# ColdCloudd/QKD_LDPC

Hardware: AMD Instinct MI355X
Metric: decoded key bits/sec + FER, N=10240 R=0.49 @ QBER=0.02, 50 iters (higher is better)
Workload: dtype f64; 1 GPU; configs[1]: alist (N=10240,M=5231,R=0.49,CW=3,SEED=666), QBER 0.02, <= 50 iterations, clamp 100.0, 4096-frame batch per GPU; frames_per_gpu=4096, decoder=sp_f64, parallelism=frames sharded over 1 GPU(s), counters all-reduced

## Files before the change

### include/qkd_ldpc.h

```cpp
#ifndef QKD_LDPC_H
#define QKD_LDPC_H

#include <stddef.h>
#include <stdint.h>

#ifdef __cplusplus
extern "C" {
#endif

#define QKD_LDPC_ABI_VERSION 1

#if defined(__GNUC__)
#define QKD_API __attribute__((visibility("default")))
#else
#define QKD_API
#endif

typedef enum qkd_status {
    QKD_OK = 0,
    QKD_ERR_INVALID_ARG = 1,
    QKD_ERR_BAD_CODE = 2,
    QKD_ERR_UNSORTED = 3,
    QKD_ERR_QBER_TOO_SMALL = 4,
    QKD_ERR_DEVICE = 5,
    QKD_ERR_OUT_OF_MEMORY = 6,
    QKD_ERR_IO = 7,
    QKD_ERR_UNSUPPORTED = 8
} qkd_status;

#define QKD_FLAG_THRESHOLD 0x1u

#define QKD_VARIANT_MASK   0x30u
#define QKD_VARIANT_SP_F64 0x00u
#define QKD_VARIANT_SP_F32 0x10u
#define QKD_VARIANT_MINSUM 0x20u
#define QKD_MINSUM_SCALE_SHIFT 8
#define QKD_MINSUM_SCALE(x) ((((uint32_t)((x) * 256.0 + 0.5)) & 0xffu) << QKD_MINSUM_SCALE_SHIFT)
#define QKD_MINSUM_DEFAULT_SCALE 0.8125
#define QKD_MINSUM_OFFSET_SHIFT 16
#define QKD_MINSUM_OFFSET(x) ((((uint32_t)((x) * 64.0 + 0.5)) & 0xffu) << QKD_MINSUM_OFFSET_SHIFT)
#define QKD_MINSUM_SELF_CORRECT 0x1000000u

typedef struct qkd_code qkd_code;
typedef struct qkd_workspace qkd_workspace;

typedef struct qkd_code_info {
    int32_t n_bits;
    int32_t n_checks;
    int32_t n_edges;
    int32_t max_bit_degree;
    int32_t max_check_degree;
    int32_t is_regular;
    int32_t device;
} qkd_code_info;

typedef struct qkd_counters {
    uint64_t frames;
    uint64_t sp_ok;
    uint64_t ldpc_ok;
    uint64_t sum_iters;
    uint64_t sum_iters_sq;
    uint32_t min_iters;
    uint32_t max_iters;
} qkd_counters;

QKD_API int qkd_abi_version(void);
QKD_API const char *qkd_last_error(void);
QKD_API const char *qkd_status_string(qkd_status s);
QKD_API int qkd_device_count(void);

QKD_API qkd_code *qkd_code_create(int32_t n_bits, int32_t n_checks, const int32_t *check_ptr,
                          const int32_t *check_idx, int device, qkd_status *status);
QKD_API qkd_code *qkd_code_from_alist(const char *path, int device, qkd_status *status);
#define QKD_READ_SORT_ROWS 0x1u
QKD_API qkd_code *qkd_code_from_alist_ex(const char *path, int device, uint32_t read_flags,
                                         qkd_status *status);
QKD_API qkd_code *qkd_code_from_dense(const char *path, int device, qkd_status *status);
QKD_API void qkd_code_destroy(qkd_code *code);
QKD_API qkd_status qkd_code_get_info(const qkd_code *code, qkd_code_info *info);
QKD_API qkd_status qkd_code_get_adjacency(const qkd_code *code, int32_t *check_ptr, int32_t *check_idx,
                                  int32_t *bit_ptr, int32_t *bit_idx);

QKD_API qkd_workspace *qkd_workspace_create(const qkd_code *code, qkd_status *status);
QKD_API void qkd_workspace_destroy(qkd_workspace *ws);


QKD_API qkd_status qkd_syndrome_batch(const qkd_code *code, const uint8_t *bits, size_t n_frames,
                              uint8_t *syndrome, void *stream);

QKD_API qkd_status qkd_decode_batch(const qkd_code *code, qkd_workspace *ws, const double *llr,
                            const uint8_t *syndrome, size_t n_frames, uint32_t max_iterations,
                            double msg_threshold, uint32_t flags, uint8_t *bits_out,
                            uint32_t *iterations, uint8_t *syndromes_match, void *stream);

QKD_API qkd_status qkd_qkd_ldpc_batch(const qkd_code *code, qkd_workspace *ws, const uint8_t *alice,
                              const uint8_t *bob, size_t n_frames, double qber,
                              uint32_t max_iterations, double msg_threshold, uint32_t flags,
                              uint8_t *bits_out, uint32_t *iterations, uint8_t *syndromes_match,
                              uint8_t *keys_match, void *stream);

QKD_API qkd_status qkd_keygen_batch(const qkd_code *code, qkd_workspace *ws, const uint64_t *seeds,
                            uint64_t seed_offset, size_t n_frames, double q_nominal,
                            uint8_t *alice, uint8_t *bob, double *exact_qber, void *stream);

QKD_API qkd_status qkd_trials_batch(const qkd_code *code, qkd_workspace *ws, const uint64_t *seeds,
                            uint64_t seed_offset, size_t n_frames, double q_nominal,
                            uint32_t max_iterations, double msg_threshold, uint32_t flags,
                            uint32_t *iterations, uint8_t *syndromes_match, uint8_t *keys_match,
                            double *exact_qber, qkd_counters *counters, void *stream);

QKD_API qkd_status qkd_interactive_batch(const qkd_code *code, qkd_workspace *ws, uint64_t simulation_seed,
                                         size_t n_points, const double *q_nominal, uint32_t max_iterations,
                                         double msg_threshold, uint32_t flags, uint32_t *iterations,
                                         uint8_t *syndromes_match, uint8_t *keys_match, double *exact_qber,
                                         uint32_t *errors, size_t *points_done);

QKD_API qkd_status qkd_counters_batch(const uint32_t *iterations, const uint8_t *syndromes_match,
                              const uint8_t *keys_match, size_t n_frames, qkd_counters *counters,
                              int device, void *stream);

QKD_API qkd_status qkd_counters_merge(const qkd_counters *records, size_t n_records, qkd_counters *out,
                                      int device, void *stream);

QKD_API qkd_status qkd_debug_set_option(qkd_workspace *ws, const char *name, const char *value);
QKD_API qkd_status qkd_debug_phase_cycles(qkd_workspace *ws, uint64_t *cycles7);
QKD_API qkd_status qkd_debug_decoder_timing(qkd_workspace *ws, int start, double *ms_total, uint64_t *launches);
QKD_API qkd_status qkd_debug_spec_replays(qkd_workspace *ws, uint64_t *replays, int reset);
QKD_API qkd_status qkd_trace_decode(const qkd_code *code, const double *llr, const uint8_t *syndrome,
                                    uint32_t max_iterations, double msg_threshold, uint32_t flags,
                                    double *c2b_trace, double *total_trace, uint32_t *iterations,
                                    uint8_t *syndrome_match);
QKD_API qkd_status qkd_debug_math(int which, const double *x, double *y, size_t n, void *stream);
QKD_API qkd_status qkd_debug_phi_sweep(int which, uint32_t first_bits, uint32_t last_bits, uint64_t *result);

QKD_API qkd_status qkd_debug_bit_order(int32_t n_bits, int32_t n_checks, const int32_t *check_ptr,
                                       const int32_t *check_idx, const char *mode, int32_t *perm_out,
                                       uint32_t *plan_out, int32_t *n_tasks_out);

QKD_API qkd_status qkd_make_seeds(uint64_t simulation_seed, size_t count, uint64_t *seeds_host);
QKD_API qkd_status qkd_qber_range(double begin, double end, double step, double *values_host,
                          size_t capacity, size_t *count);

#ifdef __cplusplus
}
#endif

#endif
```

### qkd_ldpc_amd/__init__.py

```python
from __future__ import annotations

import ctypes as C
from dataclasses import dataclass

import numpy as np

from . import _native as N
from ._native import FLAG_THRESHOLD, QkdError

try:
    import torch
except Exception:
    torch = None

__all__ = [
    "HMatrix", "QkdError", "calculate_syndrome", "sum_product_decoding",
    "sum_product_decoding_irregular", "sum_product_decoding_regular", "qkd_ldpc",
    "QKD_LDPC_irregular", "QKD_LDPC_regular", "keygen", "run_trials", "make_seeds",
    "qber_range", "Workspace", "counters_to_stats", "decoder_flags", "trace_decode", "set_debug_option",
    "spec_replays", "interactive_simulation",
]


def decoder_flags(threshold_enabled: bool = True, variant: str = "sp_f64",
                  minsum_scale: float | None = None, minsum_offset: float | None = None,
                  minsum_self_correct: bool = False) -> int:
    if variant not in N.VARIANTS:
        raise ValueError(f"unknown decoder variant {variant!r}; one of {sorted(N.VARIANTS)}")
    flags = (FLAG_THRESHOLD if threshold_enabled else 0) | N.VARIANTS[variant]
    if minsum_scale is not None:
        if variant != "minsum":
            raise ValueError("minsum_scale applies to variant='minsum' only")
        q = round(minsum_scale * 256)
        if not (1 <= q <= 255) or q != minsum_scale * 256:
            raise ValueError("minsum_scale must be k/256 for k in 1..255")
        flags |= q << N.MINSUM_SCALE_SHIFT
    if minsum_offset is not None:
        if variant != "minsum":
            raise ValueError("minsum_offset applies to variant='minsum' only")
        q = round(minsum_offset * 64)
        if not (0 <= q <= 255) or q != minsum_offset * 64:
            raise ValueError("minsum_offset must be k/64 for k in 0..255")
        flags |= q << N.MINSUM_OFFSET_SHIFT
    if minsum_self_correct:
        if variant != "minsum":
            raise ValueError("minsum_self_correct applies to variant='minsum' only")
        flags |= N.MINSUM_SELF_CORRECT
    return flags


def _ptr(t) -> int | None:
    if t is None:
        return None
    return int(t.data_ptr())


def _stream(stream, device: int) -> int | None:
    if stream is None:
        return int(torch.cuda.current_stream(device).cuda_stream)
    if isinstance(stream, int):
        return stream
    return int(stream.cuda_stream)


def _need_cuda(t, dtype, name, H: "HMatrix | None" = None):
    if not (isinstance(t, torch.Tensor) and t.is_cuda and t.dtype == dtype and t.is_contiguous()):
        raise QkdError(N.ERR_INVALID_ARG, f"{name} must be a contiguous {dtype} CUDA tensor")
    if H is not None and t.device.index != H.device:
        raise QkdError(N.ERR_INVALID_ARG,
                       f"{name} is on {t.device}, the code lives on cuda:{H.device}")


def _frames(t, width: int, name: str, frames: int | None = None) -> int:
    if t.dim() == 1 and t.numel() == width:
        f = 1
    elif t.dim() == 2 and t.shape[1] == width:
        f = int(t.shape[0])
    else:
        raise QkdError(N.ERR_INVALID_ARG,
                       f"{name} must have shape [F, {width}], got {list(t.shape)}")
    if frames is not None and f != frames:
        raise QkdError(N.ERR_INVALID_ARG, f"{name} holds {f} frames, expected {frames}")
    return f


def _need_vec(t, dtype, count: int, name: str, H: "HMatrix"):
    _need_cuda(t, dtype, name, H)
    if t.numel() != count:
        raise QkdError(N.ERR_INVALID_ARG, f"{name} must hold {count} elements, got {t.numel()}")


class HMatrix:

    def __init__(self, handle: int):
        self._h = C.c_void_p(handle)
        info = N.CodeInfo()
        N.check(N.lib().qkd_code_get_info(self._h, C.byref(info)))
        self.num_bit_nodes = info.n_bits
        self.num_check_nodes = info.n_checks
        self.n_edges = info.n_edges
        self.max_bit_nodes_weight = info.max_bit_degree
        self.max_check_nodes_weight = info.max_check_degree
        self.is_regular = bool(info.is_regular)
        self.device = info.device

    @classmethod
    def _make(cls, fn, *args):
        st = C.c_int(0)
        h = fn(*args, C.byref(st))
        if not h:
            raise QkdError(st.value, N.last_error())
        return cls(h)

    @classmethod
    def from_alist(cls, path: str, device: int = 0, sort_rows: bool = False) -> "HMatrix":
        return cls._make(N.lib().qkd_code_from_alist_ex, str(path).encode(), device,
                         N.READ_SORT_ROWS if sort_rows else 0)

    @classmethod
    def from_dense(cls, path: str, device: int = 0) -> "HMatrix":
        return cls._make(N.lib().qkd_code_from_dense, str(path).encode(), device)

    @classmethod
    def from_check_lists(cls, n_bits: int, check_ptr, check_idx, device: int = 0) -> "HMatrix":
        cp = np.ascontiguousarray(check_ptr, dtype=np.int32)
        ci = np.ascontiguousarray(check_idx, dtype=np.int32)
        return cls._make(N.lib().qkd_code_create, n_bits, cp.size - 1, cp.ctypes.data,
                         ci.ctypes.data, device)

    @classmethod
    def from_dense_array(cls, dense, device: int = 0) -> "HMatrix":
        d = np.asarray(dense)
        ptr, idx = [0], []
        for row in d:
            idx.extend(np.nonzero(row)[0].tolist())
            ptr.append(len(idx))
        return cls.from_check_lists(d.shape[1], ptr, idx, device)

    def adjacency(self):
        n, m, e = self.num_bit_nodes, self.num_check_nodes, self.n_edges
        cp = np.zeros(m + 1, np.int32)
        ci = np.zeros(e, np.int32)
        bp = np.zeros(n + 1, np.int32)
        bi = np.zeros(e, np.int32)
        N.check(N.lib().qkd_code_get_adjacency(self._h, cp.ctypes.data, ci.ctypes.data,
                                               bp.ctypes.data, bi.ctypes.data))
        return cp, ci, bp, bi

    @property
    def handle(self):
        return self._h

    def close(self):
        if getattr(self, "_h", None) is not None and self._h.value:
            N.lib().qkd_code_destroy(self._h)
            self._h = None

    def __del__(self):
        try:
            self.close()
        except Exception:
            pass


class Workspace:

    def __init__(self, H: HMatrix):
        st = C.c_int(0)
        h = N.lib().qkd_workspace_create(H.handle, C.byref(st))
        if not h:
            raise QkdError(st.value, N.last_error())
        self._h = C.c_void_p(h)

    @property
    def handle(self):
        return self._h

    def close(self):
        if getattr(self, "_h", None) is not None and self._h.value:
            N.lib().qkd_workspace_destroy(self._h)
            self._h = None

    def __del__(self):
        try:
            self.close()
        except Exception:
            pass


def _ws(ws):
    return ws.handle if ws is not None else None


def set_debug_option(name: str, value=None, workspace: "Workspace | None" = None) -> None:
    v = None if value is None else str(value).encode()
    N.check(N.lib().qkd_debug_set_option(_ws(workspace), name.encode(), v))


def spec_replays(ws: Workspace, reset: bool = False) -> int:
    v = C.c_uint64(0)
    N.check(N.lib().qkd_debug_spec_replays(ws.handle, C.byref(v), int(reset)))
    return int(v.value)


def calculate_syndrome(H: HMatrix, bits, stream=None):
    _need_cuda(bits, torch.uint8, "bits", H)
    f = _frames(bits, H.num_bit_nodes, "bits")
    out = torch.empty((f, H.num_check_nodes), dtype=torch.uint8, device=bits.device)
    N.check(N.lib().qkd_syndrome_batch(H.handle, _ptr(bits), f, _ptr(out), _stream(stream, H.device)))
    return out


@dataclass
class SPResult:
    iterations: "torch.Tensor"
    syndromes_match: "torch.Tensor"
    bits: "torch.Tensor | None"


@dataclass
class LDPCResult:
    iterations: "torch.Tensor"
    syndromes_match: "torch.Tensor"
    keys_match: "torch.Tensor"
    bits: "torch.Tensor | None"


def sum_product_decoding(H: HMatrix, llr, syndrome, max_iterations: int = 50,
                         msg_threshold: float = 100.0, threshold_enabled: bool = True,
                         want_bits: bool = True, workspace=None, stream=None,
                         variant: str = "sp_f64", minsum_scale: float | None = None,
                         minsum_offset: float | None = None, minsum_self_correct: bool = False) -> SPResult:
    _need_cuda(llr, torch.float64, "llr", H)
    _need_cuda(syndrome, torch.uint8, "syndrome", H)
    f = _frames(llr, H.num_bit_nodes, "llr")
    _frames(syndrome, H.num_check_nodes, "syndrome", f)
    dev = llr.device
    bits = torch.empty((f, H.num_bit_nodes), dtype=torch.uint8, device=dev) if want_bits else None
    iters = torch.empty(f, dtype=torch.int32, device=dev)
    ok = torch.empty(f, dtype=torch.uint8, device=dev)
    flags = decoder_flags(threshold_enabled, variant, minsum_scale, minsum_offset, minsum_self_correct)
    N.check(N.lib().qkd_decode_batch(H.handle, _ws(workspace), _ptr(llr), _ptr(syndrome), f,
                                     max_iterations, msg_threshold, flags, _ptr(bits), _ptr(iters),
                                     _ptr(ok), _stream(stream, H.device)))
    return SPResult(iters, ok, bits)


sum_product_decoding_irregular = sum_product_decoding
sum_product_decoding_regular = sum_product_decoding


def qkd_ldpc(H: HMatrix, alice, bob, qber: float, max_iterations: int = 50,
             msg_threshold: float = 100.0, threshold_enabled: bool = True,
             want_bits: bool = False, workspace=None, stream=None,
             variant: str = "sp_f64", minsum_scale: float | None = None,
             minsum_offset: float | None = None, minsum_self_correct: bool = False) -> LDPCResult:
    _need_cuda(alice, torch.uint8, "alice", H)
    _need_cuda(bob, torch.uint8, "bob", H)
    f = _frames(alice, H.num_bit_nodes, "alice")
    _frames(bob, H.num_bit_nodes, "bob", f)
    dev = alice.device
    bits = torch.empty((f, H.num_bit_nodes), dtype=torch.uint8, device=dev) if want_bits else None
    iters = torch.empty(f, dtype=torch.int32, device=dev)
    ok = torch.empty(f, dtype=torch.uint8, device=dev)
    km = torch.empty(f, dtype=torch.uint8, device=dev)
    flags = decoder_flags(threshold_enabled, variant, minsum_scale, minsum_offset, minsum_self_correct)
    N.check(N.lib().qkd_qkd_ldpc_batch(H.handle, _ws(workspace), _ptr(alice), _ptr(bob), f, qber,
                                       max_iterations, msg_threshold, flags, _ptr(bits),
                                       _ptr(iters), _ptr(ok), _ptr(km), _stream(stream, H.device)))
    return LDPCResult(iters, ok, km, bits)


QKD_LDPC_irregular = qkd_ldpc
QKD_LDPC_regular = qkd_ldpc


def keygen(H: HMatrix, seeds, q_nominal: float, seed_offset: int = 0, workspace=None,
           stream=None):
    _need_cuda(seeds, torch.int64, "seeds", H)
    if seeds.dim() != 1:
        raise QkdError(N.ERR_INVALID_ARG, f"seeds must be 1-D, got {list(seeds.shape)}")
    f = seeds.numel()
    dev = seeds.device
    a = torch.empty((f, H.num_bit_nodes), dtype=torch.uint8, device=dev)
    b = torch.empty_like(a)
    q = torch.empty(f, dtype=torch.float64, device=dev)
    N.check(N.lib().qkd_keygen_batch(H.handle, _ws(workspace), _ptr(seeds), seed_offset, f,
                                     q_nominal, _ptr(a), _ptr(b), _ptr(q), _stream(stream, H.device)))
    return a, b, q


@dataclass
class TrialResults:
    iterations: "torch.Tensor"
    syndromes_match: "torch.Tensor"
    keys_match: "torch.Tensor"
    exact_qber: "torch.Tensor"
    counters: "torch.Tensor"


def run_trials(H: HMatrix, seeds, q_nominal: float, seed_offset: int = 0,
               max_iterations: int = 50, msg_threshold: float = 100.0,
               threshold_enabled: bool = True, workspace=None, stream=None,
               out: TrialResults | None = None, variant: str = "sp_f64",
               minsum_scale: float | None = None, minsum_offset: float | None = None,
               minsum_self_correct: bool = False) -> TrialResults:
    _need_cuda(seeds, torch.int64, "seeds", H)
    if seeds.dim() != 1:
        raise QkdError(N.ERR_INVALID_ARG, f"seeds must be 1-D, got {list(seeds.shape)}")
    f = seeds.numel()
    dev = seeds.device
    if out is not None:
        _need_vec(out.iterations, torch.int32, f, "out.iterations", H)
        _need_vec(out.syndromes_match, torch.uint8, f, "out.syndromes_match", H)
        _need_vec(out.keys_match, torch.uint8, f, "out.keys_match", H)
        _need_vec(out.exact_qber, torch.float64, f, "out.exact_qber", H)
        _need_vec(out.counters, torch.uint8, N.COUNTERS_BYTES, "out.counters", H)
    if out is None:
        out = TrialResults(torch.empty(f, dtype=torch.int32, device=dev),
                           torch.empty(f, dtype=torch.uint8, device=dev),
                           torch.empty(f, dtype=torch.uint8, device=dev),
                           torch.empty(f, dtype=torch.float64, device=dev),
                           torch.empty(N.COUNTERS_BYTES, dtype=torch.uint8, device=dev))
    flags = decoder_flags(threshold_enabled, variant, minsum_scale, minsum_offset, minsum_self_correct)
    N.check(N.lib().qkd_trials_batch(H.handle, _ws(workspace), _ptr(seeds), seed_offset, f,
                                     q_nominal, max_iterations, msg_threshold, flags,
                                     _ptr(out.iterations), _ptr(out.syndromes_match),
                                     _ptr(out.keys_match), _ptr(out.exact_qber),
                                     _ptr(out.counters), _stream(stream, H.device)))
    return out


def interactive_simulation(H: HMatrix, simulation_seed: int, qbers, max_iterations: int = 50,
                           msg_threshold: float = 100.0, threshold_enabled: bool = True,
                           workspace=None, variant: str = "sp_f64") -> dict:
    q = np.ascontiguousarray(qbers, dtype=np.float64)
    p = q.size
    it = np.zeros(p, np.uint32)
    sp = np.zeros(p, np.uint8)
    ko = np.zeros(p, np.uint8)
    ex = np.zeros(p, np.float64)
    er = np.zeros(p, np.uint32)
    done = C.c_size_t(0)
    st = N.lib().qkd_interactive_batch(H.handle, _ws(workspace), simulation_seed, p, q.ctypes.data,
                                       max_iterations, msg_threshold,
                                       decoder_flags(threshold_enabled, variant), it.ctypes.data,
                                       sp.ctypes.data, ko.ctypes.data, ex.ctypes.data, er.ctypes.data,
                                       C.byref(done))
    k = done.value
    out = {"points_done": k, "exact_qber": ex[:k], "errors": er[:k], "iterations": it[:k],
           "syndromes_match": sp[:k].astype(bool), "keys_match": ko[:k].astype(bool),
           "success": (sp[:k] & ko[:k]).astype(bool)}
    if st != N.OK:
        err = QkdError(st, N.last_error())
        err.partial = out
# ... 91 lines not shown
```

### qkd_ldpc_amd/_native.py

```python
from __future__ import annotations

import ctypes as C
import os

try:
    import torch
except Exception:
    torch = None

_HERE = os.path.dirname(os.path.abspath(__file__))
LIB_PATH = os.path.join(_HERE, "lib", "libqkd_ldpc_amd.so")
if os.environ.get("QKD_AMD_LIB"):
    if os.environ.get("QKD_AMD_DIAGNOSTIC") == "1":
        import sys as _sys
        LIB_PATH = os.environ["QKD_AMD_LIB"]
        print(f"qkd_ldpc_amd: DIAGNOSTIC build {LIB_PATH} in place of the product library",
              file=_sys.stderr)
    else:
        raise ImportError("QKD_AMD_LIB is set without QKD_AMD_DIAGNOSTIC=1: refusing to load a "
                          "library other than the in-tree product build")

OK = 0
ERR_INVALID_ARG = 1
ERR_BAD_CODE = 2
ERR_UNSORTED = 3
ERR_QBER_TOO_SMALL = 4
ERR_DEVICE = 5
ERR_OUT_OF_MEMORY = 6
ERR_IO = 7
ERR_UNSUPPORTED = 8

FLAG_THRESHOLD = 0x1
READ_SORT_ROWS = 0x1
VARIANTS = {"sp_f64": 0x00, "sp_f32": 0x10, "minsum": 0x20}
MINSUM_SCALE_SHIFT = 8
MINSUM_OFFSET_SHIFT = 16
MINSUM_SELF_CORRECT = 1 << 24
MINSUM_DEFAULT_SCALE = 0.8125

EXPORTS = [
    "qkd_abi_version", "qkd_last_error", "qkd_status_string", "qkd_device_count",
    "qkd_code_create", "qkd_code_from_alist", "qkd_code_from_dense", "qkd_code_destroy",
    "qkd_code_get_info", "qkd_code_get_adjacency", "qkd_workspace_create",
    "qkd_workspace_destroy", "qkd_syndrome_batch", "qkd_decode_batch", "qkd_qkd_ldpc_batch",
    "qkd_keygen_batch", "qkd_trials_batch", "qkd_counters_batch", "qkd_make_seeds",
    "qkd_qber_range", "qkd_debug_phase_cycles", "qkd_debug_spec_replays", "qkd_debug_math", "qkd_debug_phi_sweep", "qkd_trace_decode",
    "qkd_interactive_batch",
    "qkd_code_from_alist_ex", "qkd_debug_decoder_timing", "qkd_debug_bit_order",
    "qkd_counters_merge", "qkd_debug_set_option",
]


class CodeInfo(C.Structure):
    _fields_ = [(n, C.c_int32) for n in ("n_bits", "n_checks", "n_edges", "max_bit_degree",
                                         "max_check_degree", "is_regular", "device")]


class Counters(C.Structure):
    _fields_ = [("frames", C.c_uint64), ("sp_ok", C.c_uint64), ("ldpc_ok", C.c_uint64),
                ("sum_iters", C.c_uint64), ("sum_iters_sq", C.c_uint64),
                ("min_iters", C.c_uint32), ("max_iters", C.c_uint32)]


COUNTERS_BYTES = C.sizeof(Counters)


class QkdError(RuntimeError):

    def __init__(self, status: int, message: str):
        super().__init__(message or f"qkd status {status}")
        self.status = status


_lib = None


def lib():
    global _lib
    if _lib is None:
        if not os.path.exists(LIB_PATH):
            raise ImportError(
                f"{LIB_PATH} is missing: build it with `python -m qkd_ldpc_amd.build` "
                "(hipcc --offload-arch=gfx950). There is no CPU fallback.")
        L = C.CDLL(LIB_PATH)
        P, I32, U32, U64, SZ, D = C.c_void_p, C.c_int32, C.c_uint32, C.c_uint64, C.c_size_t, C.c_double
        st = C.c_int
        sig = {
            "qkd_abi_version": (C.c_int, []),
            "qkd_last_error": (C.c_char_p, []),
            "qkd_status_string": (C.c_char_p, [st]),
            "qkd_device_count": (C.c_int, []),
            "qkd_code_create": (P, [I32, I32, P, P, C.c_int, C.POINTER(st)]),
            "qkd_code_from_alist": (P, [C.c_char_p, C.c_int, C.POINTER(st)]),
            "qkd_code_from_alist_ex": (P, [C.c_char_p, C.c_int, U32, C.POINTER(st)]),
            "qkd_code_from_dense": (P, [C.c_char_p, C.c_int, C.POINTER(st)]),
            "qkd_code_destroy": (None, [P]),
            "qkd_code_get_info": (st, [P, C.POINTER(CodeInfo)]),
            "qkd_code_get_adjacency": (st, [P, P, P, P, P]),
            "qkd_workspace_create": (P, [P, C.POINTER(st)]),
            "qkd_workspace_destroy": (None, [P]),
            "qkd_syndrome_batch": (st, [P, P, SZ, P, P]),
            "qkd_decode_batch": (st, [P, P, P, P, SZ, U32, D, U32, P, P, P, P]),
            "qkd_qkd_ldpc_batch": (st, [P, P, P, P, SZ, D, U32, D, U32, P, P, P, P, P]),
            "qkd_keygen_batch": (st, [P, P, P, U64, SZ, D, P, P, P, P]),
            "qkd_trials_batch": (st, [P, P, P, U64, SZ, D, U32, D, U32, P, P, P, P, P, P]),
            "qkd_counters_batch": (st, [P, P, P, SZ, P, C.c_int, P]),
            "qkd_counters_merge": (st, [P, SZ, P, C.c_int, P]),
            "qkd_make_seeds": (st, [U64, SZ, P]),
            "qkd_qber_range": (st, [D, D, D, P, SZ, C.POINTER(SZ)]),
            "qkd_debug_phase_cycles": (st, [P, P]),
            "qkd_debug_decoder_timing": (st, [P, C.c_int, C.POINTER(D), C.POINTER(U64)]),
            "qkd_debug_spec_replays": (st, [P, P, C.c_int]),
            "qkd_debug_math": (st, [C.c_int, P, P, SZ, P]),
            "qkd_debug_phi_sweep": (st, [C.c_int, C.c_uint32, C.c_uint32, P]),
            "qkd_debug_bit_order": (st, [I32, I32, P, P, C.c_char_p, P, P, C.POINTER(I32)]),
            "qkd_debug_set_option": (st, [P, C.c_char_p, C.c_char_p]),
            "qkd_interactive_batch": (st, [P, P, C.c_uint64, SZ, P, C.c_uint32, C.c_double, C.c_uint32,
                                           P, P, P, P, P, P]),
            "qkd_trace_decode": (st, [P, P, P, U32, D, U32, P, P, P, P]),
        }
        diagnostic = os.environ.get("QKD_AMD_LIB") and os.environ.get("QKD_AMD_DIAGNOSTIC") == "1"
        for name, (res, args) in sig.items():
            if diagnostic and not hasattr(L, name):
                continue
            fn = getattr(L, name)
            fn.restype = res
            fn.argtypes = args
        _lib = L
    return _lib


def last_error() -> str:
    return lib().qkd_last_error().decode(errors="replace")


def check(status: int) -> None:
    if status != OK:
        raise QkdError(status, last_error())
```

### qkd_ldpc_amd/csrc/decode.hip

```cpp
#include <hip/hip_runtime.h>

#include <algorithm>
#include <cmath>
#include <limits>
#include <cstdlib>
#include <cstring>

#include "qkd_internal.h"
#include "qkd_math.h"
#include "qkd_plan.h"
#include "qkd_rng.h"
#include "qkd_decode.h"
#include "qkd_spec.h"

namespace qkd {

template <int SRC, bool CLAMP, int DC, int RULE, typename T>
__device__ __forceinline__ void check_phase(const uint2* __restrict__ plan, const uint32_t* tsyn,
                                            const T* total, const uint16_t* t2idx, const double* tab2,
                                            T* __restrict__ c2b, T* row, int n_tasks, int n_pad, T thr,
                                            int wave, int lane, float ms_scale, float ms_offset) {
    constexpr int NW = kDecodeBlock / 64;
    constexpr bool FIRST = SRC != kSrcGeneral;
    int t = wave;
// ... 1104 lines not shown
}

static bool decode_ms_fits(const qkd_code* c, bool sc) {
    if (c->max_dc > 32 || c->n > kMaxBitsLds) return false;
    const int dc = c->max_dc <= 4 ? 4 : c->max_dc <= 6 ? 6 : c->max_dc <= 8 ? 8 : c->max_dc <= 16 ? 16 : 32;
    return decode_lds_bytes(c, dc, 0, kRuleMinSumLds, false, sc) <= kLdsBytesMax;
}

static qkd_status decode_grid(const qkd_code* c, DecodeFn fn, size_t lds, int* grid) {
    QKD_HIP(hipFuncSetAttribute((const void*)fn, hipFuncAttributeMaxDynamicSharedMemorySize, (int)lds));
    int per_cu = 0;
    QKD_HIP(hipOccupancyMaxActiveBlocksPerMultiprocessor(&per_cu, (const void*)fn, kDecodeBlock, lds));
    if (per_cu < 1) return set_error(QKD_ERR_UNSUPPORTED, "decode kernel cannot be resident (LDS %zu B)", lds);
    *grid = per_cu * c->cu_count;
    return QKD_OK;
}

qkd_status ws_reserve_decode(qkd_workspace* ws, size_t slots) {
    const qkd_code* c = ws->code;
    if (!ws->counter) {
        QKD_HIP(hipMalloc(&ws->counter, 128));
        QKD_HIP(hipMemset(ws->counter, 0, 128));
    }
    if (ws->c2b_slots >= slots) return QKD_OK;
    if (ws->c2b) QKD_HIP(hipFree(ws->c2b));
    ws->c2b = nullptr;
    ws->c2b_slots = 0;
    const size_t bytes = slots * ((size_t)c->max_dv + 1) * c->n_pad * sizeof(double);
    if (hipMalloc(&ws->c2b, bytes) != hipSuccess)
        return set_error(QKD_ERR_OUT_OF_MEMORY, "workspace: cannot allocate %zu B of c2b scratch", bytes);
    ws->c2b_slots = slots;
    return QKD_OK;
}

qkd_status ws_reserve_keys(qkd_workspace* ws, size_t frames, size_t low_words) {
    const qkd_code* c = ws->code;
    const size_t words = (size_t)(c->n + 63) / 64;
    if (ws->key_frames < frames) {
        if (ws->alice_w) QKD_HIP(hipFree(ws->alice_w));
        if (ws->bob_w) QKD_HIP(hipFree(ws->bob_w));
        if (ws->synw) QKD_HIP(hipFree(ws->synw));
        if (ws->zout) QKD_HIP(hipFree(ws->zout));
        ws->alice_w = ws->bob_w = ws->zout = nullptr;
        ws->synw = nullptr;
        ws->key_frames = 0;
        const size_t syn_words = 2 * (size_t)decode_m_words(c->m);
        if (hipMalloc(&ws->alice_w, frames * words * 8) != hipSuccess ||
            hipMalloc(&ws->bob_w, frames * words * 8) != hipSuccess ||
            hipMalloc(&ws->synw, frames * syn_words * 4) != hipSuccess ||
            hipMalloc(&ws->zout, frames * words * 8) != hipSuccess)
            return set_error(QKD_ERR_OUT_OF_MEMORY, "workspace: cannot allocate keys for %zu frames", frames);
        ws->key_frames = frames;
    }
    if (ws->low_words < low_words) {
        if (ws->low) QKD_HIP(hipFree(ws->low));
        ws->low = nullptr;
        ws->low_words = 0;
        if (hipMalloc(&ws->low, low_words * 4) != hipSuccess)
            return set_error(QKD_ERR_OUT_OF_MEMORY, "workspace: cannot allocate shuffle scratch");
        ws->low_words = low_words;
    }
    return QKD_OK;
}

static qkd_status ws_free(qkd_workspace* ws) {
    DeviceGuard g(ws->device);
    if (ws->c2b) (void)hipFree(ws->c2b);
    if (ws->counter) (void)hipFree(ws->counter);
    if (ws->alice_w) (void)hipFree(ws->alice_w);
    if (ws->bob_w) (void)hipFree(ws->bob_w);
    if (ws->synw) (void)hipFree(ws->synw);
    if (ws->zout) (void)hipFree(ws->zout);
    if (ws->low) (void)hipFree(ws->low);
    if (ws->ckpt) (void)hipFree(ws->ckpt);
    if (ws->win) (void)hipFree(ws->win);
    if (ws->ilv) (void)hipFree(ws->ilv);
    if (ws->fb_list) (void)hipFree(ws->fb_list);
    if (ws->spec_stat_ev) (void)hipEventSynchronize(ws->spec_stat_ev);
    if (ws->spec_stat_host) (void)hipHostFree(ws->spec_stat_host);
    if (ws->spec_stat_ev) (void)hipEventDestroy(ws->spec_stat_ev);
    if (ws->done) (void)hipEventDestroy(ws->done);
    for (hipEvent_t e : ws->dec_ev) (void)hipEventDestroy(e);
    return QKD_OK;
}

static std::mutex g_default_ws_mu;

qkd_workspace* resolve_ws(const qkd_code* code, qkd_workspace* ws) {
    if (ws) return ws;
    std::lock_guard<std::mutex> lk(g_default_ws_mu);
    if (!code->default_ws) {
        qkd_status s;
        const_cast<qkd_code*>(code)->default_ws = qkd_workspace_create(code, &s);
    }
    return code->default_ws;
}

struct WsSession {
    qkd_workspace* ws;
    hipStream_t stream;
    std::unique_lock<std::mutex> lk;
    WsSession(qkd_workspace* w, hipStream_t s) : ws(w), stream(s), lk(w->mu) {
        if (ws->done) (void)hipStreamWaitEvent(stream, ws->done, 0);
    }
    ~WsSession() {
        if (!ws->done) (void)hipEventCreateWithFlags(&ws->done, hipEventDisableTiming);
        if (ws->done) (void)hipEventRecord(ws->done, stream);
    }
};

static unsigned blocks_for(size_t n, unsigned bs) { return (unsigned)((n + bs - 1) / bs); }

static constexpr size_t kDecEvPairsMax = 256;
static hipError_t decoder_events_fold(qkd_workspace* ws) {
    const size_t pairs = ws->dec_ev_used / 2;
    double ms_sum = 0.0;
    for (size_t k = 0; k < pairs; ++k) {
        hipError_t r = hipEventSynchronize(ws->dec_ev[2 * k + 1]);
        float ms = 0.0f;
        if (r == hipSuccess) r = hipEventElapsedTime(&ms, ws->dec_ev[2 * k], ws->dec_ev[2 * k + 1]);
        if (r != hipSuccess) return r;
        ms_sum += ms;
    }
    ws->dec_ms_folded += ms_sum;
    ws->dec_pairs_folded += pairs;
    ws->dec_ev_used = 0;
    return hipSuccess;
}
static hipError_t decoder_event(qkd_workspace* ws, hipStream_t stream) {
    if (!ws->time_decoder) return hipSuccess;
    if (ws->dec_ev_used >= 2 * kDecEvPairsMax) {
        const hipError_t r = decoder_events_fold(ws);
        if (r != hipSuccess) return r;
    }
    while (ws->dec_ev.size() < ws->dec_ev_used + 2) {
        hipEvent_t e = nullptr;
        const hipError_t r = hipEventCreate(&e);
        if (r != hipSuccess) return r;
        ws->dec_ev.push_back(e);
    }
    const hipError_t r = hipEventRecord(ws->dec_ev[ws->dec_ev_used], stream);
    if (r == hipSuccess) ws->dec_ev_used++;
    return r;
}
static hipError_t decoder_event_close(qkd_workspace* ws, hipStream_t stream, hipError_t launch) {
    if (!ws->time_decoder) return launch;
    hipError_t r = launch;
    if (r == hipSuccess) r = hipEventRecord(ws->dec_ev[ws->dec_ev_used], stream);
    if (r == hipSuccess) ws->dec_ev_used++;
    else ws->dec_ev_used--;
    return r;
}

static qkd_status plan_for_layout(const qkd_code* c, const SplitLds& L, int dc, const uint2** out, int esz = 8) {
    std::lock_guard<std::mutex> lock(c->plan_mu);
    const auto key = std::make_pair(L.S, ((uint32_t)L.msg << 8) | (uint32_t)dc | (esz == 4 ? 0x80u : 0u));
    auto it = c->d_plan_enc.find(key);
    if (it == c->d_plan_enc.end()) {
        std::vector<uint2> enc(c->plan_slot_host);
        for (size_t k = 0; k < enc.size(); ++k) {
            uint2& w = enc[k];
            w.x = esz == 4 ? (uint32_t)L.msg + w.x * 4u : encode_slot(w.x, L.S, (uint32_t)L.msg, (uint32_t)sizeof(double));
            w.y = encode_seg(w.y & qkdp::kPlanChkMask, (w.y >> 20) & 63u, (w.y >> 26) + 1, (uint32_t)(k & 63),
                             (uint32_t)dc);
        }
        uint2* d = nullptr;
        if (hipMalloc(&d, enc.size() * sizeof(uint2)) != hipSuccess)
            return set_error(QKD_ERR_OUT_OF_MEMORY, "code: cannot allocate %zu B for an encoded plan",
                             enc.size() * sizeof(uint2));
        if (hipMemcpy(d, enc.data(), enc.size() * sizeof(uint2), hipMemcpyHostToDevice) != hipSuccess) {
            (void)hipFree(d);
            return set_error(QKD_ERR_DEVICE, "code: encoded plan upload failed");
        }
        it = c->d_plan_enc.emplace(key, d).first;
    }
    *out = it->second;
    return QKD_OK;
}

static qkd_status check_no_static_lds(DecodeFn fn) {
    static std::mutex mu;
    static std::map<const void*, size_t> seen;
    std::lock_guard<std::mutex> lock(mu);
    auto it = seen.find((const void*)fn);
    if (it == seen.end()) {
        hipFuncAttributes fa{};
        QKD_HIP(hipFuncGetAttributes(&fa, (const void*)fn));
        it = seen.emplace((const void*)fn, fa.sharedSizeBytes).first;
    }
    if (it->second != 0)
        return set_error(QKD_ERR_UNSUPPORTED, "split decoder with %zu B of static LDS (its slot words "
                                              "address LDS from 0)", it->second);
    return QKD_OK;
}

static qkd_status launch_decode(const qkd_code* c, qkd_workspace* ws, DecodeArgs& a, int mode,
                                uint32_t flags, hipStream_t stream) {
    int dc = 0;
    int rule = rule_of(flags);
    const DbgOpt ms_store = debug_option(ws, "QKD_MINSUM_STORE");
    const bool ms_global = ms_store.is("global");
    const bool ms_lds = ms_store.is("lds");
    a.ms_sc = (flags & QKD_MINSUM_SELF_CORRECT) ? 1 : 0;
    const bool classic = debug_option(ws, "QKD_DECODE_KERNEL").is("classic");
    if (rule == kRuleMinSum && !ms_global && !ms_lds && !classic && !a.trace && c->d_bit_code &&
        c->n <= kMaxBitsSplit && c->m <= kMaxChecksSplit && c->max_dc <= 8) {
        const SplitLds Lm(c->n_pad, (c->n + 63) / 64, c->m, c->max_dv, c->max_dc <= 4 ? 4 : c->max_dc <= 6 ? 6 : 8,
                          0, a.ms_sc ? 2 * c->n_tasks + (c->n + 63) / 64 : 0, 4, kLdsBytesMax);
        if (Lm.S >= (uint32_t)((size_t)c->max_dv * c->n_pad) && Lm.bytes <= kLdsBytesMax)
            rule = a.ms_sc ? kRuleMinSumSplitSc : kRuleMinSumSplit;
    }
    if (rule == kRuleMinSum && !ms_global && decode_ms_fits(c, a.ms_sc != 0)) rule = kRuleMinSumLds;
    if (a.ms_sc && rule != kRuleMinSumLds && rule != kRuleMinSumSplitSc)
        return set_error(QKD_ERR_UNSUPPORTED, "self-corrected min-sum needs the split or the LDS-state min-sum "
                                              "kernel (check degree <= 32, its state in LDS)");
    if (a.ms_sc && rule == kRuleMinSumLds) rule = kRuleMinSumLdsSc;
    a.ms_scale = minsum_scale_of(flags);
    a.ms_offset = (float)((flags >> QKD_MINSUM_OFFSET_SHIFT) & 0xffu) / 64.0f;
    const bool msr = rule == kRuleMinSumSplit || rule == kRuleMinSumSplitSc;
    const bool long_code = c->n > kMaxBitsSplit;
    const bool long_ok = rule == kRuleSp64 && mode == kModeKeys && c->n <= kMaxBitsSplitLong && c->d_ilv_slots &&
                         c->max_dc <= 16;
    if ((rule == kRuleSp64 || rule == kRuleSp32 || msr) && !classic && !a.trace && (!long_code || long_ok) &&
        c->m <= kMaxChecksSplit) {
        const DecodeArgs a_in = a;
        int sdc = 0;
        DecodeFn sfn = long_code ? pick_split_long(a.clamp_on != 0, c->max_dc, &sdc)
                                 : pick_split_decode(mode, rule, a.clamp_on != 0, c->max_dc, &sdc);
        const int esz = rule == kRuleSp64 ? 8 : 4;
        size_t budget = kLdsBytesMax;
        if (const DbgOpt b = debug_option(ws, "QKD_SPLIT_BUDGET")) budget = std::min(budget, (size_t)b.as_long());
        const bool spec = rule == kRuleSp64 && a.spec_cap > 0 && a.clamp_on &&
                          (mode == kModeLlr || a.first_table) && c->max_dv <= kDvUnroll && c->d_bit_code;
        const bool ckpt = spec && mode == kModeKeys && a.ckpt_unsat > 0;
        a.ftab_entries = (spec && !ckpt && mode == kModeKeys && a.tab2_entries &&
                          c->n_pat * kFoldTabPat <= kFoldTabMaxEntries)
                             ? c->n_pat * kFoldTabPat : 0;
        if (const DbgOpt e = debug_option(ws, "QKD_FOLD_TABLE")) if (e.as_int() == 0) a.ftab_entries = 0;
        if (debug_option(ws, "QKD_SPEC_POLICY").is("always")) a.spec_always = 1u;
        if (rule == kRuleMinSumSplitSc) a.ftab_entries = 2 * c->n_tasks + (c->n + 63) / 64;
        if (long_code) a.ftab_entries = std::max(a.ftab_entries, (c->n + 63) / 64);
        const SplitLds L(c->n_pad, (c->n + 63) / 64, c->m, c->max_dv, sdc, a.tab2_entries, a.ftab_entries, esz,
                         budget);
        const bool fits = rule != kRuleSp64 ? L.S >= (uint32_t)((size_t)c->max_dv * c->n_pad) : L.S >= 64;
        if (L.bytes <= kLdsBytesMax && fits) {
            int grid = 0;
            qkd_status s = decode_grid(c, sfn, L.bytes, &grid);
            if (s != QKD_OK) return s;
            grid = (int)std::min<size_t>((size_t)grid, a.n_frames);
            if (const DbgOpt g = debug_option(ws, "QKD_DECODE_GRID")) grid = std::max(1, std::min(grid, g.as_int()));
            s = ws_reserve_decode(ws, (size_t)grid);
            if (s != QKD_OK) return s;
            a.code = c->view_split();
            a.c2b = ws->c2b;
            a.plan_enc = nullptr;
            if (rule == kRuleSp64 || msr) {
                s = plan_for_layout(c, L, sdc, &a.plan_enc, esz);
                if (s != QKD_OK) return s;
            }
            const size_t slots = (size_t)c->max_dv * c->n_pad;
            if (const DbgOpt e = debug_option(ws, "QKD_C2B_PAD")) {
                const size_t pad = std::min((size_t)e.as_long(), (size_t)c->n_pad);
                a.c2b_stride = ((slots - L.S + 31) & ~(size_t)31) + pad;
            } else {
                size_t st = (slots - L.S + kC2bPad - 1) / kC2bPad;
                if ((st & 1u) == 0) st++;
                a.c2b_stride = st * kC2bPad;
            }
            if (rule == kRuleSp64 && kSlotGlobalBase + a.c2b_stride * sizeof(double) >= kSlotLds)
                return set_error(QKD_ERR_UNSUPPORTED, "code too large for the split decoder's slot words "
                                                      "(%zu global slots per frame)", a.c2b_stride);
            a.lds_budget = (uint32_t)budget;
            a.counter = ws->counter;
            const bool timing = (bool)debug_option(ws, "QKD_PHASE_TIMING");
            a.phase = nullptr;
            if (timing) {
                a.phase = reinterpret_cast<unsigned long long*>(reinterpret_cast<char*>(ws->counter) + 64);
                QKD_HIP(hipMemsetAsync(a.phase, 0, 64, stream));
            }
            a.replay_count = ws->counter + 1;
            a.spec_replays = reinterpret_cast<unsigned long long*>(reinterpret_cast<char*>(ws->counter) + 120);
            if (spec) {
                if (!long_code) {
                    int xdc = 0, sgrid = 0;
                    DecodeFn xfn = pick_split_spec(mode, c->max_dc, ckpt, &xdc);
                    if (xdc != sdc)
                        return set_error(QKD_ERR_UNSUPPORTED, "speculative kernel bucket %d != %d", xdc, sdc);
                    s = decode_grid(c, xfn, L.bytes, &sgrid);
                    if (s != QKD_OK) return s;
                    sfn = xfn;
                    grid = std::min(sgrid, grid);
                }
                if (ckpt && !long_code) {
                    const size_t need = (size_t)grid * slots;
                    if (ws->ckpt_slots < need) {
                        if (ws->ckpt) QKD_HIP(hipFree(ws->ckpt));
                        ws->ckpt = nullptr;
                        ws->ckpt_slots = 0;
                        if (hipMalloc(&ws->ckpt, need * sizeof(double)) != hipSuccess)
                            return set_error(QKD_ERR_OUT_OF_MEMORY, "workspace: cannot allocate %zu B of checkpoints",
                                             need * sizeof(double));
                        ws->ckpt_slots = need;
                    }
                    a.ckpt = ws->ckpt;
                    a.ckpt_stride = (uint32_t)slots;
                }
            }
            a.win = nullptr;
            a.win_count = 0;
            if (spec) {
                a.win_shift = kSpecWinShift;
                a.win_lag = kSpecWinLag;
                a.win_count = (uint32_t)((a.n_frames + (1u << kSpecWinShift) - 1) >> kSpecWinShift);
                const size_t need = 2 * (size_t)a.win_count;
                if (ws->win_words < need) {
                    if (ws->win) QKD_HIP(hipFree(ws->win));
                    ws->win = nullptr;
                    ws->win_words = 0;
                    if (hipMalloc(&ws->win, need * sizeof(uint32_t)) != hipSuccess)
                        return set_error(QKD_ERR_OUT_OF_MEMORY, "workspace: cannot allocate the policy windows");
                    ws->win_words = need;
                }
                a.win = ws->win;
            }
            if (rule == kRuleSp64 || msr) {
                s = check_no_static_lds(sfn);
                if (s != QKD_OK) return s;
            }
            const bool tsg = IlvLds(c->m, false).bytes > kLdsBytesMax;
            const bool ug = tsg && IlvLds(c->m, true).bytes > kLdsBytesMax;
            const IlvLds IL(c->m, tsg, ug);
            bool ilv = mode == kModeKeys && spec && !ckpt && !a.bits_out && a.first_table && c->d_ilv_slots &&
                       IL.bytes <= kLdsBytesMax;
            bool ilv_forced = false;
            if (ilv) {
                const DbgOpt ie = debug_option(ws, "QKD_ILV");
                ilv_forced = (bool)ie;
                ilv = ie ? ie.as_int() != 0
                         : (size_t)L.S * 4 < slots && (size_t)a.n_frames * 2 >= (size_t)kIlvCols * c->cu_count;
            }
            DecodeFn ifn = nullptr;
            int igrid = 0;
            const size_t istride = (slots * kIlvCols + (size_t)((c->n + 63) / 64) * kIlvCols * 2 +
                                    (ug ? 2 : 1) * (((size_t)(c->m + 1) / 2 + 1) / 2) + 63) & ~(size_t)63;
            if (ilv) {
                ifn = pick_ilv(c->ilv_rs, c->max_dc, tsg, ug);
                QKD_HIP(hipFuncSetAttribute((const void*)ifn, hipFuncAttributeMaxDynamicSharedMemorySize, (int)IL.bytes));
                int per_cu = 0;
                QKD_HIP(hipOccupancyMaxActiveBlocksPerMultiprocessor(&per_cu, (const void*)ifn, kIlvBlock, IL.bytes));
                if (per_cu < 1) return set_error(QKD_ERR_UNSUPPORTED, "interleaved decoder cannot be resident");
                igrid = per_cu * c->cu_count;
                igrid = (int)std::min<size_t>((size_t)igrid, ((size_t)a.n_frames + kIlvCols - 1) / kIlvCols);
                if (const DbgOpt g = debug_option(ws, "QKD_ILV_GRID")) igrid = std::max(1, std::min(igrid, g.as_int()));
                const size_t need = (size_t)igrid * istride;
                if (ws->ilv_elems < need) {
                    if (ws->ilv) QKD_HIP(hipFree(ws->ilv));
                    ws->ilv = nullptr;
                    ws->ilv_elems = 0;
                    if (hipMalloc(&ws->ilv, need * sizeof(double)) != hipSuccess) {
                        (void)hipGetLastError();
                        if (ilv_forced)
                            return set_error(QKD_ERR_OUT_OF_MEMORY, "workspace: cannot allocate %zu B of "
                                                                    "interleaved message lines", need * sizeof(double));
                        ilv = false;
                    } else {
                        ws->ilv_elems = need;
                    }
                }
            }
            if (long_code && !ilv) {
                a = a_in;
                goto classic_path;
            }
            if (ilv) {
                if (ws->fb_frames < a.n_frames) {
                    if (ws->fb_list) QKD_HIP(hipFree(ws->fb_list));
                    ws->fb_list = nullptr;
                    ws->fb_frames = 0;
                    if (hipMalloc(&ws->fb_list, (size_t)a.n_frames * sizeof(uint32_t)) != hipSuccess)
                        return set_error(QKD_ERR_OUT_OF_MEMORY, "workspace: cannot allocate the hand-off list");
                    ws->fb_frames = a.n_frames;
                }
            }
            if (mode == kModeKeys) {
                a.synw = ws->synw;
                a.zout = ws->zout;
                QKD_HIP(launch_frame_syn(a, stream, debug_option(ws, "QKD_SYN_SLICED").is("0"),
                                         debug_option(ws, "QKD_SYN_BYTES").is("0")));
            } else {
                QKD_HIP(hipMemsetAsync(ws->counter, 0, 8, stream));
                if (a.win) QKD_HIP(hipMemsetAsync(a.win, 0, 2 * (size_t)a.win_count * sizeof(uint32_t), stream));
            }
            QKD_HIP(decoder_event(ws, stream));
            if (ilv) {
                QKD_HIP(hipMemsetAsync(ws->counter + 2, 0, 8, stream));
                DecodeArgs ai = a;
                ai.ilv_store = ws->ilv;
                ai.ilv_stride = istride;
                ai.fb_list = ws->fb_list;
                ai.fb_count = ws->counter + 3;
                hipLaunchKernelGGL(ifn, dim3(igrid), dim3(kIlvBlock), IL.bytes, stream, ai);
                DecodeArgs af = a;
                af.counter = ws->counter + 2;
                af.frame_list = ws->fb_list;
                af.frame_count = ws->counter + 3;
                af.spec_cap = 0;
                af.spec_always = 1;
                af.phase = nullptr;
                int xdc = 0;
                DecodeFn ffn = long_code ? pick_split_long(a.clamp_on != 0, c->max_dc, &xdc)
                                         : pick_split_decode(mode, rule, a.clamp_on != 0, c->max_dc, &xdc);
// ... 552 lines not shown
            hi = b.y * 0.6931471805599453;
            sl = e.slope;
        } else {
            const float at = __builtin_fminf(a, qkds::kPsiHuge);
            const qkds::PhiVal e = qkds::phi_core<false, true>(at * qkds::kLn2, __builtin_amdgcn_exp2f(-at),
                                                               __builtin_amdgcn_logf(at));
            const qkds::f2 b = qkds::phi_bounds_out(a, a);
            S = (double)at * 0.6931471805599453;
            v = e.v;
            lo = b.x;
            hi = b.y;
            sl = e.slope;
        }
        const double u = exp(-S), w = -expm1(-S);
        const double phi = log1p(2.0 * u / w);
        const double dphi = 2.0 * u / (w * (1.0 + u));
        ++pts;
        bad_hi += hi < phi;
        bad_lo += lo > phi;
        bad_sl += sl * (1.0 + R) < dphi;
        if (phi > 1e-30 && bits >= 0x00800000u && v < 3.0e38) {
            const float err = (float)(fabs(v / phi - 1.0) / R);
            if (err > e_max) { e_max = err; e_at = bits; }
        }
        const float sr = (float)(dphi / sl);
        if (sr > s_max && bits >= 0x00800000u) { s_max = sr; s_at = bits; }
    }
    atomicAdd(&cnt[0], pts);
    if (bad_hi) atomicAdd(&cnt[1], bad_hi);
    if (bad_lo) atomicAdd(&cnt[2], bad_lo);
    if (bad_sl) atomicAdd(&cnt[3], bad_sl);
    sweep_max(e_max, e_at, &mx[0], &mx[2]);
    sweep_max(s_max, s_at, &mx[1], &mx[3]);
}

qkd_status qkd_debug_phi_sweep(int which, uint32_t first_bits, uint32_t last_bits, uint64_t* result) {
    clear_error();
    if ((which != 4 && which != 5) || !result || first_bits > last_bits || last_bits >= 0x7f800000u)
        return set_error(QKD_ERR_INVALID_ARG, "bad argument");
    unsigned long long* d_cnt = nullptr;
    uint32_t* d_mx = nullptr;
    QKD_HIP(hipMalloc(&d_cnt, 4 * sizeof(unsigned long long)));
    if (hipMalloc(&d_mx, 4 * sizeof(uint32_t)) != hipSuccess) {
        (void)hipFree(d_cnt);
        return set_error(QKD_ERR_OUT_OF_MEMORY, "phi sweep: cannot allocate");
    }
    hipError_t e = hipMemset(d_cnt, 0, 4 * sizeof(unsigned long long));
    if (e == hipSuccess) e = hipMemset(d_mx, 0, 4 * sizeof(uint32_t));
    if (e == hipSuccess) {
        hipLaunchKernelGGL(phi_sweep_kernel, dim3(4096), dim3(256), 0, nullptr, which, first_bits, last_bits, d_cnt,
                           d_mx);
        e = hipGetLastError();
    }
    unsigned long long cnt[4] = {0, 0, 0, 0};
    uint32_t mx[4] = {0, 0, 0, 0};
    if (e == hipSuccess) e = hipMemcpy(cnt, d_cnt, sizeof cnt, hipMemcpyDeviceToHost);
    if (e == hipSuccess) e = hipMemcpy(mx, d_mx, sizeof mx, hipMemcpyDeviceToHost);
    (void)hipFree(d_cnt);
    (void)hipFree(d_mx);
    if (e != hipSuccess) return set_error(QKD_ERR_DEVICE, "phi sweep: %s", hipGetErrorString(e));
    for (int k = 0; k < 4; ++k) result[k] = cnt[k];
    for (int k = 0; k < 4; ++k) result[4 + k] = mx[k];
    return QKD_OK;
}

qkd_status qkd_trace_decode(const qkd_code* c, const double* llr, const uint8_t* syndrome,
                            uint32_t max_iterations, double msg_threshold, uint32_t flags,
                            double* c2b_trace, double* total_trace, uint32_t* iterations,
                            uint8_t* syndrome_match) {
    clear_error();
    if (!c || !llr || !syndrome || !iterations || !syndrome_match)
        return set_error(QKD_ERR_INVALID_ARG, "null argument");
    qkd_status s = check_decode_params(max_iterations, msg_threshold, flags);
    if (s != QKD_OK) return s;
    if ((flags & QKD_VARIANT_MASK) != QKD_VARIANT_SP_F64)
        return set_error(QKD_ERR_UNSUPPORTED, "trace is provided for the reference rule (QKD_VARIANT_SP_F64) only");
    DeviceGuard g(c->device);
    qkd_workspace* ws = qkd_workspace_create(c, &s);
    if (!ws) return s;
    const size_t stride = (size_t)c->max_dv * c->n_pad + c->n_pad;
    double *d_llr = nullptr, *d_tr = nullptr;
    uint8_t *d_syn = nullptr, *d_ok = nullptr;
    uint32_t* d_it = nullptr;
    auto cleanup = [&]() {
        for (void* p : {(void*)d_llr, (void*)d_tr, (void*)d_syn, (void*)d_ok, (void*)d_it})
            if (p) (void)hipFree(p);
        qkd_workspace_destroy(ws);
    };
    hipStream_t st = nullptr;
    if (hipMalloc(&d_llr, (size_t)c->n * 8) != hipSuccess || hipMalloc(&d_syn, (size_t)c->m) != hipSuccess ||
        hipMalloc(&d_ok, 1) != hipSuccess || hipMalloc(&d_it, 4) != hipSuccess ||
        hipMalloc(&d_tr, stride * max_iterations * 8) != hipSuccess) {
        cleanup();
        return set_error(QKD_ERR_OUT_OF_MEMORY, "trace: cannot allocate %zu B", stride * max_iterations * 8);
    }
    std::vector<uint8_t> syn01((size_t)c->m);
    for (int32_t j = 0; j < c->m; ++j) syn01[j] = syndrome[j] ? 1 : 0;
    hipError_t e = hipMemcpy(d_llr, llr, (size_t)c->n * 8, hipMemcpyHostToDevice);
    if (e == hipSuccess) e = hipMemcpy(d_syn, syn01.data(), (size_t)c->m, hipMemcpyHostToDevice);
    if (e != hipSuccess) {
        cleanup();
        return set_error(QKD_ERR_DEVICE, "trace: %s", hipGetErrorString(e));
    }
    DecodeArgs a{};
    a.pinf = std::numeric_limits<float>::infinity();
    a.n_frames = 1;
    a.max_it = max_iterations;
    a.thr = msg_threshold;
    a.clamp_on = (flags & QKD_FLAG_THRESHOLD) ? 1 : 0;
    a.llr = d_llr;
    a.syn = d_syn;
    a.iters = d_it;
    a.sp_ok = d_ok;
    a.trace = d_tr;
    a.trace_stride = stride;
    s = launch_decode(c, ws, a, kModeLlr, flags, st);
    if (s == QKD_OK) {
        std::vector<double> tr(stride * max_iterations);
        e = hipDeviceSynchronize();
        if (e == hipSuccess) e = hipMemcpy(iterations, d_it, 4, hipMemcpyDeviceToHost);
        if (e == hipSuccess) e = hipMemcpy(syndrome_match, d_ok, 1, hipMemcpyDeviceToHost);
        if (e == hipSuccess) e = hipMemcpy(tr.data(), d_tr, tr.size() * 8, hipMemcpyDeviceToHost);
        if (e != hipSuccess) {
            s = set_error(QKD_ERR_DEVICE, "trace: %s", hipGetErrorString(e));
        } else {
            const size_t nm = (size_t)c->max_dv * c->n_pad;
            for (uint32_t t = 0; t < *iterations; ++t) {
                const double* src = tr.data() + t * stride;
                if (c2b_trace)
                    for (int32_t i = 0; i < c->n; ++i)
                        for (int32_t k = 0; k < c->bit_ptr[i + 1] - c->bit_ptr[i]; ++k)
                            c2b_trace[(size_t)t * c->e + c->bit_ptr[i] + k] = src[(size_t)k * c->n_pad + i];
                if (total_trace)
                    for (int32_t i = 0; i < c->n; ++i) total_trace[(size_t)t * c->n + i] = src[nm + i];
            }
        }
    }
    cleanup();
    return s;
}

qkd_status qkd_debug_spec_replays(qkd_workspace* ws, uint64_t* replays, int reset) {
    if (!ws || !replays) return set_error(QKD_ERR_INVALID_ARG, "null argument");
    *replays = 0;
    if (!ws->counter) return QKD_OK;
    DeviceGuard g(ws->device);
    QKD_HIP(hipDeviceSynchronize());
    char* p = reinterpret_cast<char*>(ws->counter) + 120;
    QKD_HIP(hipMemcpy(replays, p, 8, hipMemcpyDeviceToHost));
    if (reset) QKD_HIP(hipMemset(p, 0, 8));
    return QKD_OK;
}

qkd_status qkd_debug_decoder_timing(qkd_workspace* ws, int start, double* ms_total, uint64_t* launches) {
    if (!ws) return set_error(QKD_ERR_INVALID_ARG, "null workspace");
    DeviceGuard g(ws->device);
    std::lock_guard<std::mutex> lk(ws->mu);
    if (!start) QKD_HIP(decoder_events_fold(ws));
    if (ms_total) *ms_total = start ? 0.0 : ws->dec_ms_folded;
    if (launches) *launches = start ? 0 : ws->dec_pairs_folded;
    ws->dec_ev_used = 0;
    ws->dec_ms_folded = 0.0;
    ws->dec_pairs_folded = 0;
    ws->time_decoder = start != 0;
    return QKD_OK;
}

qkd_status qkd_debug_phase_cycles(qkd_workspace* ws, uint64_t* cycles7) {
    if (!ws || !cycles7) return set_error(QKD_ERR_INVALID_ARG, "null argument");
    if (!ws->counter) return set_error(QKD_ERR_INVALID_ARG, "workspace has not decoded yet");
    DeviceGuard g(ws->device);
    QKD_HIP(hipDeviceSynchronize());
    QKD_HIP(hipMemcpy(cycles7, reinterpret_cast<char*>(ws->counter) + 64, 56, hipMemcpyDeviceToHost));
    return QKD_OK;
}

qkd_status qkd_counters_batch(const uint32_t* iterations, const uint8_t* syndromes_match,
                              const uint8_t* keys_match, size_t n_frames, qkd_counters* counters,
                              int device, void* stream) {
    clear_error();
    if (!iterations || !syndromes_match || !counters) return set_error(QKD_ERR_INVALID_ARG, "null argument");
    qkd_status s = check_frames(n_frames);
    if (s != QKD_OK) return s;
    DeviceGuard g(device);
    QKD_HIP(launch_counters(iterations, syndromes_match, keys_match, n_frames, counters, (hipStream_t)stream));
    return QKD_OK;
}

qkd_status qkd_counters_merge(const qkd_counters* records, size_t n_records, qkd_counters* out, int device,
                              void* stream) {
    clear_error();
    if (!records || !out) return set_error(QKD_ERR_INVALID_ARG, "null argument");
    if (n_records == 0 || n_records > 0xffffffffu) return set_error(QKD_ERR_INVALID_ARG, "bad record count");
    DeviceGuard g(device);
    hipLaunchKernelGGL(counters_merge_kernel, dim3(1), dim3(64), 0, (hipStream_t)stream, records,
                       (uint32_t)n_records, out);
    QKD_HIP(hipGetLastError());
    return QKD_OK;
}

qkd_status qkd_trials_batch(const qkd_code* c, qkd_workspace* ws, const uint64_t* seeds,
                            uint64_t seed_offset, size_t n_frames, double q_nominal,
                            uint32_t max_iterations, double msg_threshold, uint32_t flags,
                            uint32_t* iterations, uint8_t* syndromes_match, uint8_t* keys_match,
                            double* exact_qber, qkd_counters* counters, void* stream) {
    clear_error();
    if (!c || !seeds || !iterations || !syndromes_match)
        return set_error(QKD_ERR_INVALID_ARG, "null argument");
    qkd_status s = check_frames(n_frames);
    if (s == QKD_OK) s = check_decode_params(max_iterations, msg_threshold, flags);
    if (s != QKD_OK) return s;
    if (!(q_nominal > 0.0 && q_nominal < 1.0)) return set_error(QKD_ERR_INVALID_ARG, "QBER must be in (0,1)");
    DeviceGuard g(c->device);
    ws = resolve_ws(c, ws);
    if (!ws) return set_error(QKD_ERR_OUT_OF_MEMORY, "no workspace");
    WsSession sess(ws, (hipStream_t)stream);
    s = keygen_into_ws(c, ws, seeds, seed_offset, n_frames, q_nominal, exact_qber, (hipStream_t)stream);
    if (s != QKD_OK) return s;
    const double q = (double)qkdr::num_errors((uint32_t)c->n, q_nominal) / (double)c->n;
    s = decode_keys(c, ws, n_frames, q, max_iterations, msg_threshold, flags, nullptr, iterations,
                    syndromes_match, keys_match, (hipStream_t)stream);
    if (s != QKD_OK) return s;
    if (counters) QKD_HIP(launch_counters(iterations, syndromes_match, keys_match, n_frames, counters,
                                          (hipStream_t)stream));
    return QKD_OK;
}

}
```

### qkd_ldpc_amd/csrc/decode_split.hip

```cpp
#include <hip/hip_runtime.h>

#include <type_traits>

#include "qkd_decode.h"
#include "qkd_spec.h"

namespace qkd {

#ifndef QKD_RUN_SYN
#define QKD_RUN_SYN 1
#endif
constexpr bool kRunSyn = QKD_RUN_SYN != 0;

template <int DC>
struct SegWeights {
    const float* w;
    uint64_t mask;
    __device__ __forceinline__ SegWeights(const float* wtab, int deg, int p) {
        if constexpr (DC <= 8) {
            w = wtab + (deg * 8 + min(p, DC - 1)) * DC;
            mask = 0;
        } else {
            w = nullptr;
            const uint64_t seg = deg >= 64 ? ~0ull : ((1ull << (uint32_t)deg) - 1ull);
// ... 414 lines not shown
            }
        }
    };
    using Full = std::integral_constant<bool, true>;
    using Part = std::integral_constant<bool, false>;
    for (int r0 = 0; __builtin_amdgcn_readfirstlane(r0 * kDecodeBlock) < cn; r0 += kSp32Chunk) {
        if ((r0 + kSp32Chunk) * kDecodeBlock <= cn) batch(Full{}, r0);
        else batch(Part{}, r0);
    }
}

template <int DC>
__device__ __forceinline__ void spec_check_phase_psi(const uint2* __restrict__ plan, const uint32_t* tsyn,
                                                 const SplitStore<double>& ms, double* row, const float* wtab,
                                                 int n_tasks,
                                                 uint32_t n_pad, uint32_t dummy, float thr_dn, float thr_up,
                                                 uint32_t* round_word, int wave, int lane) {
    using qkds::f2;
    constexpr int NW = kDecodeBlock / 64;
    int t = wave;
    if (t >= n_tasks) return;
    const __amdgpu_buffer_rsrc_t prs = plan_rsrc(plan);
    uint32_t bad = 0;
    if (lane < DC) row[64 + lane] = 0.0;
    auto slot = [&](uint2 p) -> uint32_t { return pw_slot(p); };
    auto input = [&](double xv, uint2 w, bool& neg) -> f2 {
        const f2 bv = qkds::unpack_iv(xv);
        neg = bv.x < 0.0f;
        const bool ok = bv.x == bv.x;
        bad |= fold64(__ballot(!ok) & __ballot(pw_slot(w) != dummy));
        return neg_iv_if(neg, bv);
    };
    uint2 wt = plan_word(prs, t, lane);
    uint2 wn = plan_word(prs, t + NW, lane);
    uint2 wnn = plan_word(prs, t + 2 * NW, lane);
    bool neg_t;
    row[lane] = qkds::pack_iv(input(ms.ld_w(slot(wt)), wt, neg_t));
    uint64_t sgn_t = __ballot(neg_t);
    uint32_t sb_t = seg_sbit(wt);
    using Raw = SplitStore<double>::Raw;
    auto step = [&](const uint2 w_t, const uint2 w_n, const uint2 w_nn, uint2& w_ld, const Raw& x_n,
                    Raw& x_ld) -> bool {
        w_ld = plan_word(prs, t + 3 * NW, lane);
        x_ld = ms.ld_raw(slot(w_nn));
        const uint32_t sb_n = seg_sbit(w_n);
        bool neg_n;
        const f2 ph_n = input(ms.pick(x_n), w_n, neg_n);
        wave_lds_sync();
        const int deg = seg_deg<DC>(w_t);
        const f2 sum = seg_sum<DC>(row, seg_start(w_t), seg_weights<DC>(wtab, w_t, lane));
        const float nr = DC <= 8 ? (float)(DC + 2) : (float)(deg + 2);
        const float mg = __builtin_fmaf(sum.y, nr * qkds::kSumRel, qkds::kRefSumAbs);
        f2 ext = sum + f2{-mg, mg};
        ext.x = ext.x > 0.0f ? ext.x : 0.0f;
        bad |= fold64(__ballot(!(ext.y < qkds::kPsiSumMax)));
        f2 m = qkds::phi_bounds_out(ext.x, ext.y);
        m.x = __builtin_amdgcn_fmed3f(m.x, 0.0f, thr_dn);
        m.y = __builtin_amdgcn_fmed3f(m.y, 0.0f, thr_up);
        const uint32_t sigma = seg_parity_acc<DC>(sgn_t, w_t, sb_t + (neg_t ? 1u : 0u));
        ms.st_w(slot(w_t), qkds::pack_iv(neg_iv_if(sigma != 0u, m)));
        row[lane] = qkds::pack_iv(ph_n);
        sgn_t = __ballot(neg_n);
        neg_t = neg_n;
        sb_t = sb_n;
        t = __builtin_amdgcn_readfirstlane(t + NW);
        return t < n_tasks;
    };
    Raw xa = ms.ld_raw(slot(wn)), xb;
    uint2 wd;
    for (;;) {
        if (!step(wt, wn, wnn, wd, xa, xb)) break;
        if (!step(wn, wnn, wd, wt, xb, xa)) break;
        if (!step(wnn, wd, wt, wn, xa, xb)) break;
        if (!step(wd, wt, wn, wnn, xb, xa)) break;
    }
    if (bad != 0 && lane == 0) atomicOr(round_word, 2u);
}

template <int DC>
__device__ __forceinline__ void spec_check_phase_paired(const uint2* __restrict__ plan, const uint32_t* tsyn,
                                                        const SplitStore<double>& ms, double* row, const float* wtab,
                                                        int n_tasks,
                                                        uint32_t n_pad, uint32_t dummy, float thr_dn, float thr_up,
                                                        uint32_t* round_word, int wave, int lane) {
    using qkds::f2;
    constexpr int NW = kDecodeBlock / 64;
    int t = wave;
    if (t >= n_tasks) return;
    const __amdgpu_buffer_rsrc_t prs = plan_rsrc(plan);
    uint32_t bad = 0;
    if (lane < DC) row[64 + lane] = 0.0;
    auto slot = [&](uint2 p) -> uint32_t { return pw_slot(p); };
    auto input = [&](double xv, uint2 w, bool& neg, f2& ab) -> bool {
        const f2 bv = qkds::unpack_iv(xv);
        neg = bv.y < 0.0f;
        ab = neg_iv_if(neg, bv);
        const bool ok = ab.x > 1.0e-30f;
        bad |= fold64(__ballot(!ok) & __ballot(pw_slot(w) != dummy));
        return ok;
    };
    uint2 wt = plan_word(prs, t, lane);
    uint2 wn = plan_word(prs, t + NW, lane);
    uint2 wnn = plan_word(prs, t + 2 * NW, lane);
    bool neg_t;
    {
        f2 ab;
        const bool ok = input(ms.ld_w(slot(wt)), wt, neg_t, ab);
        row[lane] = qkds::pack_iv(ok ? qkds::phi_bounds(ab.x, ab.y) : f2{0.0f, 0.0f});
    }
    uint64_t sgn_t = __ballot(neg_t);
    uint32_t sb_t = seg_sbit(wt);
    using Raw = SplitStore<double>::Raw;
    auto step = [&](const uint2 w_t, const uint2 w_n, const uint2 w_nn, uint2& w_ld, const Raw& x_n,
                    Raw& x_ld) -> bool {
        w_ld = plan_word(prs, t + 3 * NW, lane);
        x_ld = ms.ld_raw(slot(w_nn));
        const uint32_t sb_n = seg_sbit(w_n);
        bool neg_n;
        f2 ab_n;
        input(ms.pick(x_n), w_n, neg_n, ab_n);
        wave_lds_sync();
        const int start = seg_start(w_t);
        const int deg = seg_deg<DC>(w_t);
        const f2 sum = seg_sum<DC>(row, start, seg_weights<DC>(wtab, w_t, lane));
        const float nr = DC <= 8 ? (float)(DC + 2) : (float)(deg + 2);
        const float mg = __builtin_fmaf(sum.y, nr * qkds::kSumRel, qkds::kRefSumAbs);
        f2 ext = sum + f2{-mg, mg};
        ext.x = ext.x > 0.0f ? ext.x : 0.0f;
        bad |= fold64(__ballot(!(ext.y < qkds::kPsiSumMax)));
        f2 ph_n, m;
        qkds::phi_pair(ab_n.x, ab_n.y, ext.x, ext.y, ph_n, m);
        m.x = __builtin_amdgcn_fmed3f(m.x, 0.0f, thr_dn);
        m.y = __builtin_amdgcn_fmed3f(m.y, 0.0f, thr_up);
        const uint32_t sigma = seg_parity_acc<DC>(sgn_t, w_t, sb_t + (neg_t ? 1u : 0u));
        ms.st_w(slot(w_t), qkds::pack_iv(neg_iv_if(sigma != 0u, m)));
        row[lane] = qkds::pack_iv(ph_n);
        sgn_t = __ballot(neg_n);
        neg_t = neg_n;
        sb_t = sb_n;
        t = __builtin_amdgcn_readfirstlane(t + NW);
        return t < n_tasks;
    };
    Raw xa = ms.ld_raw(slot(wn)), xb;
    uint2 wd;
    for (;;) {
        if (!step(wt, wn, wnn, wd, xa, xb)) break;
        if (!step(wn, wnn, wd, wt, xb, xa)) break;
        if (!step(wnn, wd, wt, wn, xa, xb)) break;
        if (!step(wd, wt, wn, wnn, xb, xa)) break;
    }
    if (bad != 0 && lane == 0) atomicOr(round_word, 2u);
}

__device__ __forceinline__ uint32_t fold_tab_pos(uint32_t p, uint32_t code) { return p * 16u + (code ^ (p & 15u)); }
__device__ void fold_table_fill(const DeviceCode& c, const double* ctab, double log_p, double thr, double* ftab,
                                int entries) {
    static_assert(kFoldTabPat == 64, "16 codes x 4 entries");
    for (int e = threadIdx.x; e < entries; e += kDecodeBlock) {
        const int p = e / kFoldTabPat;
        const uint32_t code = ((uint32_t)e >> 2) & 15u;
        const int k = e & 3;
        const uint32_t at = fold_tab_pos((uint32_t)p, code) * 4u + (uint32_t)k;
        const uint8_t* degs = c.pat_deg + p * c.max_dv;
        double acc = (code & 1u) ? -log_p : log_p;
        double cv[kDvUnroll];
        int dv = 0;
#pragma unroll
        for (int m = 0; m < kDvUnroll; ++m) {
            const int d = m < c.max_dv ? (int)degs[m] : 0;
            if (d != 0 && dv == m) dv = m + 1;
            const double cm = ctab[d];
            cv[m] = ((code >> (1 + m)) & 1u) ? -cm : cm;
        }
#pragma unroll
        for (int m = 0; m < kDvUnroll; ++m) acc = m < dv ? acc + cv[m] : acc;
        double v = 0.0;
        if (k == kDvUnroll) {
            v = __builtin_bit_cast(double, (unsigned long long)(acc <= 0 ? 1 : 0));
        } else if (k < dv) {
            const double ck = k == 0 ? cv[0] : (k == 1 ? cv[1] : cv[2]);
            v = qkds::pack_iv(qkds::psi_of_exact(clamp_msg(acc - ck, thr)));
        }
        ftab[at] = v;
    }
    __syncthreads();
}

#ifndef QKD_IV_CHUNK
#define QKD_IV_CHUNK 2
#endif
constexpr int kIvChunk = QKD_IV_CHUNK;
static_assert(kIvChunk - 1 <= kBitPadRounds, "per-bit arrays padded past the last load batch (host.cpp)");
template <bool FOLD, int MODE, bool DV3>
__device__ __forceinline__ void spec_bit_phase(const DeviceCode& c, const DecodeArgs& a, const SplitStore<double>& ms,
                                               const uint32_t* qsyn, const double* ctab, const double* ftab,
                                               uint32_t* xsyn,
                                               uint32_t* xunc, uint64_t* zw, uint64_t bobmask, bool keep,
                                               uint32_t f, int tid, int wave, int lane) {
    using qkds::f2;
    static_assert(!DV3 || kDvUnroll == 3, "DV3 unrolls three rows");
    const uint32_t n_pad = __builtin_amdgcn_readfirstlane((uint32_t)c.n_pad);
    const int cn = __builtin_amdgcn_readfirstlane(c.n);
    const double llr_p = a.log_p;
#ifndef QKD_FIXED_ROWS
#define QKD_FIXED_ROWS 1
#endif
    const bool fixed_rows = QKD_FIXED_ROWS && DV3 && n_pad <= ms.S && ms.S <= 2 * n_pad;
#ifndef QKD_R1_SPLIT
#define QKD_R1_SPLIT 1
#endif
    const uint32_t vlane = (uint32_t)lane * 8u;
    auto gsoff = [&](int k, uint32_t iw) -> uint32_t {
        return ms.gofs((uint32_t)k * n_pad + iw);
    };
    auto ld_k = [&](auto fx, int k, uint32_t iw, uint32_t i) -> double {
        const uint32_t x = (uint32_t)k * n_pad + i;
        if constexpr (decltype(fx)::value >= 1) {
            if (k == 0) return ms.l[x];
            if (k == 2) return BufIo<double>::ld(ms.gw, vlane, gsoff(k, iw));
            if constexpr (decltype(fx)::value == 2) return ms.l[x];
            if constexpr (decltype(fx)::value == 3) return BufIo<double>::ld(ms.gw, vlane, gsoff(k, iw));
        }
        return ms.ld_row((uint32_t)k * n_pad + iw, x);
    };
    auto st_k = [&](auto fx, int k, uint32_t iw, uint32_t i, double v) {
        const uint32_t x = (uint32_t)k * n_pad + i;
        if constexpr (decltype(fx)::value >= 1) {
            if (k == 0) { ms.l[x] = v; return; }
            if (k == 2) { BufIo<double>::st(ms.gw, vlane, gsoff(k, iw), v); return; }
            if constexpr (decltype(fx)::value == 2) { ms.l[x] = v; return; }
            if constexpr (decltype(fx)::value == 3) { BufIo<double>::st(ms.gw, vlane, gsoff(k, iw), v); return; }
        }
        ms.st_row((uint32_t)k * n_pad + iw, x, v);
    };
    const uint32_t lsign = (uint32_t)qkdm::hi32(a.log_p) >> 31;
    qkds::f2 lpv;
    asm volatile("v_mov_b32 %0, %1" : "=v"(lpv.x) : "s"(a.lp_dn));
    asm volatile("v_mov_b32 %0, %1" : "=v"(lpv.y) : "s"(a.lp_up));
    typedef double VB[kIvChunk][kDvUnroll];
    auto batch_load = [&](auto fx, int r0, VB& v, uint64_t (&bc)[kIvChunk], uint32_t (&pat)[kIvChunk]) {
#pragma unroll
        for (int u = 0; u < kIvChunk; ++u) {
            const int i = tid + (r0 + u) * kDecodeBlock;
            const bool ok = i < cn;
            bc[u] = c.bit_code[i];
            pat[u] = (FOLD && ftab) ? (uint32_t)c.bit_pat[i] : 0u;
            const uint32_t iw = __builtin_amdgcn_readfirstlane((uint32_t)((r0 + u) * kDecodeBlock + wave * 64));
#pragma unroll
            for (int k = 0; k < kDvUnroll; ++k)
                v[u][k] = FOLD ? 0.0 : ld_k(fx, k, iw, (uint32_t)i);
            (void)ok;
        }
    };
    auto batch_compute = [&](auto fx, auto fullc, int r0, VB& v, uint64_t (&bc)[kIvChunk],
                             uint32_t (&pat)[kIvChunk]) {
        constexpr bool FULLC = decltype(fullc)::value;
#pragma unroll
        for (int u = 0; u < kIvChunk; ++u) {
            const int r = r0 + u;
            if (!FULLC && r * kDecodeBlock >= cn) break;
            const int i = tid + r * kDecodeBlock;
            const uint32_t iw = __builtin_amdgcn_readfirstlane((uint32_t)(r * kDecodeBlock + wave * 64));
            const bool full = FULLC || (r + 1) * kDecodeBlock <= cn;
            const bool ok = full || i < cn;
            const int deg = DV3 ? kDvUnroll : (int)(bc[u] >> 48) & 3;
            int32_t jc[kDvUnroll];
#pragma unroll
            for (int k = 0; k < kDvUnroll; ++k) jc[k] = (int32_t)(bc[u] >> (16 * k)) & 0xffff;
            const uint32_t bob = (uint32_t)(bobmask >> r) & 1u;
            bool z, unc = false;
            f2 bo[kDvUnroll];
            if (FOLD && ftab) {
                const uint32_t sgi = bob ^ lsign;
                uint32_t code = bob;
#pragma unroll
                for (int k = 0; k < kDvUnroll; ++k) {
                    const int j = jc[k];
                    code |= (((qsyn[j >> 5] >> (j & 31)) & 1u) ^ sgi) << (1 + k);
                }
                const double* e = ftab + fold_tab_pos(pat[u], code) * 4u;
#pragma unroll
                for (int k = 0; k < kDvUnroll; ++k) bo[k] = qkds::unpack_iv(e[k]);
                z = ok && __builtin_bit_cast(unsigned long long, e[kDvUnroll]) != 0ull;
            } else if (FOLD) {
                const uint32_t sgi = bob ^ lsign;
                double acc = bob ? -llr_p : llr_p;
                double cv[kDvUnroll];
#pragma unroll
                for (int k = 0; k < kDvUnroll; ++k) {
                    const int j = jc[k];
                    const uint32_t sp = (qsyn[j >> 5] >> (j & 31)) & 1u;
                    const double cm = ctab[((uint32_t)(bc[u] >> (50 + 4 * k)) & 15u) + 1u];
                    cv[k] = (DV3 || k < deg) ? ((sp ^ sgi) ? -cm : cm) : 0.0;
                }
#pragma unroll
                for (int k = 0; k < kDvUnroll; ++k) acc = (DV3 || k < deg) ? acc + cv[k] : acc;
                z = ok && acc <= 0;
                static_assert(kDvUnroll == 3, "rows 0 and 1 paired, row 2 alone");
                qkds::psi_of_exact2(clamp_msg(acc - cv[0], a.thr), clamp_msg(acc - cv[1], a.thr), bo[0], bo[1]);
                bo[2] = qkds::psi_of_exact(clamp_msg(acc - cv[2], a.thr));
            } else {
                f2 L;
                if constexpr (MODE == kModeLlr) L = qkds::iv_of(ok ? a.llr[(size_t)f * c.n + c.perm[i]] : 0.0);
                else L = bob ? f2{-lpv.y, -lpv.x} : lpv;
                f2 cs[kDvUnroll];
                f2 T = L;
                const float pinf = a.pinf;
                auto amax = [pinf](f2 x) { return __builtin_amdgcn_fmed3f(x.y, -x.x, pinf); };
                float mag = amax(L);
#pragma unroll
                for (int k = 0; k < kDvUnroll; ++k) {
                    cs[k] = (DV3 || k < deg) ? qkds::unpack_iv(v[u][k]) : f2{0.0f, 0.0f};
                    T = T + cs[k];
                    mag = mag + amax(cs[k]);
                }
                const float mg = __builtin_fmaf(mag, (float)(kDvUnroll + 2) * qkds::kSumRel, 1.0e-30f);
                T = T + f2{-mg, mg};
                const bool z1 = T.y <= 0.0f;
                unc = ok && !(z1 || T.x > 0.0f);
                z = ok && z1;
#pragma unroll
                for (int k = 0; k < kDvUnroll; ++k) {
                    f2 e = L + f2{-mg, mg};
#pragma unroll
                    for (int m = 0; m < kDvUnroll; ++m)
                        if (m != k) e = e + cs[m];
                    bo[k] = f2{__builtin_amdgcn_fmed3f(e.x, -a.thr_up, a.thr_dn),
                               __builtin_amdgcn_fmed3f(e.y, -a.thr_dn, a.thr_up)};
                }
            }
            const uint64_t zb = __ballot(z);
            const bool wave_in = FULLC || r * kDecodeBlock + wave * 64 < cn;
            const bool flip =
                kRunSyn ? (ok && z != (((zw[(r * kDecodeBlock >> 6) + wave] >> lane) & 1ull) != 0)) : z;
            if (lane == 0 && wave_in) zw[(r * kDecodeBlock >> 6) + wave] = zb;
            if (flip) {
#pragma unroll
                for (int k = 0; k < kDvUnroll; ++k) {
                    int32_t j = jc[k];
                    asm volatile("" : "+v"(j));
                    if (DV3 || k < deg) atomicXor(&xsyn[j >> 5], 1u << (j & 31));
                }
            }
            if (unc) {
#pragma unroll
                for (int k = 0; k < kDvUnroll; ++k) {
                    int32_t j = jc[k];
                    asm volatile("" : "+v"(j));
                    if (DV3 || k < deg) atomicOr(&xunc[j >> 5], 1u << (j & 31));
                }
            }
            if (!keep) continue;
            if (DV3 && full) {
#pragma unroll
                for (int k = 0; k < kDvUnroll; ++k) st_k(fx, k, iw, (uint32_t)i, qkds::pack_iv(bo[k]));
            } else if (ok) {
#pragma unroll
                for (int k = 0; k < kDvUnroll; ++k)
                    if (k < deg) ms.st_row((uint32_t)k * n_pad + iw, (uint32_t)k * n_pad + i, qkds::pack_iv(bo[k]));
            }
        }
    };
    using NoFx = std::integral_constant<int, 0>;
    using Fx = std::integral_constant<int, 1>;
    using FxL = std::integral_constant<int, 2>;
    using FxG = std::integral_constant<int, 3>;
    using Full = std::integral_constant<bool, true>;
    using Part = std::integral_constant<bool, false>;
    auto batch = [&](auto fx, auto fullc, int r0) {
        VB v;
        uint64_t bc[kIvChunk];
        uint32_t pat[kIvChunk];
        batch_load(fx, r0, v, bc, pat);
        batch_compute(fx, fullc, r0, v, bc, pat);
    };
    if (fixed_rows) {
        for (int r0 = 0; __builtin_amdgcn_readfirstlane(r0 * kDecodeBlock) < cn; r0 += kIvChunk) {
            const uint32_t x0 = n_pad + __builtin_amdgcn_readfirstlane((uint32_t)(r0 * kDecodeBlock + wave * 64));
            const uint32_t x1 = x0 + (uint32_t)(kIvChunk - 1) * kDecodeBlock;
            const bool full = (r0 + kIvChunk) * kDecodeBlock <= cn;
            if (QKD_R1_SPLIT && full && x1 < ms.S)
                batch(FxL{}, Full{}, r0);
            else if (QKD_R1_SPLIT && full && x0 >= ms.S)
                batch(FxG{}, Full{}, r0);
            else
                batch(Fx{}, Part{}, r0);
        }
    } else {
        for (int r0 = 0; __builtin_amdgcn_readfirstlane(r0 * kDecodeBlock) < cn; r0 += kIvChunk)
            batch(NoFx{}, Part{}, r0);
    }
}

#ifndef QKD_XCD_REGIONS
#define QKD_XCD_REGIONS 1
#endif
__device__ __forceinline__ uint32_t region_of_block() {
    if (QKD_XCD_REGIONS && (gridDim.x & 7u) == 0)
        return (blockIdx.x & 7u) * (gridDim.x >> 3) + (blockIdx.x >> 3);
    return blockIdx.x;
}

#ifdef QKD_SPLIT_WAVES_PER_EU
#define QKD_SPLIT_BOUNDS __launch_bounds__(kDecodeBlock, QKD_SPLIT_WAVES_PER_EU)
#else
#define QKD_SPLIT_BOUNDS __launch_bounds__(kDecodeBlock)
#endif
template <int MODE, int RULE, int DC, bool CLAMP, int SPEC, bool LONG = false>
__global__ QKD_SPLIT_BOUNDS void decode_split_kernel(DecodeArgs a) {
    static_assert(!LONG || (MODE == kModeKeys && RULE == kRuleSp64 && SPEC == 0), "long codes: exact keys path");
    using T = typename RuleMsg<RULE>::T;
    constexpr bool MSR = RULE == kRuleMinSumSplit || RULE == kRuleMinSumSplitSc;
    constexpr bool MSC = RULE == kRuleMinSumSplitSc;
    constexpr bool F32 = RULE != kRuleSp64;
    constexpr bool FOLDS = MODE == kModeKeys && (RULE == kRuleSp64 || RULE == kRuleSp32 || MSR);
    constexpr bool TABLES = MODE == kModeKeys && RULE == kRuleSp64;
    extern __shared__ __attribute__((aligned(16))) char smem[];
    const DeviceCode& c = a.code;
    const SplitLds L(c.n_pad, (c.n + 63) / 64, c.m, c.max_dv, DC, a.tab2_entries, a.ftab_entries, (int)sizeof(T),
                     a.lds_budget);
    const int m_words = decode_m_words(c.m);
    uint32_t* tsyn = reinterpret_cast<uint32_t*>(smem + L.tsyn);
    uint32_t* xsyn = reinterpret_cast<uint32_t*>(smem + L.xsyn);
    uint32_t* qsyn = reinterpret_cast<uint32_t*>(smem + L.qsyn);
    uint32_t* xunc = reinterpret_cast<uint32_t*>(smem + L.xunc);
    uint64_t* zw = reinterpret_cast<uint64_t*>(smem + L.zw);
    uint32_t* ctl = reinterpret_cast<uint32_t*>(smem + L.ctl);
    double* ctab = reinterpret_cast<double*>(smem + L.ctab);
    double* tab2 = reinterpret_cast<double*>(smem + L.tab2);
    float* wtab = reinterpret_cast<float*>(smem + L.wtab);
    for (int e = threadIdx.x; e < seg_weight_entries(DC); e += kDecodeBlock) {
        const int k = e % DC;
        const int p = (e / DC) % 8, deg = e / (DC * 8);
        const bool in = k < deg && k != p;
        wtab[e] = MSR ? (in ? 0.0f : __builtin_inff()) : (in ? 1.0f : 0.0f);
    }
    using MS = SplitStore<T, F32>;
    T* const region = reinterpret_cast<T*>(a.c2b) + (size_t)region_of_block() * a.c2b_stride;
    const MS ms{
        reinterpret_cast<T*>(smem + L.msg),
        L.S,
        __builtin_amdgcn_make_buffer_rsrc(reinterpret_cast<char*>(region) - kSlotGlobalBase, (short)0,
                                          (int)(kSlotGlobalBase + a.c2b_stride * sizeof(T)), 0x00020000),
        kSlotGlobalBase - L.S * (uint32_t)sizeof(T)};
    const uint2* const plan = (RULE == kRuleSp64 || MSR) ? a.plan_enc : c.plan_slot;
    const uint32_t dummy_w = encode_slot((uint32_t)c.n, L.S, (uint32_t)L.msg, (uint32_t)sizeof(T));
    const int tid = threadIdx.x;
    const int lane = tid & 63;
    const int wave = __builtin_amdgcn_readfirstlane(tid >> 6);
    T* row = reinterpret_cast<T*>(smem + L.tval) + wave * (64 + DC);
    const int n_tasks = c.n_tasks;
    const uint32_t n_pad = (uint32_t)c.n_pad;
    const T thr = (T)a.thr;
    const T llr_p = (T)a.log_p;
    const uint32_t lsign = (uint32_t)qkdm::hi32(a.log_p) >> 31;
    const bool fold1 = FOLDS && a.first_table && c.max_dv <= kDvUnroll;
    const bool dv3 = c.min_dv == kDvUnroll && c.max_dv == kDvUnroll;
    const bool tab2_on = fold1 && a.tab2_entries;
    uint32_t rnd = 0;
    if (tid == 0) { ctl[2] = 0; ctl[3] = 0; ctl[4] = 0; ctl[5] = 0; ctl[6] = 1; ctl[7] = 0; }
    static_assert(!SPEC || (RULE == kRuleSp64 && CLAMP), "speculation: binary64 rule, clamped messages");
    constexpr bool CKPT = SPEC == 2;
    static_assert(!CKPT || MODE == kModeKeys, "checkpointed speculation: keys path");
#ifndef QKD_EXACT_CHUNK
#define QKD_EXACT_CHUNK kBitChunk
#endif
    constexpr int BC = SPEC ? kBitChunkSpec : QKD_EXACT_CHUNK;
    if (TABLES && tid <= kFirstTableDeg) ctab[tid] = a.first_c2b[tid];
    if constexpr (RULE == kRuleSp32 && FOLDS) {
        if (tid <= kFirstTableDeg) {
            const float p = __builtin_fabsf(RuleMath<kRuleSp32>::tanh_half((float)a.log_p));
            float S = 0.0f;
            for (int k = 1; k < tid; ++k) S = S + p;
            float v = RuleMath<kRuleSp32>::two_atanh(S);
            if (CLAMP) v = clamp_msg(v, (float)a.thr);
            ctab[tid] = (double)v;
        }
    }
    if constexpr (MSR && FOLDS) {
        if (tid <= kFirstTableDeg) {
            float v = tid <= 1 ? __builtin_inff() : a.ms_scale * __builtin_fabsf((float)a.log_p);
            if (a.ms_offset > 0.0f) v = __builtin_fmaxf(v - a.ms_offset, 0.0f);
            if (CLAMP) v = clamp_msg(v, (float)a.thr);
            ctab[tid] = (double)v;
        }
    }
    uint64_t* const scw = MSC ? reinterpret_cast<uint64_t*>(smem + L.ftab) : nullptr;
    uint64_t* const bwl = MSC ? scw + 2 * c.n_tasks : (LONG ? reinterpret_cast<uint64_t*>(smem + L.ftab) : nullptr);
    if (tab2_on) {
        __syncthreads();
        second_table_fill<CLAMP>(c, ctab, a.log_p, a.thr, tab2, a.tab2_entries);
    }
    double* ftab = nullptr;
    if constexpr (SPEC == 1) {
        if (fold1 && a.ftab_entries) {
            ftab = reinterpret_cast<double*>(smem + L.ftab);
            __syncthreads();
            fold_table_fill(c, ctab, a.log_p, a.thr, ftab, a.ftab_entries);
        }
    }
    PhaseClock pc(a.phase);

    unsigned long long* const win64 = reinterpret_cast<unsigned long long*>(a.win);
    auto window_of = [&](uint32_t fr) -> int {
        if (!SPEC || a.spec_always || fr >= a.n_frames) return -1;
        const uint32_t wn = fr >> a.win_shift;
        return wn < a.win_lag ? -1 : (int)(wn - a.win_lag);
    };
    auto spec_policy = [&](uint32_t fr, unsigned long long v) -> uint32_t {
        const int k = window_of(fr);
        if (k < 0) return 1u;
        const uint32_t W = 1u << a.win_shift;
        for (uint32_t polls = 0; (uint32_t)v < W; ++polls) {
            if (polls >= (1u << 24)) return 1u;
            __builtin_amdgcn_s_sleep(2);
            v = __hip_atomic_load(win64 + k, __ATOMIC_RELAXED, __HIP_MEMORY_SCOPE_AGENT);
        }
        return (uint32_t)(v >> 32) * 6u <= W ? 1u : 0u;
    };
    auto window_peek = [&](uint32_t fr) -> unsigned long long {
        const int k = window_of(fr);
        return k < 0 ? 0ull : __hip_atomic_load(win64 + k, __ATOMIC_RELAXED, __HIP_MEMORY_SCOPE_AGENT);
    };
    auto claim = [&]() -> uint32_t {
        const uint32_t k = atomicAdd(a.counter, 1u);
        if (a.frame_list == nullptr) return k;
        return k < *a.frame_count ? a.frame_list[k] : a.n_frames;
    };
    if (tid == 0) {
        ctl[1] = claim();
        ctl[6] = spec_policy(ctl[1], window_peek(ctl[1]));
    }
    uint32_t next_f = 0;
    for (;;) {
        pc.mark(4);
        for (int w = tid; w < m_words; w += kDecodeBlock) {
            xsyn[w] = 0;
            xunc[w] = 0;
        }
        __syncthreads();
        const uint32_t f = (uint32_t)__builtin_amdgcn_readfirstlane((int)ctl[1]);
        if (f >= a.n_frames) break;
        if (tid == 0) next_f = claim();
        uint32_t frame_replays = 0;

        const uint64_t* bw = reinterpret_cast<const uint64_t*>(smem + L.tval);
        if (MODE == kModeKeys) {
            uint64_t* w = reinterpret_cast<uint64_t*>(smem + L.tval);
            uint64_t* aw = reinterpret_cast<uint64_t*>(smem + L.aw);
            const bool ka = a.key_ok != nullptr;
            for (int q = tid; q < (int)a.words; q += kDecodeBlock) {
                const uint64_t bv = a.bob_w[(size_t)f * a.words + q];
                const uint64_t av = ka ? a.alice_w[(size_t)f * a.words + q] : 0ull;
                w[q] = bv;
                aw[q] = av;
                if constexpr (MSC || LONG) bwl[q] = bv;
            }
            const uint32_t* sy = a.synw + (size_t)f * 2 * m_words;
            for (int q = tid; q < m_words; q += kDecodeBlock) {
                tsyn[q] = sy[q];
                qsyn[q] = sy[m_words + q];
            }
            __syncthreads();
        }
        const bool spec0 = SPEC == 1 && ctl[6] != 0;
        uint64_t bobmask = 0;
        auto init_slots = [&](bool as_interval) {
            int r = 0;
            for (int i = tid; i < c.n; i += kDecodeBlock, ++r) {
                T l;
                if (MODE == kModeLlr) {
                    l = (T)a.llr[(size_t)f * c.n + c.perm[i]];
                } else {
                    const uint32_t bb = (uint32_t)((bw[i >> 6] >> (i & 63)) & 1u);
                    if (!LONG || r < 64) bobmask |= (uint64_t)bb << r;
                    l = bb ? -llr_p : llr_p;
                }
                if (!fold1) {
                    T sv = l;
                    if constexpr (SPEC) if (as_interval) sv = qkds::pack_iv(qkds::iv_of((double)l));
                    const int deg = c.bit_deg[i];
                    for (int k = 0; k < deg; ++k) ms.st((uint32_t)k * n_pad + i, sv);
                }
            }
            if (tid == 0) ms.st((uint32_t)c.n, (T)0);
        };
        init_slots(spec0);
        auto bob_r = [&](int r) -> uint32_t {
            if constexpr (LONG)
                if (r >= 64) return (uint32_t)(bwl[(r * kDecodeBlock >> 6) + wave] >> lane) & 1u;
            return (uint32_t)(bobmask >> r) & 1u;
        };
        if constexpr (kRunSyn) {
            const int zwords = (int)(n_pad >> 6);
            for (int q = tid; q < zwords; q += kDecodeBlock)
                zw[q] = (MODE == kModeKeys && q < (int)a.words) ? bw[q] : 0ull;
            if (MODE == kModeKeys) {
                for (int w = tid; w < m_words; w += kDecodeBlock)
                    xsyn[w] = tsyn[w] ^ qsyn[w] ^ (lsign ? c.chk_odd[w] : 0u);
            }
        }
        if (MODE == kModeLlr) {
            for (int j0 = wave * 64; j0 < c.m; j0 += kDecodeBlock) {
                const int j = j0 + lane;
                const int sj = j < c.m ? (a.syn[(size_t)f * c.m + j] != 0) : 0;
                const uint64_t sm = __ballot(sj);
                if (lane == 0) {
                    tsyn[j0 >> 5] = (uint32_t)sm;
                    tsyn[(j0 >> 5) + 1] = (uint32_t)(sm >> 32);
                }
            }
        }
        __syncthreads();
        pc.mark(0);
        unsigned long long next_win = 0;
        if (SPEC && tid == 0) next_win = window_peek(next_f);

        bool spec = spec0;
        if (SPEC == 1 && !spec && tid == 0) {
            atomicAdd(a.replay_count, 1u);
            frame_replays++;
        }
        bool done = false;
        uint32_t it = 0;
        uint32_t it_ck = 0;
        uint32_t ck_lim = (CKPT && ctl[6] != 0) ? a.ckpt_unsat : 0u;
        auto ckpt_io = [&](bool save) {
            if constexpr (CKPT) {
                double* bk = a.ckpt + (size_t)blockIdx.x * a.ckpt_stride;
                const uint32_t tot = (uint32_t)c.max_dv * n_pad;
                for (uint32_t x = tid; x < tot; x += kDecodeBlock) {
                    if (save) {
                        const T v = ms.ld(x);
                        bk[x] = v;
                        ms.st(x, qkds::pack_iv(qkds::iv_of(v)));
                    } else {
                        ms.st(x, bk[x]);
                    }
                }
            }
        };
        for (;;) {
            if (it >= a.max_it) break;
            const bool folded = fold1 && it == 0;
            uint32_t* rw = ctl + 4 + (rnd & 1u);
            if (SPEC && spec) {
                if constexpr (SPEC) {
                    if (!folded && fold1 && it == 1) {
                        spec_check_phase_psi<DC>(plan, tsyn, ms, row, wtab, n_tasks, n_pad, dummy_w,
                                                 a.thr_dn, a.thr_up, rw, wave, lane);
                        __syncthreads();
                    } else if (!folded) {
                        spec_check_phase_paired<DC>(plan, tsyn, ms, row, wtab, n_tasks, n_pad, dummy_w, a.thr_dn,
                                                    a.thr_up, rw, wave, lane);
                        __syncthreads();
                    }
                }
            } else if (!folded) {
                if constexpr (MSR) {
                    const int sc_mode = it == 0 ? 0 : (fold1 && it == 1 ? 2 : 1);
                    if (a.ms_offset > 0.0f)
                        ms_split_check_phase<CLAMP, DC, MSC, true>(plan, ms, row, wtab, scw, sc_mode, bwl,
                                                                   (uint32_t)L.msg, n_pad, lsign, n_tasks, (float)thr,
                                                                   a.ms_scale, a.ms_offset, wave, lane);
                    else
                        ms_split_check_phase<CLAMP, DC, MSC, false>(plan, ms, row, wtab, scw, sc_mode, bwl,
                                                                    (uint32_t)L.msg, n_pad, lsign, n_tasks, (float)thr,
                                                                    a.ms_scale, a.ms_offset, wave, lane);
                } else if constexpr (RULE == kRuleSp32)
                    sp32_check_phase<CLAMP, DC>(c.plan_slot, tsyn, ms, row, wtab, n_tasks, n_pad, thr, wave, lane);
                else if (TABLES && it == 1 && tab2_on)
                    split_check_phase<kSrcTable, CLAMP, DC, RULE>(plan, tsyn, tab2, ms, row, n_tasks, n_pad, thr,
                                                                   wave, lane);
                else
                    split_check_phase<kSrcFirst, CLAMP, DC, RULE>(plan, tsyn, tab2, ms, row, n_tasks, n_pad, thr,
                                                                   wave, lane);
                __syncthreads();
            }
            pc.mark((FOLDS && it < 2 && fold1) ? 5 + (int)it : 1);
            const bool keep = it + 1 < a.max_it;
            if (SPEC && spec) {
                if constexpr (SPEC) {
                    if (dv3) {
                        if (folded)
                            spec_bit_phase<true, MODE, true>(c, a, ms, qsyn, ctab, ftab, xsyn, xunc, zw, bobmask, keep,
                                                             f, tid, wave, lane);
                        else
                            spec_bit_phase<false, MODE, true>(c, a, ms, qsyn, ctab, ftab, xsyn, xunc, zw, bobmask, keep,
                                                              f, tid, wave, lane);
                    } else {
                        if (folded)
                            spec_bit_phase<true, MODE, false>(c, a, ms, qsyn, ctab, ftab, xsyn, xunc, zw, bobmask, keep,
                                                              f, tid, wave, lane);
                        else
                            spec_bit_phase<false, MODE, false>(c, a, ms, qsyn, ctab, ftab, xsyn, xunc, zw, bobmask, keep,
                                                               f, tid, wave, lane);
                    }
                }
            } else if (F32 && c.bit_code != nullptr) {
                if constexpr (F32) {
                    if (dv3) {
                        if (folded)
                            sp32_bit_phase<true, MODE, CLAMP, true>(c, a, ms, qsyn, ctab, xsyn, zw, bobmask, keep, f,
                                                                    tid, wave, lane);
                        else
                            sp32_bit_phase<false, MODE, CLAMP, true>(c, a, ms, qsyn, ctab, xsyn, zw, bobmask, keep, f,
                                                                     tid, wave, lane);
                    } else {
                        if (folded)
                            sp32_bit_phase<true, MODE, CLAMP, false>(c, a, ms, qsyn, ctab, xsyn, zw, bobmask, keep, f,
                                                                     tid, wave, lane);
                        else
                            sp32_bit_phase<false, MODE, CLAMP, false>(c, a, ms, qsyn, ctab, xsyn, zw, bobmask, keep,
                                                                      f, tid, wave, lane);
                    }
                }
            } else
            for (int r0 = 0; r0 * kDecodeBlock < c.n; r0 += BC) {
                T v[BC][kDvUnroll];
                int32_t jc[BC][kDvUnroll];
                int dg[BC];
#pragma unroll
                for (int u = 0; u < BC; ++u) {
                    const int i = tid + (r0 + u) * kDecodeBlock;
                    const bool ok = i < c.n;
                    dg[u] = ok ? c.bit_deg[i] : 0;
                    const uint32_t iw = (uint32_t)((r0 + u) * kDecodeBlock + wave * 64);
#pragma unroll
                    for (int k = 0; k < kDvUnroll; ++k) {
                        const bool ld = ok && k < c.max_dv;
                        const uint32_t x = (uint32_t)k * n_pad + i;
                        v[u][k] = folded ? (T)0 : ms.ld_row((uint32_t)k * n_pad + iw, x);
                        jc[u][k] = ld ? c.bit_chk[k * n_pad + i] : 0;
                    }
                }
#pragma unroll
                for (int u = 0; u < BC; ++u) {
                    const int r = r0 + u;
                    if (r * kDecodeBlock >= c.n) break;
                    const int i = tid + r * kDecodeBlock;
                    const uint32_t iw = (uint32_t)(r * kDecodeBlock + wave * 64);
                    const bool ok = i < c.n;
                    const int deg = dg[u];
                    T acc;
                    if (MODE == kModeLlr) acc = ok ? (T)a.llr[(size_t)f * c.n + c.perm[i]] : (T)0;
                    else acc = bob_r(r) ? -llr_p : llr_p;
                    if constexpr (FOLDS) if (folded && ok) {
                        const uint32_t sgi = bob_r(r) ^ lsign;
#pragma unroll
                        for (int k = 0; k < kDvUnroll; ++k) {
                            if (k < deg) {
                                const int j = jc[u][k];
                                const uint32_t sp = (qsyn[j >> 5] >> (j & 31)) & 1u;
                                const T cm = (T)ctab[c.chk_deg[j]];
                                v[u][k] = (sp ^ sgi) ? -cm : cm;
                            }
                        }
                    }
#pragma unroll
                    for (int k = 0; k < kDvUnroll; ++k) acc = k < deg ? acc + v[u][k] : acc;
                    for (int k = kDvUnroll; k < deg; ++k) acc = acc + ms.ld((uint32_t)k * n_pad + i);
                    const bool z = ok && acc <= 0;
                    const uint64_t zb = __ballot(z);
                    const bool flip =
                        kRunSyn ? (ok && z != (((zw[(r * kDecodeBlock >> 6) + wave] >> lane) & 1ull) != 0)) : z;
                    if (lane == 0 && r * kDecodeBlock + wave * 64 < c.n) zw[(r * kDecodeBlock >> 6) + wave] = zb;
                    if (flip) {
#pragma unroll
                        for (int k = 0; k < kDvUnroll; ++k)
                            if (k < deg) atomicXor(&xsyn[jc[u][k] >> 5], 1u << (jc[u][k] & 31));
                        for (int k = kDvUnroll; k < deg; ++k) {
                            const int j = c.bit_chk[k * n_pad + i];
                            atomicXor(&xsyn[j >> 5], 1u << (j & 31));
                        }
                    }
                    if (!keep || !ok) continue;
                    if (TABLES && folded && tab2_on) {
                        uint32_t code = bob_r(r);
#pragma unroll
                        for (int k = 0; k < kTab2MaxDv; ++k)
                            if (k < deg) code |= ((uint32_t)qkdm::hi32(v[u][k]) >> 31) << (1 + k);
                        const uint32_t base = (uint32_t)(c.bit_pat[i] * tab2_stride(c.max_dv)) + code * c.max_dv;
#pragma unroll
                        for (int k = 0; k < kDvUnroll; ++k)
                            if (k < deg)
                                ms.st_row((uint32_t)k * n_pad + iw, (uint32_t)k * n_pad + i,
                                          (T)qkdm::from_bits(base + k));
                    } else {
#pragma unroll
                        for (int k = 0; k < kDvUnroll; ++k) {
                            if (k < deg) {
                                T b = acc - v[u][k];
                                if (CLAMP) b = clamp_msg(b, thr);
                                ms.st_row((uint32_t)k * n_pad + iw, (uint32_t)k * n_pad + i, b);
                            }
                        }
                        for (int k = kDvUnroll; k < deg; ++k) {
                            const uint32_t x = (uint32_t)k * n_pad + i;
                            T b = acc - ms.ld(x);
                            if (CLAMP) b = clamp_msg(b, thr);
                            ms.st(x, b);
                        }
                    }
                }
            }
            __syncthreads();
            pc.mark(2);
            if (tid == 0) {
                ctl[4 + ((rnd + 1) & 1u)] = 0;
                if (CKPT) ctl[2 + ((rnd + 1) & 1u)] = 0;
            }
            bool mismatch = false, uncertain = false;
            uint32_t nbad = 0;
            for (int w = tid; w < m_words; w += kDecodeBlock) {
                const uint32_t u = xunc[w];
                const uint32_t d = (xsyn[w] ^ tsyn[w]) & ~u;
                mismatch |= d != 0;
                if (CKPT) nbad += __builtin_popcount(d);
                uncertain |= u != 0;
                if (!kRunSyn) xsyn[w] = 0;
                xunc[w] = 0;
            }
            const uint32_t wv = __builtin_amdgcn_readfirstlane(
                (uint32_t)(__any(mismatch) ? 1u : 0u) | (uint32_t)(__any(uncertain) ? 4u : 0u));
            if (wv && lane == 0) atomicOr(rw, wv);
            if (CKPT && nbad) atomicAdd(ctl + 2 + (rnd & 1u), nbad);
            __syncthreads();
            const uint32_t fl = *rw;
            const uint32_t unsat = CKPT ? ctl[2 + (rnd & 1u)] : 0u;
            rnd++;
            pc.mark(3);
            if (spec && ((fl & 2u) || ((fl & 4u) && (!(fl & 1u) || it + 1 >= a.max_it)))) {
                spec = false;
                it = it_ck;
                if (CKPT) {
                    ckpt_io(false);
                    __syncthreads();
                    ck_lim >>= 1;
                } else if (!fold1) {
                    init_slots(false);
                    __syncthreads();
                } else if (tid == 0) {
                    ms.st((uint32_t)c.n, (T)0);
                }
                if (tid == 0) {
                    atomicAdd(a.replay_count, 1u);
                    atomicAdd(a.spec_replays, 1ull);
                    frame_replays++;
                }
                continue;
            }
            if (!(fl & 1u)) {
                done = true;
                break;
            }
            ++it;
            if (spec && it >= it_ck + a.spec_cap && it < a.max_it) {
                spec = false;
                it = it_ck;
                if (CKPT) {
                    ckpt_io(false);
                    __syncthreads();
                    ck_lim >>= 1;
                } else if (!fold1) {
                    init_slots(false);
                    __syncthreads();
                } else if (tid == 0) {
                    ms.st((uint32_t)c.n, (T)0);
                }
                if (tid == 0) {
                    atomicAdd(a.replay_count, 1u);
                    atomicAdd(a.spec_replays, 1ull);
                    frame_replays++;
                }
            } else if (CKPT && !spec && it >= 2 && it + 1 < a.max_it && unsat < ck_lim) {
                ckpt_io(true);
                __syncthreads();
                spec = true;
                it_ck = it;
            }
        }

        if (MODE == kModeKeys) {
            if (a.key_ok) {
                const uint64_t* aw = reinterpret_cast<const uint64_t*>(smem + L.aw);
                bool mis = false;
                if (tid < (int)a.words) {
                    uint64_t d = zw[tid] ^ aw[tid];
                    if ((tid + 1) * 64 > c.n) d &= (1ull << (c.n - tid * 64)) - 1ull;
                    mis = d != 0;
                }
                if (__any(mis) && lane == 0) atomicOr(ctl + 7, 1u);
            }
            if (a.bits_out)
                for (int q = tid; q < (int)a.words; q += kDecodeBlock) a.zout[(size_t)f * a.words + q] = zw[q];
        } else if (a.bits_out) {
            for (int i = tid; i < c.n; i += kDecodeBlock)
                a.bits_out[(size_t)f * c.n + c.perm[i]] = (uint8_t)((zw[i >> 6] >> (i & 63)) & 1u);
        }
        if (tid == 0) {
            a.iters[f] = done ? it + 1 : a.max_it;
            a.sp_ok[f] = done ? 1 : 0;
            ctl[1] = next_f;
            if (SPEC) {
                __hip_atomic_fetch_add(win64 + (f >> a.win_shift), ((unsigned long long)frame_replays << 32) | 1ull,
                                       __ATOMIC_RELAXED, __HIP_MEMORY_SCOPE_AGENT);
                ctl[6] = spec_policy(next_f, next_win);
            }
        }
        __syncthreads();
        if (MODE == kModeKeys && a.key_ok && tid == 0) {
            a.key_ok[f] = ctl[7] ? 0 : 1;
            ctl[7] = 0;
        }
    }
    pc.flush();
}

#ifndef QKD_SYN_FRAMES
#define QKD_SYN_FRAMES 4
#endif
constexpr int kSynFrames = QKD_SYN_FRAMES;
constexpr int kSynBlock = 256;
constexpr int kSynRow = 8;
__global__ __launch_bounds__(kSynBlock) void frame_syn_kernel(DeviceCode c, uint64_t* alice_w, uint64_t* bob_w,
                                                              uint32_t words, uint32_t n_frames, uint32_t lsign,
                                                              uint32_t* synw, uint32_t* counter, uint32_t* win,
                                                              uint32_t win_words) {
    extern __shared__ uint2 kw[];
    if (blockIdx.x == 0 && threadIdx.x < 2) counter[threadIdx.x] = 0;
    for (uint32_t i = blockIdx.x * kSynBlock + threadIdx.x; i < win_words; i += gridDim.x * kSynBlock) win[i] = 0;
    const uint32_t w32 = 2 * words;
    const uint32_t f0 = blockIdx.x * kSynFrames;
    const uint32_t nf = min((uint32_t)kSynFrames, n_frames - f0);
    for (uint32_t q = threadIdx.x; q < nf * words; q += kSynBlock) {
        const uint32_t fr = q / words;
        const uint32_t w = q - fr * words;
        const uint64_t av = alice_w[(size_t)(f0 + fr) * words + w];
        const uint64_t bv = bob_w[(size_t)(f0 + fr) * words + w];
        kw[fr * w32 + 2 * w] = make_uint2((uint32_t)av, (uint32_t)bv);
        kw[fr * w32 + 2 * w + 1] = make_uint2((uint32_t)(av >> 32), (uint32_t)(bv >> 32));
    }
    __syncthreads();
    const int m_words = decode_m_words(c.m);
    const int lane = threadIdx.x & 63;
    for (int j0 = (int)(threadIdx.x & ~63u); j0 < c.m; j0 += kSynBlock) {
        const int j = j0 + lane;
        uint32_t pa[kSynFrames], pb[kSynFrames];
#pragma unroll
        for (int fr = 0; fr < kSynFrames; ++fr) pa[fr] = pb[fr] = 0;
        uint32_t deg = 0;
        auto take = [&](int bit) {
            if (bit < 0) return;
            deg++;
            const uint32_t wi = (uint32_t)bit >> 5, sh = (uint32_t)bit & 31u;
#pragma unroll
            for (int fr = 0; fr < kSynFrames; ++fr) {
                const uint2 v = kw[fr * w32 + wi];
                pa[fr] ^= v.x >> sh;
                pb[fr] ^= v.y >> sh;
            }
        };
        if (j < c.m) {
            int bits[kSynRow];
#pragma unroll
            for (int k = 0; k < kSynRow; ++k) bits[k] = k < c.max_dc ? c.chk_bits[k * c.m_pad + j] : -1;
#pragma unroll
            for (int k = 0; k < kSynRow; ++k) take(bits[k]);
            for (int k = kSynRow; k < c.max_dc; ++k) take(c.chk_bits[k * c.m_pad + j]);
        }
#pragma unroll
        for (int fr = 0; fr < kSynFrames; ++fr) {
            const uint64_t sm = __ballot(pa[fr] & 1u);
            const uint64_t qm = __ballot((pa[fr] ^ pb[fr] ^ (lsign & deg)) & 1u);
            if (lane == 0 && (uint32_t)fr < nf) {
                uint32_t* o = synw + (size_t)(f0 + fr) * 2 * m_words;
                o[j0 >> 5] = (uint32_t)sm;
                o[(j0 >> 5) + 1] = (uint32_t)(sm >> 32);
                o[m_words + (j0 >> 5)] = (uint32_t)qm;
                o[m_words + (j0 >> 5) + 1] = (uint32_t)(qm >> 32);
            }
        }
    }
    constexpr uint32_t kSynPermBatch = 8;
    constexpr uint32_t NWS = kSynBlock / 64;
    for (uint32_t w0 = (threadIdx.x >> 6) * kSynPermBatch; w0 < words; w0 += NWS * kSynPermBatch) {
        uint32_t ob[kSynPermBatch];
#pragma unroll
        for (uint32_t u = 0; u < kSynPermBatch; ++u) {
            const uint32_t q = (w0 + u) * 64 + (uint32_t)lane;
            ob[u] = q < (uint32_t)c.n ? (uint32_t)c.perm[q] : 0xffffffffu;
        }
#pragma unroll
        for (int fr = 0; fr < kSynFrames; ++fr) {
            uint64_t mya = 0, myb = 0;
#pragma unroll
            for (uint32_t u = 0; u < kSynPermBatch; ++u) {
                const bool in = ob[u] != 0xffffffffu;
                const uint32_t o = in ? ob[u] : 0u;
                const uint2 v = kw[fr * w32 + (o >> 5)];
                const uint64_t am = __ballot(in && ((v.x >> (o & 31u)) & 1u));
                const uint64_t bm = __ballot(in && ((v.y >> (o & 31u)) & 1u));
                if ((uint32_t)lane == u) {
                    mya = am;
                    myb = bm;
                }
            }
            const uint32_t w = w0 + (uint32_t)lane;
            if ((uint32_t)lane < kSynPermBatch && w < words && (uint32_t)fr < nf) {
                alice_w[(size_t)(f0 + fr) * words + w] = mya;
                bob_w[(size_t)(f0 + fr) * words + w] = myb;
            }
        }
    }
}

__global__ void zout_unpack_kernel(const uint64_t* zout, const int32_t* inv, uint32_t n, uint32_t words,
                                   uint32_t n_frames, uint8_t* out) {
    const size_t gid = (size_t)blockIdx.x * blockDim.x + threadIdx.x;
    if (gid >= (size_t)n_frames * n) return;
    const size_t f = gid / n;
    const uint32_t q = (uint32_t)inv[gid - f * n];
    out[gid] = (uint8_t)((zout[f * words + (q >> 6)] >> (q & 63)) & 1u);
}

constexpr int kSlicedFrames = 16;
constexpr int kSlicedBlock = 1024;
constexpr int kSlicedPre = 8;
template <int S, uint32_t MASK>
__device__ __forceinline__ uint32_t transpose_stage(uint32_t x, uint32_t lane) {
    const uint32_t y = (uint32_t)__builtin_amdgcn_ds_swizzle((int)x, 0x1F | (S << 10));
    const bool hi = (lane & (uint32_t)S) != 0;
    const uint32_t ys = __builtin_amdgcn_alignbit(y, y, hi ? (uint32_t)S : 32u - (uint32_t)S);
    const uint32_t k = hi ? ~MASK : MASK;
    return (x & k) | (ys & ~k);
}
__device__ __forceinline__ uint32_t wave_transpose32(uint32_t x, uint32_t lane) {
    x = transpose_stage<16, 0x0000FFFFu>(x, lane);
    x = transpose_stage<8, 0x00FF00FFu>(x, lane);
    x = transpose_stage<4, 0x0F0F0F0Fu>(x, lane);
    x = transpose_stage<2, 0x33333333u>(x, lane);
    return transpose_stage<1, 0x55555555u>(x, lane);
}
template <bool BYTES>
__global__ __launch_bounds__(kSlicedBlock) void frame_syn_sliced_kernel(DeviceCode c, uint64_t* alice_w,
                                                                        uint64_t* bob_w, uint32_t words,
                                                                        uint32_t n_frames, uint32_t lsign,
                                                                        uint32_t* synw, uint32_t* counter,
                                                                        uint32_t* win, uint32_t win_words,
                                                                        const uint8_t* alice_b,
                                                                        const uint8_t* bob_b) {
    extern __shared__ uint32_t T[];
    const uint32_t tid = threadIdx.x, lane = tid & 63u;
    const uint32_t wave = (uint32_t)__builtin_amdgcn_readfirstlane((int)(tid >> 6));
    constexpr uint32_t NW = kSlicedBlock / 64;
    if (blockIdx.x == 0 && tid < 2) counter[tid] = 0;
    for (uint32_t i = blockIdx.x * kSlicedBlock + tid; i < win_words; i += gridDim.x * kSlicedBlock) win[i] = 0;
    const uint32_t f0 = blockIdx.x * kSlicedFrames;
    const uint32_t nf = min((uint32_t)kSlicedFrames, n_frames - f0);
    const uint32_t fr = lane & 15u;
    const bool bob_lane = (lane & 16u) != 0;
    const uint32_t half = lane >> 5;
    const uint32_t pairs = (words + 1) / 2;
    auto load_pair = [&](uint32_t p) -> uint64_t {
        const uint32_t w = 2 * p + half;
// ... 204 lines not shown
```

### qkd_ldpc_amd/csrc/host.cpp

```cpp
#include <algorithm>
#include <cerrno>
#include <cmath>
#include <cstdio>
#include <cstdlib>
#include <cstring>
#include <fstream>
#include <map>
#include <new>
#include <sstream>

#include "qkd_internal.h"
#include "qkd_plan.h"
#include "qkd_rng.h"

namespace qkd {

static thread_local std::string g_last_error;

qkd_status set_error(qkd_status s, const char* fmt, ...) {
    char buf[1024];
    va_list ap;
    va_start(ap, fmt);
    vsnprintf(buf, sizeof buf, fmt, ap);
    va_end(ap);
    g_last_error = buf;
    return s;
}

void clear_error() { g_last_error.clear(); }

static const char* const kDebugOptions[] = {
    "QKD_SPEC_CAP", "QKD_SPEC_CKPT", "QKD_CKPT_UNSAT", "QKD_SPEC_POLICY", "QKD_FOLD_TABLE",
    "QKD_DECODE_KERNEL", "QKD_MINSUM_STORE", "QKD_DECODE_GRID", "QKD_SPLIT_BUDGET", "QKD_C2B_PAD",
    "QKD_ILV", "QKD_ILV_GRID", "QKD_KEYGEN", "QKD_SYN_SLICED", "QKD_SYN_BYTES", "QKD_BIT_ORDER",
    "QKD_PHASE_TIMING"};
static std::mutex g_dbg_mu;
static std::map<std::string, std::string> g_dbg;

DbgOpt debug_option(const qkd_workspace* ws, const char* name) {
    std::lock_guard<std::mutex> lock(g_dbg_mu);
    DbgOpt o;
    if (ws) {
        const auto it = ws->dbg.find(name);
        if (it != ws->dbg.end()) {
            o.set = true;
            o.v = it->second;
            return o;
        }
    }
    const auto it = g_dbg.find(name);
    if (it != g_dbg.end()) {
        o.set = true;
        o.v = it->second;
    }
    return o;
}

static int32_t round_up(int32_t x, int32_t a) { return (x + a - 1) / a * a; }

static void free_device(qkd_code* c) {
    if (!c) return;
    DeviceGuard g(c->device);
    if (c->d_chk_bits) (void)hipFree(c->d_chk_bits);
    if (c->d_chk_deg) (void)hipFree(c->d_chk_deg);
    if (c->d_bit_chk) (void)hipFree(c->d_bit_chk);
    if (c->d_bit_pos) (void)hipFree(c->d_bit_pos);
    c->d_bit_pos = nullptr;
    if (c->d_bit_deg) (void)hipFree(c->d_bit_deg);
    if (c->d_bit_pat) (void)hipFree(c->d_bit_pat);
    if (c->d_bit_code) (void)hipFree(c->d_bit_code);
    c->d_bit_code = nullptr;
    if (c->d_pat_deg) (void)hipFree(c->d_pat_deg);
    for (void* p : {(void*)c->d_perm, (void*)c->d_inv, (void*)c->d_bit_chk_s, (void*)c->d_bit_deg_s,
                    (void*)c->d_bit_pat_s, (void*)c->d_chk_rows16, (void*)c->d_ilv_slots, (void*)c->d_chk_odd})
        if (p) (void)hipFree(p);
    c->d_chk_odd = nullptr;
    c->d_chk_rows16 = nullptr;
    c->chk_rs = 0;
    c->d_ilv_slots = nullptr;
    c->ilv_rs = 0;
    c->d_perm = c->d_inv = c->d_bit_chk_s = nullptr;
    c->d_bit_deg_s = nullptr;
    c->d_bit_pat_s = nullptr;
    c->d_bit_pat = nullptr;
    c->d_pat_deg = nullptr;
    if (c->d_plan) (void)hipFree(c->d_plan);
    c->d_plan = nullptr;
    if (c->d_plan_slot) (void)hipFree(c->d_plan_slot);
    c->d_plan_slot = nullptr;
    for (auto& kv : c->d_plan_enc) (void)hipFree(kv.second);
    c->d_plan_enc.clear();
    if (c->d_jump) (void)hipFree(c->d_jump);
    c->d_jump = nullptr;
    if (c->d_jpoly) (void)hipFree(c->d_jpoly);
    c->d_jpoly = nullptr;
    if (c->d_jpoly2) (void)hipFree(c->d_jpoly2);
    c->d_jpoly2 = nullptr;
    c->d_chk_bits = nullptr;
    c->d_chk_deg = nullptr;
    c->d_bit_chk = nullptr;
    c->d_bit_deg = nullptr;
}

static void bank_balance_runs(int32_t n, int32_t n_pad, const std::vector<int32_t>& bdeg,
                              const qkdp::WavePlan& plan, std::vector<int32_t>& perm, std::vector<int32_t>& inv) {
    const int32_t n_tasks = plan.n_tasks;
    std::vector<std::vector<int32_t>> tasks_of(n);
    std::vector<std::vector<int32_t>> runs(n_tasks);
    for (int32_t t = 0; t < n_tasks; ++t)
        for (int l = 0; l < 64; ++l) {
            const uint32_t w = plan.word[(size_t)t * 64 + l];
            const uint32_t b = w & qkdp::kPlanBitMask;
            if (b >= (uint32_t)n) continue;
            if ((int32_t)(w >> 24) == bdeg[b] - 1) runs[t].push_back((int32_t)b);
            if (tasks_of[b].empty() || tasks_of[b].back() != t) tasks_of[b].push_back(t);
        }
    auto cost = [&](int32_t t) {
        int ex = 0;
        for (int h = 0; h < 2; ++h) {
            int cnt[32] = {0};
            for (int l = h * 32; l < h * 32 + 32; ++l) {
                const uint32_t w = plan.word[(size_t)t * 64 + l];
                const uint32_t b = w & qkdp::kPlanBitMask;
                const int32_t row = (int32_t)(w >> 24);
                if (b >= (uint32_t)n || row == bdeg[b] - 1) continue;
                cnt[((uint32_t)row * (uint32_t)n_pad + (uint32_t)inv[b]) & 31u]++;
            }
            int mx = 0;
            for (int k = 0; k < 32; ++k) mx = std::max(mx, cnt[k]);
            ex += mx > 0 ? mx - 1 : 0;
        }
        return ex;
    };
    std::vector<int> cur(n_tasks);
    for (int32_t t = 0; t < n_tasks; ++t) cur[t] = cost(t);
    uint64_t rng = 0x9e3779b97f4a7c15ull;
    auto next = [&]() {
        rng ^= rng << 13;
        rng ^= rng >> 7;
        rng ^= rng << 17;
        return rng;
    };
    const int64_t iters = std::min<int64_t>(200000, (int64_t)20 * n);
    std::vector<int32_t> aff;
    std::vector<int> nc;
    for (int64_t it = 0; it < iters; ++it) {
        const auto& run = runs[next() % (uint64_t)n_tasks];
        if (run.size() < 2) continue;
        const int32_t a = run[next() % run.size()], b = run[next() % run.size()];
        if (a == b) continue;
        aff.clear();
        for (int32_t t : tasks_of[a]) aff.push_back(t);
        for (int32_t t : tasks_of[b]) aff.push_back(t);
        std::sort(aff.begin(), aff.end());
        aff.erase(std::unique(aff.begin(), aff.end()), aff.end());
        int before = 0;
        for (int32_t t : aff) before += cur[t];
        std::swap(inv[a], inv[b]);
        int after = 0;
        nc.resize(aff.size());
        for (size_t k = 0; k < aff.size(); ++k) after += nc[k] = cost(aff[k]);
        if (after <= before) {
            for (size_t k = 0; k < aff.size(); ++k) cur[aff[k]] = nc[k];
        } else {
            std::swap(inv[a], inv[b]);
        }
    }
    for (int32_t i = 0; i < n; ++i) perm[inv[i]] = i;
}

static void internal_bit_order(int32_t n, int32_t n_pad, const std::vector<int32_t>& bdeg,
                               const qkdp::WavePlan& plan, std::vector<int32_t>& perm, std::vector<int32_t>& inv,
                               const char* mode) {
    int32_t nx = 0;
    for (size_t k = 0; k < (size_t)plan.n_tasks * 64; ++k) {
        const uint32_t b = plan.word[k] & qkdp::kPlanBitMask;
        if (b < (uint32_t)n && (int32_t)(plan.word[k] >> 24) == bdeg[b] - 1 && inv[b] < 0) {
            inv[b] = nx;
            perm[nx++] = (int32_t)b;
        }
    }
    for (int32_t i = 0; i < n; ++i)
        if (inv[i] < 0) {
            inv[i] = nx;
            perm[nx++] = i;
        }
    if (mode && !strcmp(mode, "identity")) {
        for (int32_t i = 0; i < n; ++i) perm[i] = inv[i] = i;
// ... 80 lines not shown
            const int32_t bk = fill[b] - c->bit_ptr[b];
            c->bit_idx[fill[b]++] = j;
            bit_chk[(size_t)bk * c->n_pad + b] = j;
            bit_pos[(size_t)bk * c->n_pad + b] = (uint8_t)slot;
            krow[k] = bk;
        }
    }
    qkdp::WavePlan plan;
    if (!qkdp::build_wave_plan(n, m, cptr, cidx, krow.data(), plan))
        return set_error(QKD_ERR_UNSUPPORTED, "check degree outside [1, %d]", qkdp::kPlanMaxDegree);
    c->n_tasks = plan.n_tasks;
    std::vector<uint16_t> bit_pat(n, 0);
    c->n_pat = 0;
    c->pat_deg.clear();
    if (max_dv <= kTab2MaxDv) {
        std::map<std::vector<uint8_t>, int> ids;
        for (int32_t i = 0; i < n; ++i) {
            std::vector<uint8_t> key(max_dv, 0);
            for (int32_t k = c->bit_ptr[i]; k < c->bit_ptr[i + 1]; ++k) {
                const int32_t j = c->bit_idx[k];
                key[k - c->bit_ptr[i]] = (uint8_t)(cptr[j + 1] - cptr[j]);
            }
            auto it = ids.find(key);
            if (it == ids.end()) {
                it = ids.emplace(key, (int)ids.size()).first;
                c->pat_deg.insert(c->pat_deg.end(), key.begin(), key.end());
            }
            bit_pat[i] = (uint16_t)it->second;
        }
        c->n_pat = (int32_t)ids.size();
        if ((size_t)c->n_pat * tab2_stride(max_dv) > (size_t)kTab2MaxEntries) {
            c->n_pat = 0;
            c->pat_deg.clear();
        }
    }
    bool reg = true;
    for (int32_t i = 0; i < n; ++i) {
        bit_deg[i] = (uint8_t)bdeg[i];
        reg = reg && bdeg[i] == bdeg[0];
    }
    for (int32_t j = 0; j < m; ++j) reg = reg && chk_deg[j] == chk_deg[0];
    c->is_regular = reg ? 1 : 0;

    int ndev = 0;
    if (hipGetDeviceCount(&ndev) != hipSuccess || ndev <= 0)
        return set_error(QKD_ERR_DEVICE, "no HIP device available");
    if (device < 0 || device >= ndev)
        return set_error(QKD_ERR_INVALID_ARG, "device %d out of range (%d devices)", device, ndev);
    DeviceGuard g(device);
    QKD_HIP(hipDeviceGetAttribute(&c->cu_count, hipDeviceAttributeMultiprocessorCount, device));
    QKD_HIP(hipMalloc(&c->d_chk_bits, chk_bits.size() * sizeof(int32_t)));
    QKD_HIP(hipMalloc(&c->d_chk_deg, chk_deg.size()));
    QKD_HIP(hipMalloc(&c->d_bit_chk, bit_chk.size() * sizeof(int32_t)));
    QKD_HIP(hipMalloc(&c->d_bit_deg, bit_deg.size()));
    QKD_HIP(hipMemcpy(c->d_chk_bits, chk_bits.data(), chk_bits.size() * sizeof(int32_t),
                      hipMemcpyHostToDevice));
    QKD_HIP(hipMemcpy(c->d_chk_deg, chk_deg.data(), chk_deg.size(), hipMemcpyHostToDevice));
    {
        std::vector<uint32_t> odd((size_t)((m + 63) / 64) * 2, 0u);
        for (int32_t j = 0; j < m; ++j)
            if (chk_deg[j] & 1u) odd[j >> 5] |= 1u << (j & 31);
        QKD_HIP(hipMalloc(&c->d_chk_odd, odd.size() * sizeof(uint32_t)));
        QKD_HIP(hipMemcpy(c->d_chk_odd, odd.data(), odd.size() * sizeof(uint32_t), hipMemcpyHostToDevice));
    }
    QKD_HIP(hipMalloc(&c->d_bit_pos, bit_pos.size()));
    QKD_HIP(hipMemcpy(c->d_bit_pos, bit_pos.data(), bit_pos.size(), hipMemcpyHostToDevice));
    QKD_HIP(hipMemcpy(c->d_bit_chk, bit_chk.data(), bit_chk.size() * sizeof(int32_t),
                      hipMemcpyHostToDevice));
    QKD_HIP(hipMemcpy(c->d_bit_deg, bit_deg.data(), bit_deg.size(), hipMemcpyHostToDevice));
    if (c->n_pat > 0) {
        QKD_HIP(hipMalloc(&c->d_bit_pat, bit_pat.size() * sizeof(uint16_t)));
        QKD_HIP(hipMalloc(&c->d_pat_deg, c->pat_deg.size()));
        QKD_HIP(hipMemcpy(c->d_bit_pat, bit_pat.data(), bit_pat.size() * sizeof(uint16_t),
                          hipMemcpyHostToDevice));
        QKD_HIP(hipMemcpy(c->d_pat_deg, c->pat_deg.data(), c->pat_deg.size(), hipMemcpyHostToDevice));
    }
    const bool split = n <= kMaxBitsSplitLong && m <= kMaxChecksSplit;
    std::vector<int32_t> perm(n), inv(n, -1);
    if (split) {
    const DbgOpt bit_order = debug_option(nullptr, "QKD_BIT_ORDER");
    internal_bit_order(n, c->n_pad, bdeg, plan, perm, inv, bit_order ? bit_order.c_str() : nullptr);
    std::vector<int32_t> bit_chk_s(bit_chk.size(), -1);
    std::vector<uint8_t> bit_deg_s(n, 0);
    for (int32_t q = 0; q < n; ++q) {
        const int32_t b = perm[q];
        bit_deg_s[q] = bit_deg[b];
        for (int32_t k = 0; k < max_dv; ++k)
            bit_chk_s[(size_t)k * c->n_pad + q] = bit_chk[(size_t)k * c->n_pad + b];
    }
    QKD_HIP(hipMalloc(&c->d_perm, (size_t)n * sizeof(int32_t)));
    QKD_HIP(hipMemcpy(c->d_perm, perm.data(), (size_t)n * sizeof(int32_t), hipMemcpyHostToDevice));
    QKD_HIP(hipMalloc(&c->d_inv, (size_t)n * sizeof(int32_t)));
    QKD_HIP(hipMemcpy(c->d_inv, inv.data(), (size_t)n * sizeof(int32_t), hipMemcpyHostToDevice));
    if (n < 65535 && max_dc <= 16) {
        const int32_t rs = max_dc <= 8 ? 8 : 16;
        std::vector<uint16_t> rows((size_t)m * rs, 0xffff);
        for (int32_t j = 0; j < m; ++j)
            for (int32_t k = 0; k < chk_deg[j]; ++k) rows[(size_t)j * rs + k] = (uint16_t)chk_bits[(size_t)k * c->m_pad + j];
        QKD_HIP(hipMalloc(&c->d_chk_rows16, rows.size() * sizeof(uint16_t)));
        QKD_HIP(hipMemcpy(c->d_chk_rows16, rows.data(), rows.size() * sizeof(uint16_t), hipMemcpyHostToDevice));
        c->chk_rs = rs;
    }
    QKD_HIP(hipMalloc(&c->d_bit_chk_s, bit_chk_s.size() * sizeof(int32_t)));
    QKD_HIP(hipMemcpy(c->d_bit_chk_s, bit_chk_s.data(), bit_chk_s.size() * sizeof(int32_t), hipMemcpyHostToDevice));
    QKD_HIP(hipMalloc(&c->d_bit_deg_s, bit_deg_s.size()));
    QKD_HIP(hipMemcpy(c->d_bit_deg_s, bit_deg_s.data(), bit_deg_s.size(), hipMemcpyHostToDevice));
    if (c->n_pat > 0) {
        std::vector<uint16_t> bit_pat_s((size_t)round_up(n, kDecodeBlock) + kBitPadRounds * kDecodeBlock, 0);
        for (int32_t q = 0; q < n; ++q) bit_pat_s[q] = bit_pat[perm[q]];
        QKD_HIP(hipMalloc(&c->d_bit_pat_s, bit_pat_s.size() * sizeof(uint16_t)));
        QKD_HIP(hipMemcpy(c->d_bit_pat_s, bit_pat_s.data(), bit_pat_s.size() * sizeof(uint16_t),
                          hipMemcpyHostToDevice));
    }
    bool packable = m <= 65536 && max_dv <= 3;
    for (int32_t j = 0; j < m && packable; ++j) packable = chk_deg[j] >= 1 && chk_deg[j] <= 16;
    const size_t rounds_pad = std::max((size_t)c->n_pad, (size_t)round_up(n, kDecodeBlock)) +
                              (size_t)kBitPadRounds * kDecodeBlock;
    if (packable) {
        std::vector<uint64_t> code(rounds_pad, 0);
        for (int32_t q = 0; q < n; ++q) {
            const int32_t i = perm[q];
            uint64_t w = (uint64_t)bdeg[i] << 48;
            for (int32_t k = 0; k < bdeg[i]; ++k) {
                const int32_t j = bit_chk[(size_t)k * c->n_pad + i];
                w |= (uint64_t)j << (16 * k);
                w |= (uint64_t)(chk_deg[j] - 1) << (50 + 4 * k);
            }
            code[q] = w;
        }
        QKD_HIP(hipMalloc(&c->d_bit_code, code.size() * sizeof(uint64_t)));
        QKD_HIP(hipMemcpy(c->d_bit_code, code.data(), code.size() * sizeof(uint64_t), hipMemcpyHostToDevice));
        const int32_t rs = max_dc <= 8 ? 8 : 16;
        std::vector<uint32_t> lines((size_t)m * rs, 0xffffffffu);
        for (int32_t j = 0; j < m; ++j)
            for (int32_t k = cptr[j]; k < cptr[j + 1]; ++k)
                lines[(size_t)j * rs + (k - cptr[j])] = (uint32_t)krow[k] * (uint32_t)c->n_pad + (uint32_t)inv[cidx[k]];
        QKD_HIP(hipMalloc(&c->d_ilv_slots, lines.size() * sizeof(uint32_t)));
        QKD_HIP(hipMemcpy(c->d_ilv_slots, lines.data(), lines.size() * sizeof(uint32_t), hipMemcpyHostToDevice));
        c->ilv_rs = rs;
    }
    }
    std::vector<uint2> plan2(plan.word.size());
    for (size_t k = 0; k < plan.word.size(); ++k) plan2[k] = make_uint2(plan.word[k], plan.seg[k]);
    QKD_HIP(hipMalloc(&c->d_plan, plan2.size() * sizeof(uint2)));
    QKD_HIP(hipMemcpy(c->d_plan, plan2.data(), plan2.size() * sizeof(uint2), hipMemcpyHostToDevice));
    if (split) {
        for (size_t k = 0; k < plan.word.size(); ++k) {
            const uint32_t b = plan.word[k] & qkdp::kPlanBitMask;
            plan2[k].x = (plan.word[k] >> 24) * (uint32_t)c->n_pad + (b < (uint32_t)n ? (uint32_t)inv[b] : b);
        }
        QKD_HIP(hipMalloc(&c->d_plan_slot, plan2.size() * sizeof(uint2)));
        QKD_HIP(hipMemcpy(c->d_plan_slot, plan2.data(), plan2.size() * sizeof(uint2), hipMemcpyHostToDevice));
        c->plan_slot_host = std::move(plan2);
    }
    const uint64_t draws = qkdr::trial_draws((uint32_t)n);
    const uint64_t per_lane = (draws + kKeygenLanes - 1) / kKeygenLanes;
    c->keygen_chunk = (uint32_t)((per_lane + 63) / 64 * 64);
    std::vector<uint64_t> jump((size_t)kKeygenLevels * 256 * 4);
    qkdr::xoshiro_jump_matrices(c->keygen_chunk, kKeygenLevels, jump.data());
    QKD_HIP(hipMalloc(&c->d_jump, jump.size() * sizeof(uint64_t)));
    QKD_HIP(hipMemcpy(c->d_jump, jump.data(), jump.size() * sizeof(uint64_t), hipMemcpyHostToDevice));
    std::vector<uint64_t> jp((size_t)kKeygenLanes * 4);
    if (!qkdr::xoshiro_jump_polys(c->keygen_chunk, kKeygenLanes, jp.data()))
        return set_error(QKD_ERR_DEVICE, "xoshiro256 characteristic polynomial: unexpected degree");
    QKD_HIP(hipMalloc(&c->d_jpoly, jp.size() * sizeof(uint64_t)));
    QKD_HIP(hipMemcpy(c->d_jpoly, jp.data(), jp.size() * sizeof(uint64_t), hipMemcpyHostToDevice));
    {
        uint64_t P[4];
        if (!qkdr::xoshiro_charpoly(P))
            return set_error(QKD_ERR_DEVICE, "xoshiro256 characteristic polynomial: unexpected degree");
        const uint32_t kl = kKgSplitLanes;
        c->kg_cb = (uint32_t)(((n + kl - 1) / kl + 31) / 32 * 32);
        c->kg_cs = (uint32_t)((draws - (uint64_t)n + kl - 1) / kl);
        std::vector<uint64_t> jp2((size_t)2 * kl * 4);
        for (uint32_t l = 0; l < kl; ++l) {
            qkdr::poly_x_pow((uint64_t)l * c->kg_cb, P, &jp2[(size_t)l * 4]);
            qkdr::poly_x_pow((uint64_t)n + (uint64_t)l * c->kg_cs, P, &jp2[(size_t)(kl + l) * 4]);
        }
        QKD_HIP(hipMalloc(&c->d_jpoly2, jp2.size() * sizeof(uint64_t)));
        QKD_HIP(hipMemcpy(c->d_jpoly2, jp2.data(), jp2.size() * sizeof(uint64_t), hipMemcpyHostToDevice));
    }
    return QKD_OK;
}

static qkd_code* make_code(int32_t n, int32_t m, const int32_t* cptr, const int32_t* cidx,
                           int device, qkd_status* status) {
    qkd_code* c = new (std::nothrow) qkd_code();
    qkd_status s = c ? build_code(c, n, m, cptr, cidx, device)
                     : set_error(QKD_ERR_OUT_OF_MEMORY, "out of host memory");
    if (s != QKD_OK) {
        free_device(c);
        delete c;
        c = nullptr;
    }
    if (status) *status = s;
    return c;
}


static void parse_ints(const std::string& line, std::vector<long>& out) {
    out.clear();
    const char* s = line.c_str();
    for (;;) {
        while (*s == ' ' || *s == '\t' || *s == '\r' || *s == '\v' || *s == '\f' || *s == '\n') s++;
        if (!*s) break;
        char* end = nullptr;
        errno = 0;
        long v = strtol(s, &end, 10);
        if (end == s || errno == ERANGE || v > INT32_MAX || v < INT32_MIN) break;
        out.push_back(v);
        s = end;
    }
}

static bool read_lines(const char* path, std::vector<std::vector<long>>& rows) {
    std::ifstream f(path);
    if (!f.is_open()) return false;
    std::string line;
    std::vector<long> v;
    while (std::getline(f, line)) {
        parse_ints(line, v);
        rows.push_back(v);
    }
    return true;
}

static qkd_status parse_alist(const char* path, int32_t& n, int32_t& m, std::vector<int32_t>& cptr,
                              std::vector<int32_t>& cidx, bool sort_rows) {
    std::vector<std::vector<long>> v;
    if (!path || !read_lines(path, v))
        return set_error(QKD_ERR_IO, "Failed to open file: %s", path ? path : "(null)");
    if (v.empty()) return set_error(QKD_ERR_IO, "File is empty or cannot be read properly: %s", path);
    if (v.size() < 4) return set_error(QKD_ERR_IO, "Insufficient data in the file: %s", path);
    if (v[0].size() != 2 || v[1].size() != 2)
        return set_error(QKD_ERR_IO, "File format does not match the alist format: %s", path);
    const long cols = v[0][0], rows = v[0][1];
    const size_t nb = v[2].size(), nc = v[3].size();
    if (v.size() < 4 + nb + nc) return set_error(QKD_ERR_IO, "Insufficient data in the file: %s", path);
    if (cols != (long)nb)
        return set_error(QKD_ERR_IO, "Number of columns '%ld' is not the same as the length of the third line '%zu'. File: %s", cols, nb, path);
    if (rows != (long)nc)
        return set_error(QKD_ERR_IO, "Number of rows '%ld' is not the same as the length of the fourth line '%zu'. File: %s", rows, nc, path);
    for (size_t i = 0; i < nb + nc; ++i) {
        const auto& L = v[4 + i];
        const long w = i < nb ? v[2][i] : v[3][i - nb];
        long nz = 0;
        for (long x : L) nz += (x != 0);
        if (nz != w || w < 0 || (size_t)w > L.size())
            return set_error(QKD_ERR_IO, "Number of non-zero elements '%ld' in the line '%zu' does not match the weight '%ld'. File: %s", nz, 5 + i, w, path);
    }
    n = (int32_t)cols;
    m = (int32_t)rows;
    cptr.assign(m + 1, 0);
    cidx.clear();
    for (int32_t j = 0; j < m; ++j) {
        const auto& L = v[4 + nb + j];
        for (long k = 0; k < v[3][j]; ++k) cidx.push_back((int32_t)(L[k] - 1));
        if (sort_rows) std::sort(cidx.begin() + cptr[j], cidx.end());
        cptr[j + 1] = (int32_t)cidx.size();
    }
    std::vector<std::vector<int32_t>> from_checks(n);
    for (int32_t j = 0; j < m; ++j)
        for (int32_t k = cptr[j]; k < cptr[j + 1]; ++k) {
            const int32_t b = cidx[k];
            if (b < 0 || b >= n)
                return set_error(QKD_ERR_BAD_CODE, "check %d lists bit %d outside [1,%d]. File: %s", j + 1, b + 1, n, path);
            from_checks[b].push_back(j);
        }
    for (int32_t i = 0; i < n; ++i) {
        const auto& L = v[4 + i];
        std::vector<int32_t> row;
        for (long k = 0; k < v[2][i]; ++k) row.push_back((int32_t)(L[k] - 1));
        if (sort_rows) std::sort(row.begin(), row.end());
        if (row != from_checks[i]) {
            std::vector<int32_t> s = row;
            std::sort(s.begin(), s.end());
            if (s == from_checks[i])
                return set_error(QKD_ERR_UNSORTED, "bit %d: check list not ascending. File: %s", i + 1, path);
            return set_error(QKD_ERR_BAD_CODE, "bit %d: check list disagrees with the check rows. File: %s", i + 1, path);
        }
    }
    return QKD_OK;
}

static qkd_status parse_dense(const char* path, int32_t& n, int32_t& m, std::vector<int32_t>& cptr,
                              std::vector<int32_t>& cidx) {
    std::vector<std::vector<long>> v;
    if (!path || !read_lines(path, v))
        return set_error(QKD_ERR_IO, "Failed to open file: %s", path ? path : "(null)");
    if (v.empty()) return set_error(QKD_ERR_IO, "File is empty or cannot be read properly: %s", path);
    for (const auto& r : v)
        for (long x : r)
            if (x != 0 && x != 1)
                return set_error(QKD_ERR_IO, "Parity check matrix can only take values 0 or 1. File: %s", path);
    for (const auto& r : v)
        if (r.size() != v[0].size())
            return set_error(QKD_ERR_IO, "Different lengths of rows in a matrix. File: %s", path);
    n = (int32_t)v[0].size();
    m = (int32_t)v.size();
    for (int32_t i = 0; i < n; ++i) {
        long w = 0;
        for (int32_t j = 0; j < m; ++j) w += v[j][i];
        if (w <= 0)
            return set_error(QKD_ERR_IO, "Column '%d' weight cannot be equal to or less than zero. File: %s", i + 1, path);
    }
    cptr.assign(m + 1, 0);
// ... 166 lines not shown
```

### qkd_ldpc_amd/csrc/qkd_decode.h

```cpp
#pragma once
#include <hip/hip_runtime.h>

#include "qkd_internal.h"
#include "qkd_math.h"
#include "qkd_plan.h"
#include "qkd_spec.h"

namespace qkd {


constexpr int kSpecCapDefault = 8;
constexpr int kCkptUnsatDefault = 128;
constexpr double kSpecCkptSwitch = 1.0 / 16.0;
constexpr double kSpecReplayMax = 1.0 / 6.0;
constexpr uint32_t kSpecWinShift = 8;
constexpr uint32_t kSpecWinLag = 8;
constexpr uint64_t kSpecStatEvery = 64;

constexpr int kFirstTableDeg = 16;


enum DecodeMode : int {
    kModeLlr = 0,
    kModeKeys = 1
};

enum DecodeRule : int {
    kRuleSp64 = 0, kRuleSp32 = 1, kRuleMinSum = 2, kRuleMinSumLds = 3, kRuleMinSumLdsSc = 4,
    kRuleMinSumSplit = 5, kRuleMinSumSplitSc = 6
};
template <int RULE> struct RuleMsg { using T = float; };
template <> struct RuleMsg<kRuleSp64> { using T = double; };

struct DecodeArgs {
    DeviceCode code;
    uint32_t n_frames;
    uint32_t max_it;
    double thr;
    int clamp_on;
    float ms_scale;
    float ms_offset;
    int ms_sc;
    const double* llr;
    const uint8_t* syn;
    const uint64_t* alice_w;
    const uint64_t* bob_w;
    const uint8_t* alice_b;
    const uint8_t* bob_b;
    uint32_t words;
    double log_p;
    int first_table;
    double first_c2b[kFirstTableDeg + 1];
    int tab2_entries;
    int ftab_entries;
    uint8_t* bits_out;
    uint32_t* iters;
    uint8_t* sp_ok;
    uint8_t* key_ok;
    double* c2b;
    size_t c2b_stride;
    uint32_t* counter;
    unsigned long long* phase;
    double* trace;
    size_t trace_stride;
    double* totals;
    size_t totals_stride;
    uint32_t lds_budget;
    const uint2* plan_enc;
    const uint32_t* synw;
    uint64_t* zout;
    uint32_t spec_cap;
    float lp_dn, lp_up, thr_dn, thr_up;
    float pinf;
    unsigned long long* spec_replays;
    uint32_t* replay_count;
    uint32_t spec_always;
    uint32_t* win;
    uint32_t win_count;
    uint32_t win_shift;
    uint32_t win_lag;
    double* ckpt;
    uint32_t ckpt_stride;
    uint32_t ckpt_unsat;
    double* ilv_store;
    size_t ilv_stride;
    uint32_t* fb_list;
    uint32_t* fb_count;
    const uint32_t* frame_list;
    const uint32_t* frame_count;
};

constexpr int kIlvCols = 16;
constexpr int kIlvCtlWords = 64;
#ifndef QKD_ILV_BLOCK
#define QKD_ILV_BLOCK 1024
#endif
constexpr int kIlvBlock = QKD_ILV_BLOCK;
constexpr int kRingStage = 16;
struct IlvLds {
    size_t tsyn, xsyn, xunc, ctl, ctab, ring, bytes;
    __host__ __device__ IlvLds(int m, bool tsyn_global, bool xunc_global = false) {
        const size_t mw2 = (size_t)(m + 1) / 2;
        const size_t k = tsyn_global ? 0 : 1;
        const size_t u = xunc_global ? 0 : 1;
        tsyn = 0;
        xsyn = k * mw2 * 4;
        xunc = (k + 1) * mw2 * 4;
        ctl = ((k + 1 + u) * mw2 * 4 + 15) & ~(size_t)15;
        ctab = ctl + (size_t)kIlvCtlWords * 4;
        ring = ctab + (size_t)(kFirstTableDeg + 1) * 8;
        bytes = ring + (size_t)(kIlvBlock / kIlvCols) * 4 * kRingStage * 4;
    }
};

struct PhaseClock {
    unsigned long long* out;
    long long t = 0;
    __device__ explicit PhaseClock(unsigned long long* o) : out(threadIdx.x == 0 ? o : nullptr) {
        if (out) t = clock64();
    }
    __device__ __forceinline__ void mark(int k) {
        if (out) {
            const long long n = clock64();
            atomicAdd(out + k, (unsigned long long)(n - t));
            t = n;
        }
    }
    __device__ void flush() {}
};

template <typename T>
__device__ __forceinline__ T clamp_msg(T v, T thr) {
    return v > thr ? thr : (v < -thr ? -thr : v);
}

__device__ __forceinline__ bool block_any(bool p, uint32_t* flags, uint32_t& k) {
    uint32_t* f = flags + (k & 1u);
    const bool wave_hit = __any(p);
    if (wave_hit && (threadIdx.x & 63) == 0) atomicOr(f, 1u);
    __syncthreads();
    const bool r = *f != 0;
    if (threadIdx.x == 0) flags[(k + 1) & 1u] = 0;
    k++;
    return r;
}


__host__ __device__ inline int decode_m_words(int m) { return ((m + 63) / 64) * 2; }

struct DecodeLds {
    size_t tsyn, xsyn, qsyn, tval, ctab, tab2, t2idx, ctl, cst, czf, bytes;
    __host__ __device__ DecodeLds(int n_pad, int n_words, int m, int dc, int tab2_entries, int total_esz,
                                  int cst_checks = 0, int row_esz = 0, bool zf = false) {
        const int m_words = decode_m_words(m);
        const int esz = row_esz ? row_esz : total_esz;
        tsyn = ((size_t)n_pad * total_esz + 15) & ~(size_t)15;
        xsyn = tsyn + (size_t)m_words * 4;
        qsyn = xsyn + (size_t)m_words * 4;
        tval = (qsyn + (size_t)m_words * 4 + 15) & ~(size_t)15;
        const size_t rows = (size_t)(kDecodeBlock / 64) * (64 + dc) * esz;
        const size_t stage = (size_t)n_words * 16;
        ctab = (tval + (rows > stage ? rows : stage) + 15) & ~(size_t)15;
        tab2 = ctab + (size_t)(kFirstTableDeg + 1) * 8;
        t2idx = tab2 + (size_t)tab2_entries * 8;
        ctl = (t2idx + (tab2_entries ? (size_t)n_pad * 2 : 0) + 15) & ~(size_t)15;
        cst = ctl + 16;
        czf = cst + (size_t)cst_checks * 16;
        bytes = czf + (zf ? (size_t)cst_checks * 4 : 0);
    }
};

constexpr int kDvUnroll = 3;
constexpr int kFoldTabPat = (2 << kDvUnroll) * (kDvUnroll + 1);
constexpr int kBitChunk = 5;
#ifndef QKD_SPEC_EXACT_CHUNK
#define QKD_SPEC_EXACT_CHUNK 2
#endif
constexpr int kBitChunkSpec = QKD_SPEC_EXACT_CHUNK;
static_assert(kTab2MaxDv <= kDvUnroll, "tables need every row of their bits unrolled");
constexpr int kPlanGroup = 4;

__device__ __forceinline__ uint32_t pw_bit(uint2 p) { return p.x & qkdp::kPlanBitMask; }
__device__ __forceinline__ uint32_t pw_slot(uint2 p) { return p.x; }
__device__ __forceinline__ uint32_t pw_row(uint2 p) { return p.x >> 24; }
__device__ __forceinline__ uint32_t pw_chk(uint2 p) { return p.y & qkdp::kPlanChkMask; }
__device__ __forceinline__ int pw_start(uint2 p) { return (int)((p.y >> 20) & 63u); }
__device__ __forceinline__ int pw_deg(uint2 p) { return (int)(p.y >> 26) + 1; }
__device__ __forceinline__ int seg_parity(uint64_t ballot, uint2 w) {
    const uint64_t sh = ballot >> pw_start(w);
    const int deg = pw_deg(w);
    if (deg < 32) return __popc(__builtin_amdgcn_ubfe((uint32_t)sh, 0, (uint32_t)deg)) & 1;
    const uint64_t m = deg == 64 ? ~0ull : ((1ull << deg) - 1ull);
    return __popcll(sh & m) & 1;
}
__device__ __forceinline__ int seg_parity32(uint64_t ballot, uint2 w) {
    const uint32_t sh = (uint32_t)(ballot >> pw_start(w));
    return __popc(__builtin_amdgcn_ubfe(sh, 0, (uint32_t)pw_deg(w))) & 1;
}

enum CheckSrc : int {
    kSrcGeneral = 0,
    kSrcFirst = 1,
    kSrcTable = 2
};

template <int RULE> struct RuleMath;
template <> struct RuleMath<kRuleSp64> {
    static __device__ __forceinline__ double tanh_half(double x) { return qkdm::tanh_flat(x / 2.0); }
    static __device__ __forceinline__ double two_atanh(double p) { return 2.0 * qkdm::atanh_flat(p); }
};
namespace sp32m {
template <bool PSI>
__device__ __forceinline__ float phi(float x, float u) {
    float t = __builtin_fmaf(x, 1.0f / 6.0f, -0.5f);
    t = __builtin_fmaf(x, t, 1.0f);
    const float w = x < 0.03125f ? x * t : 1.0f - u;
    const float lg = __builtin_amdgcn_logf((2.0f - w) * __builtin_amdgcn_rcpf(w));
    const float vlo = PSI ? lg : qkds::kLn2 * lg;
    const float s = u * u;
    float h = __builtin_fmaf(s, 0.2f, 1.0f / 3.0f);
    h = __builtin_fmaf(s, h, 1.0f);
// ... 27 lines not shown
        const float lg1 = __builtin_amdgcn_logf(arg.y);
        const f2 vlo = f2{__builtin_amdgcn_logf(arg.x), qkds::kLn2 * lg1};
        const f2 sq = u * u;
        f2 h = __builtin_elementwise_fma(sq, f2(0.2f), f2(1.0f / 3.0f));
        h = __builtin_elementwise_fma(sq, h, f2(1.0f));
        const f2 vhi = (u * f2{2.0f * qkds::kInvLn2, 2.0f}) * h;
        return f2{xx.x < 2.0f ? vlo.x : vhi.x, xx.y < 2.0f ? vlo.y : vhi.y};
    }
};

template <typename T>
__device__ __forceinline__ void msg_store(T* p, T v) {
    *p = v;
}

__device__ __forceinline__ void wave_lds_sync() {
    __builtin_amdgcn_fence(__ATOMIC_RELEASE, "wavefront");
    __builtin_amdgcn_wave_barrier();
    __builtin_amdgcn_fence(__ATOMIC_ACQUIRE, "wavefront");
}

template <int SRC, bool CLAMP, int RULE, typename T>
__device__ __forceinline__ T edge_in(T x, T old, T thr) {
    if (SRC == kSrcGeneral) {
        x = x - old;
        if (CLAMP) x = clamp_msg(x, thr);
    }
    if constexpr (RULE == kRuleMinSum) return x;
    else return SRC == kSrcTable ? x : RuleMath<RULE>::tanh_half(x);
}

template <bool CLAMP, int DC, int RULE, typename T>
__device__ __forceinline__ T edge_out(T tv, uint2 w, uint32_t sbit, int lane, T thr, const T* row,
                                      float ms_scale, float ms_offset = 0.0f) {
    const int start = pw_start(w);
    const int deg = pw_deg(w);
    T o[DC];
#pragma unroll
    for (int k = 0; k < DC; ++k) o[k] = row[start + k];
    T v;
    if constexpr (RULE == kRuleMinSum) {
        uint32_t neg = sbit ^ (tv < 0 ? 1u : 0u);
        T mn = __builtin_inff();
#pragma unroll
        for (int k = 0; k < DC; ++k) {
            if (k < deg) {
                neg ^= o[k] < 0 ? 1u : 0u;
                if (start + k != lane) mn = fminf(mn, fabsf(o[k]));
            }
        }
        v = (T)ms_scale * mn;
        if (ms_offset > 0.0f) v = fmaxf(v - (T)ms_offset, (T)0);
        v = neg ? -v : v;
    } else if constexpr (RULE == kRuleSp64) {
        T P = sbit ? (T)-1 : (T)1;
        P = P * o[0];
#pragma unroll
        for (int k = 1; k < DC; ++k) P = k < deg ? P * o[k] : P;
        v = RuleMath<RULE>::two_atanh(P / tv);
    } else {
        T S = (T)0;
        uint32_t neg = sbit;
#pragma unroll
        for (int k = 0; k < DC; ++k) {
            if (k < deg && start + k != lane) {
                S = S + __builtin_fabsf(o[k]);
                neg ^= o[k] < (T)0 ? 1u : 0u;
            }
        }
        v = RuleMath<RULE>::two_atanh(S);
        v = neg ? -v : v;
    }
    if (CLAMP) v = clamp_msg(v, thr);
    return v;
}

template <bool CLAMP>
__device__ void second_table_fill(const DeviceCode& c, const double* ctab, double log_p, double thr,
                                  double* tab2, int entries) {
    const int dvm = c.max_dv;
    const int stride = tab2_stride(dvm);
    for (int e = threadIdx.x; e < entries; e += kDecodeBlock) {
        const int p = e / stride;
        const int r = e - p * stride;
        const int code = r / dvm;
        const int k = r - code * dvm;
        const uint8_t* degs = c.pat_deg + p * dvm;
        double total = (code & 1) ? -log_p : log_p;
        double ck = 0.0;
        int dv = 0;
        for (int m = 0; m < dvm; ++m) {
            if (degs[m] == 0) break;
            const double cm = ctab[degs[m]];
            const double v = ((code >> (1 + m)) & 1) ? -cm : cm;
            total = total + v;
            if (m == k) ck = v;
            dv = m + 1;
        }
        double y = 0.0;
        if (k < dv) {
            double b = total - ck;
            if (CLAMP) b = clamp_msg(b, thr);
            y = qkdm::tanh_flat(b / 2.0);
        }
        tab2[e] = y;
    }
    __syncthreads();
}

__host__ __device__ inline int seg_weight_entries(int dc) { return dc <= 8 ? 9 * 8 * dc : 0; }

struct SplitLds {
    size_t tsyn, xsyn, qsyn, xunc, zw, aw, tval, ctab, tab2, ftab, ctl, wtab, msg, bytes;
    uint32_t S;
    __host__ __device__ SplitLds(int n_pad, int n_words, int m, int max_dv, int dc, int tab2_entries,
                                 int ftab_entries, int esz, size_t budget) {
        const int m_words = decode_m_words(m);
        tsyn = 0;
        qsyn = tsyn + (size_t)m_words * 4;
        xsyn = qsyn + (size_t)m_words * 4;
        xunc = xsyn + (size_t)m_words * 4;
        zw = (xunc + (size_t)m_words * 4 + 15) & ~(size_t)15;
        aw = (zw + (size_t)(n_pad / 64) * 8 + 15) & ~(size_t)15;
        tval = (aw + (size_t)n_words * 8 + 15) & ~(size_t)15;
        const size_t rows = (size_t)(kDecodeBlock / 64) * (64 + dc) * esz;
        const size_t stage = (size_t)n_words * 8;
        ctab = (tval + (rows > stage ? rows : stage) + 15) & ~(size_t)15;
        tab2 = ctab + (size_t)(kFirstTableDeg + 1) * 8;
        ftab = (tab2 + (size_t)tab2_entries * 8 + 15) & ~(size_t)15;
        ctl = (ftab + (size_t)ftab_entries * 8 + 15) & ~(size_t)15;
        wtab = ctl + 48;
        msg = (wtab + (size_t)seg_weight_entries(dc) * 4 + 15) & ~(size_t)15;
        const size_t slots = (size_t)max_dv * n_pad;
        const size_t fit = budget > msg + 64 * (size_t)esz ? (budget - msg) / (size_t)esz - 64 : 0;
        S = (uint32_t)(slots < fit ? slots : fit) & ~63u;
        bytes = msg + ((size_t)S + 64) * esz;
    }
};

constexpr uint32_t kSlotLds = 0x80000000u;
constexpr uint32_t kSlotGlobalBase = 0x40000u;
__host__ __device__ inline uint32_t encode_slot(uint32_t x, uint32_t S, uint32_t msg, uint32_t esz) {
    return x < S ? (kSlotLds | (msg + x * esz)) : (kSlotGlobalBase + (x - S) * esz);
}

constexpr uint32_t kSegStartShift = 5, kSegWiShift = 11, kSegWordShift = 19;
__host__ __device__ inline uint32_t encode_seg(uint32_t j, uint32_t start, uint32_t deg, uint32_t lane, uint32_t dc) {
    const uint32_t p = lane - start;
    const uint32_t pc = p < dc - 1 ? p : dc - 1;
    const uint32_t wi = dc <= 8 ? deg * 8 + pc : dc <= 16 ? (deg - 1) * dc + pc : deg - 1;
    return (j & 31u) | (start << kSegStartShift) | (wi << kSegWiShift) | (((j >> 5) * 4u) << kSegWordShift);
}

using DecodeFn = void (*)(DecodeArgs);
DecodeFn pick_split_decode(int mode, int rule, bool clamp, int max_dc, int* dc);
DecodeFn pick_split_long(bool clamp, int max_dc, int* dc);
DecodeFn pick_split_spec(int mode, int max_dc, bool ckpt, int* dc);
DecodeFn pick_ilv(int rs, int max_dc, bool tsyn_global, bool xunc_global = false);
hipError_t launch_frame_syn(const DecodeArgs& a, hipStream_t stream, bool gather = false, bool pack_first = false);
hipError_t launch_pack_keys(const DecodeArgs& a, hipStream_t stream);
hipError_t launch_key_match(const DecodeArgs& a, hipStream_t stream);

}
```

### qkd_ldpc_amd/csrc/qkd_internal.h

```cpp
#pragma once
#include <hip/hip_runtime.h>

#include <cstdarg>
#include <cstdint>
#include <cstdlib>
#include <map>
#include <mutex>
#include <string>
#include <vector>

#include "../../include/qkd_ldpc.h"

namespace qkd {

#ifndef QKD_DECODE_BLOCK
#define QKD_DECODE_BLOCK 1024
#endif
constexpr int kDecodeBlock = QKD_DECODE_BLOCK;
constexpr int kTab2MaxDv = 3;
constexpr int kTab2MaxEntries = 2048;
constexpr int kFoldTabMaxEntries = 1024;
constexpr size_t kC2bPad = 64;
constexpr int kBitPadRounds = 4;
__host__ __device__ inline int tab2_stride(int max_dv) { return (1 << (1 + max_dv)) * max_dv; }

constexpr int kMaxCheckDegree = 64;
constexpr int kMaxBitsLds = 20480;
constexpr int kMaxBitsSplit = 64 * kDecodeBlock;
constexpr int kMaxBitsSplitLong = 128 * kDecodeBlock;
constexpr int32_t kMaxChecksSplit = 65536;
#ifndef QKD_KEYGEN_LEVELS
#define QKD_KEYGEN_LEVELS 6
#endif
constexpr int kKeygenLevels = QKD_KEYGEN_LEVELS;
constexpr int kKeygenLanes = 1 << kKeygenLevels;
constexpr int kKeygenBlock = kKeygenLanes < 64 ? 64 : kKeygenLanes;
constexpr int kKeygenFrames = kKeygenBlock / kKeygenLanes;
constexpr uint32_t kKeygenFastMaxErrors = 4096;
#ifndef QKD_KG_SPLIT_LANES
#define QKD_KG_SPLIT_LANES 64
#endif
constexpr uint32_t kKgSplitLanes = QKD_KG_SPLIT_LANES;
#ifndef QKD_KG_PAIRS
#define QKD_KG_PAIRS 1
#endif
constexpr uint32_t kKgPairs = QKD_KG_PAIRS;
constexpr uint32_t kKgBlock = 128 * kKgPairs;
constexpr uint32_t kKgSplitFrames = kKgPairs * (64 / kKgSplitLanes);
static_assert(kKgSplitLanes >= 1 && 64 % kKgSplitLanes == 0, "lanes per frame divide a wave");

struct DeviceCode {
    int32_t n, m, e;
    int32_t n_pad, m_pad;
    int32_t max_dv, max_dc, min_dc;
    int32_t min_dv;
    int32_t n_tasks;
    const int32_t* chk_bits;
    const uint8_t* chk_deg;
    const uint2* plan;
    const int32_t* bit_chk;
    const uint8_t* bit_pos;
    const uint8_t* bit_deg;
    int32_t n_pat;
    const uint16_t* bit_pat;
    const uint8_t* pat_deg;
    const uint64_t* bit_code;
    const uint2* plan_slot;
    const int32_t* perm;
    const int32_t* inv;
    const uint16_t* chk_rows16;
    int32_t chk_rs;
    const uint32_t* ilv_slots;
    int32_t ilv_rs;
    const uint32_t* chk_odd;
};

}

struct SpecClean {
    int clean = 0;
    uint64_t skip = 0;
};

struct qkd_workspace {
    const qkd_code* code = nullptr;
    int device = 0;
    std::mutex mu;
    std::map<std::string, std::string> dbg;
    double* c2b = nullptr;
    size_t c2b_slots = 0;
    uint32_t* counter = nullptr;
    uint64_t* alice_w = nullptr;
    uint64_t* bob_w = nullptr;
    size_t key_frames = 0;
    uint32_t* synw = nullptr;
    uint64_t* zout = nullptr;
    uint32_t* low = nullptr;
    size_t low_words = 0;
    hipEvent_t done = nullptr;
    uint32_t* spec_stat_host = nullptr;
    hipEvent_t spec_stat_ev = nullptr;
    bool spec_stat_pending = false;
    double spec_stat_q = 0.0;
    size_t spec_stat_frames = 0;
    double spec_ckpt_q = 2.0;
    std::map<double, SpecClean> spec_clean;
    double* ckpt = nullptr;
    size_t ckpt_slots = 0;
    uint32_t* win = nullptr;
    size_t win_words = 0;
    double* ilv = nullptr;
    size_t ilv_elems = 0;
    uint32_t* fb_list = nullptr;
    size_t fb_frames = 0;
    bool time_decoder = false;
    std::vector<hipEvent_t> dec_ev;
    size_t dec_ev_used = 0;
    double dec_ms_folded = 0.0;
    uint64_t dec_pairs_folded = 0;
};

struct qkd_code {
    int device = 0;
    int32_t n = 0, m = 0, e = 0;
    int32_t max_dv = 0, max_dc = 0, min_dc = 0, min_dv = 0, is_regular = 0;
    int32_t n_pad = 0, m_pad = 0;
    int32_t n_tasks = 0;
    std::vector<int32_t> check_ptr, check_idx, bit_ptr, bit_idx;
    int32_t* d_chk_bits = nullptr;
    uint8_t* d_chk_deg = nullptr;
    int32_t* d_bit_chk = nullptr;
    uint8_t* d_bit_pos = nullptr;
    uint8_t* d_bit_deg = nullptr;
    uint2* d_plan = nullptr;
    uint2* d_plan_slot = nullptr;
    std::vector<uint2> plan_slot_host;
    mutable std::map<std::pair<uint32_t, uint32_t>, uint2*> d_plan_enc;
    mutable std::mutex plan_mu;
    int32_t n_pat = 0;
    std::vector<uint8_t> pat_deg;
    uint16_t* d_bit_pat = nullptr;
    uint64_t* d_bit_code = nullptr;
    uint8_t* d_pat_deg = nullptr;
    int32_t* d_perm = nullptr;
    int32_t* d_inv = nullptr;
    uint16_t* d_chk_rows16 = nullptr;
    int32_t chk_rs = 0;
    uint32_t* d_ilv_slots = nullptr;
    int32_t ilv_rs = 0;
    uint32_t* d_chk_odd = nullptr;
    int32_t* d_bit_chk_s = nullptr;
    uint8_t* d_bit_deg_s = nullptr;
    uint16_t* d_bit_pat_s = nullptr;
    uint32_t keygen_chunk = 0;
    uint64_t* d_jump = nullptr;
    uint64_t* d_jpoly = nullptr;
    uint32_t kg_cb = 0, kg_cs = 0;
    uint64_t* d_jpoly2 = nullptr;
    int cu_count = 0;
    qkd_workspace* default_ws = nullptr;

    qkd::DeviceCode view() const {
        return qkd::DeviceCode{n, m, e, n_pad, m_pad, max_dv, max_dc, min_dc, min_dv, n_tasks,
                               d_chk_bits, d_chk_deg, d_plan, d_bit_chk, d_bit_pos, d_bit_deg,
                               n_pat, d_bit_pat, d_pat_deg, nullptr, nullptr, nullptr, nullptr,
                               nullptr, 0, nullptr, 0, d_chk_odd};
    }
    qkd::DeviceCode view_split() const {
        return qkd::DeviceCode{n, m, e, n_pad, m_pad, max_dv, max_dc, min_dc, min_dv, n_tasks,
                               d_chk_bits, d_chk_deg, d_plan, d_bit_chk_s, nullptr, d_bit_deg_s,
                               n_pat, d_bit_pat_s, d_pat_deg, d_bit_code, d_plan_slot, d_perm, d_inv,
                               d_chk_rows16, chk_rs, d_ilv_slots, ilv_rs, d_chk_odd};
    }
};

namespace qkd {

qkd_status set_error(qkd_status s, const char* fmt, ...);
void clear_error();

struct DbgOpt {
    bool set = false;
    std::string v;
    explicit operator bool() const { return set; }
    const char* c_str() const { return v.c_str(); }
    int as_int() const { return atoi(v.c_str()); }
    long as_long() const { return atol(v.c_str()); }
    bool is(const char* s) const { return set && v == s; }
};
DbgOpt debug_option(const qkd_workspace* ws, const char* name);

struct DeviceGuard {
    int prev = -1;
    explicit DeviceGuard(int dev) {
        if (hipGetDevice(&prev) != hipSuccess) prev = -1;
        if (prev != dev) (void)hipSetDevice(dev);
    }
    ~DeviceGuard() {
        int cur = -1;
        if (prev >= 0 && hipGetDevice(&cur) == hipSuccess && cur != prev) (void)hipSetDevice(prev);
    }
};

#define QKD_HIP(call)                                                                     \
    do {                                                                                  \
        hipError_t e_ = (call);                                                           \
        if (e_ != hipSuccess)                                                             \
            return ::qkd::set_error(QKD_ERR_DEVICE, "%s failed: %s (%s:%d)", #call,       \
                                    hipGetErrorString(e_), __FILE__, __LINE__);           \
    } while (0)

qkd_status ws_reserve_decode(qkd_workspace* ws, size_t slots);
qkd_status ws_reserve_keys(qkd_workspace* ws, size_t frames, size_t low_words);
qkd_workspace* resolve_ws(const qkd_code* code, qkd_workspace* ws);

}
```

### qkd_ldpc_amd/csrc/qkd_plan.h

```cpp
#pragma once
#include <stdint.h>

#include <algorithm>
#include <vector>

namespace qkdp {

constexpr uint32_t kPlanBitMask = 0xFFFFFFu;
constexpr uint32_t kPlanChkMask = 0xFFFFFu;
constexpr int kPlanMaxBits = (int)kPlanBitMask;
constexpr int kPlanMaxChecks = (int)kPlanChkMask + 1;
constexpr int kPlanPadTasks = 128;
constexpr int kPlanMaxDegree = 64;
constexpr int kPlanMaxBitDegree = 32;

inline uint32_t plan_word(uint32_t bit, uint32_t krow) { return bit | (krow << 24); }
inline uint32_t plan_seg(uint32_t chk, uint32_t start, uint32_t deg) {
    return chk | (start << 20) | ((deg - 1) << 26);
}

struct WavePlan {
    int32_t n_tasks = 0;
    std::vector<uint32_t> word;
    std::vector<uint32_t> seg;
    std::vector<int32_t> chk;
    std::vector<int32_t> slot_of_edge;
};

inline bool build_wave_plan(int32_t n, int32_t m, const int32_t* cptr, const int32_t* cidx,
                            const int32_t* krow, WavePlan& p) {
    const uint32_t idle = plan_word((uint32_t)n, 0);
    const uint32_t idle_seg = plan_seg(0, 0, 1);
    std::vector<std::vector<int32_t>> by_deg(kPlanMaxDegree + 1);
    for (int32_t j = 0; j < m; ++j) {
        const int32_t d = cptr[j + 1] - cptr[j];
        if (d < 1 || d > kPlanMaxDegree) return false;
        by_deg[d].push_back(j);
    }
    std::vector<int> degs;
    for (int d = kPlanMaxDegree; d >= 1; --d)
        if (!by_deg[d].empty()) degs.push_back(d);
    std::vector<size_t> next(kPlanMaxDegree + 1, 0);
    const int nc = (int)degs.size();
    const int cap = 64;
    p.word.clear();
    p.seg.clear();
    p.chk.clear();
    p.slot_of_edge.assign(cptr[m], -1);
    int32_t left = m;
    std::vector<std::vector<int8_t>> reach(nc + 1, std::vector<int8_t>(cap + 1, 0));
    std::vector<std::vector<int8_t>> take(nc + 1, std::vector<int8_t>(cap + 1, 0));
    while (left > 0) {
        for (auto& r : reach) std::fill(r.begin(), r.end(), 0);
        reach[0][0] = 1;
        for (int i = 0; i < nc; ++i) {
            const int d = degs[i];
            const int avail = (int)(by_deg[d].size() - next[d]);
            for (int c = cap; c >= 0; --c) {
                if (!reach[i][c]) continue;
                for (int x = std::min(avail, (cap - c) / d); x >= 0; --x) {
                    const int c2 = c + x * d;
                    if (!reach[i + 1][c2]) {
                        reach[i + 1][c2] = 1;
                        take[i + 1][c2] = (int8_t)x;
                    }
                }
            }
        }
        int best = cap;
        while (best > 0 && !reach[nc][best]) --best;
        std::vector<int> cnt(nc, 0);
        for (int i = nc, c = best; i > 0; --i) {
            cnt[i - 1] = take[i][c];
            c -= cnt[i - 1] * degs[i - 1];
        }
        const int32_t task = p.n_tasks++;
        p.word.resize((size_t)p.n_tasks * 64, idle);
        p.seg.resize((size_t)p.n_tasks * 64, idle_seg);
        p.chk.resize((size_t)p.n_tasks * 64, -1);
        int lane = 0;
        for (int i = 0; i < nc; ++i) {
            const int d = degs[i];
            for (int x = 0; x < cnt[i]; ++x) {
                const int32_t j = by_deg[d][next[d]++];
                --left;
                for (int k = 0; k < d; ++k) {
                    const size_t slot = (size_t)task * 64 + lane + k;
                    p.word[slot] = plan_word((uint32_t)cidx[cptr[j] + k], (uint32_t)krow[cptr[j] + k]);
                    p.seg[slot] = plan_seg((uint32_t)j, (uint32_t)lane, (uint32_t)d);
                    p.chk[slot] = j;
                    p.slot_of_edge[cptr[j] + k] = (int32_t)slot;
                }
                lane += d;
            }
        }
        for (int l = lane; l < 64; ++l) p.seg[(size_t)task * 64 + l] = plan_seg(0, (uint32_t)l, 1);
    }
    p.word.resize((size_t)(p.n_tasks + kPlanPadTasks) * 64, idle);
    p.seg.resize((size_t)(p.n_tasks + kPlanPadTasks) * 64, idle_seg);
    p.chk.resize((size_t)(p.n_tasks + kPlanPadTasks) * 64, -1);
    return true;
}

}
```

Baseline: 33.92 billion bit/s.

## Add one-check-per-lane check phase for speculative sum-product decode

Adds a check-node phase layout where each lane owns a whole check (degree padded to 4 or 6), with a host-built plan that places most checks in lane-per-check tasks. The few leftover checks keep the existing packed wave plan, which is appended after the main plan. The goal is to avoid the segmented intra-wave reductions and plan-word decoding of the edge-per-lane layout, and to prefetch the next task's words during compute. It also reads kernel arguments through the kernarg segment pointer to reduce register pressure. The cost is padding lanes for low-degree checks and a more complex plan encoding.

```diff
diff --git a/include/qkd_ldpc.h b/include/qkd_ldpc.h
--- a/include/qkd_ldpc.h
+++ b/include/qkd_ldpc.h
@@ -126,6 +126,7 @@
 QKD_API qkd_status qkd_debug_phase_cycles(qkd_workspace *ws, uint64_t *cycles7);
 QKD_API qkd_status qkd_debug_decoder_timing(qkd_workspace *ws, int start, double *ms_total, uint64_t *launches);
 QKD_API qkd_status qkd_debug_spec_replays(qkd_workspace *ws, uint64_t *replays, int reset);
+QKD_API qkd_status qkd_debug_check_lanes(qkd_workspace *ws, int32_t *form, int32_t *lane_tasks, int32_t *edge_tasks);
 QKD_API qkd_status qkd_trace_decode(const qkd_code *code, const double *llr, const uint8_t *syndrome,
                                     uint32_t max_iterations, double msg_threshold, uint32_t flags,
                                     double *c2b_trace, double *total_trace, uint32_t *iterations,
diff --git a/qkd_ldpc_amd/__init__.py b/qkd_ldpc_amd/__init__.py
--- a/qkd_ldpc_amd/__init__.py
+++ b/qkd_ldpc_amd/__init__.py
@@ -18,7 +18,7 @@
     "sum_product_decoding_irregular", "sum_product_decoding_regular", "qkd_ldpc",
     "QKD_LDPC_irregular", "QKD_LDPC_regular", "keygen", "run_trials", "make_seeds",
     "qber_range", "Workspace", "counters_to_stats", "decoder_flags", "trace_decode", "set_debug_option",
-    "spec_replays", "interactive_simulation",
+    "spec_replays", "check_lanes", "interactive_simulation",
 ]
 
 
@@ -201,6 +201,12 @@
     v = C.c_uint64(0)
     N.check(N.lib().qkd_debug_spec_replays(ws.handle, C.byref(v), int(reset)))
     return int(v.value)
+
+
+def check_lanes(ws: Workspace):
+    v = [C.c_int32(0) for _ in range(3)]
+    N.check(N.lib().qkd_debug_check_lanes(ws.handle, *[C.byref(x) for x in v]))
+    return tuple(int(x.value) for x in v)
 
 
 def calculate_syndrome(H: HMatrix, bits, stream=None):
diff --git a/qkd_ldpc_amd/_native.py b/qkd_ldpc_amd/_native.py
--- a/qkd_ldpc_amd/_native.py
+++ b/qkd_ldpc_amd/_native.py
@@ -47,7 +47,7 @@
     "qkd_qber_range", "qkd_debug_phase_cycles", "qkd_debug_spec_replays", "qkd_debug_math", "qkd_debug_phi_sweep", "qkd_trace_decode",
     "qkd_interactive_batch",
     "qkd_code_from_alist_ex", "qkd_debug_decoder_timing", "qkd_debug_bit_order",
-    "qkd_counters_merge", "qkd_debug_set_option",
+    "qkd_counters_merge", "qkd_debug_set_option", "qkd_debug_check_lanes",
 ]
 
 
@@ -111,6 +111,7 @@
             "qkd_debug_phase_cycles": (st, [P, P]),
             "qkd_debug_decoder_timing": (st, [P, C.c_int, C.POINTER(D), C.POINTER(U64)]),
             "qkd_debug_spec_replays": (st, [P, P, C.c_int]),
+            "qkd_debug_check_lanes": (st, [P, C.POINTER(I32), C.POINTER(I32), C.POINTER(I32)]),
             "qkd_debug_math": (st, [C.c_int, P, P, SZ, P]),
             "qkd_debug_phi_sweep": (st, [C.c_int, C.c_uint32, C.c_uint32, P]),
             "qkd_debug_bit_order": (st, [I32, I32, P, P, C.c_char_p, P, P, C.POINTER(I32)]),
diff --git a/qkd_ldpc_amd/csrc/decode.hip b/qkd_ldpc_amd/csrc/decode.hip
--- a/qkd_ldpc_amd/csrc/decode.hip
+++ b/qkd_ldpc_amd/csrc/decode.hip
@@ -1280,9 +1280,10 @@
     return r;
 }
 
-static qkd_status plan_for_layout(const qkd_code* c, const SplitLds& L, int dc, const uint2** out, int esz = 8) {
+static qkd_status plan_for_layout(const qkd_code* c, const SplitLds& L, int dc, const uint2** out, int esz = 8,
+                                  int cl_form = 0) {
     std::lock_guard<std::mutex> lock(c->plan_mu);
-    const auto key = std::make_pair(L.S, ((uint32_t)L.msg << 8) | (uint32_t)dc | (esz == 4 ? 0x80u : 0u));
+    const auto key = std::make_pair(L.S, ((uint32_t)cl_form << 28) | ((uint32_t)L.msg << 8) | (uint32_t)dc | (esz == 4 ? 0x80u : 0u));
     auto it = c->d_plan_enc.find(key);
     if (it == c->d_plan_enc.end()) {
         std::vector<uint2> enc(c->plan_slot_host);
@@ -1291,6 +1292,27 @@
             w.x = esz == 4 ? (uint32_t)L.msg + w.x * 4u : encode_slot(w.x, L.S, (uint32_t)L.msg, (uint32_t)sizeof(double));
             w.y = encode_seg(w.y & qkdp::kPlanChkMask, (w.y >> 20) & 63u, (w.y >> 26) + 1, (uint32_t)(k & 63),
                              (uint32_t)dc);
+        }
+        if (cl_form != 0) {
+            const qkd_code::ClHost& h = c->cl_host[cl_form - 1];
+            const size_t at = enc.size();
+            enc.insert(enc.end(), h.rem.begin(), h.rem.end());
+            for (size_t k = at; k < enc.size(); ++k) {
+                uint2& w = enc[k];
+                w.x = encode_slot(w.x, L.S, (uint32_t)L.msg, (uint32_t)sizeof(double));
+                w.y = encode_seg(w.y & qkdp::kPlanChkMask, (w.y >> 20) & 63u, (w.y >> 26) + 1, (uint32_t)(k & 63),
+                                 (uint32_t)dc);
+            }
+            const size_t tasks = h.chk.size() / 64;
+            std::vector<uint32_t> words(tasks * (size_t)(dc + 1) * 64);
+            for (size_t t = 0; t < tasks; ++t) {
+                for (size_t k = 0; k < (size_t)dc * 64; ++k)
+                    words[t * (size_t)(dc + 1) * 64 + k] =
+                        encode_slot(h.slot[t * (size_t)dc * 64 + k], L.S, (uint32_t)L.msg, (uint32_t)sizeof(double));
+                for (size_t l = 0; l < 64; ++l) words[(t * (size_t)(dc + 1) + (size_t)dc) * 64 + l] = h.chk[t * 64 + l];
+            }
+            words.resize((words.size() + 1) & ~(size_t)1, 0u);
+            for (size_t k = 0; k < words.size(); k += 2) enc.push_back(make_uint2(words[k], words[k + 1]));
         }
         uint2* d = nullptr;
         if (hipMalloc(&d, enc.size() * sizeof(uint2)) != hipSuccess)
@@ -1382,9 +1404,26 @@
             a.code = c->view_split();
             a.c2b = ws->c2b;
             a.plan_enc = nullptr;
+            a.cl_split = 0;
+            ws->last_cl_form = 0;
+            ws->last_cl_tasks = 0;
+            ws->last_cl_rem_tasks = c->n_tasks;
             if (rule == kRuleSp64 || msr) {
-                s = plan_for_layout(c, L, sdc, &a.plan_enc, esz);
+                int cl_form = 0;
+                if (spec && !ckpt && !long_code && rule == kRuleSp64 && c->cl_dc == sdc) {
+                    cl_form = kCheckLanesDefault;
+                    if (const DbgOpt e = debug_option(ws, "QKD_CHECK_LANES")) cl_form = std::max(0, std::min(2, e.as_int()));
+                }
+                s = plan_for_layout(c, L, sdc, &a.plan_enc, esz, cl_form);
                 if (s != QKD_OK) return s;
+                a.cl_split = 0;
+                if (cl_form != 0) {
+                    const qkd_code::ClHost& h = c->cl_host[cl_form - 1];
+                    a.cl_split = 0x80000000u | (uint32_t)h.cl_tasks | ((uint32_t)h.rem_tasks << 16);
+                    ws->last_cl_form = cl_form;
+                    ws->last_cl_tasks = h.cl_tasks;
+                    ws->last_cl_rem_tasks = h.rem_tasks;
+                }
             }
             const size_t slots = (size_t)c->max_dv * c->n_pad;
             if (const DbgOpt e = debug_option(ws, "QKD_C2B_PAD")) {
@@ -2243,6 +2282,14 @@
     return QKD_OK;
 }
 
+qkd_status qkd_debug_check_lanes(qkd_workspace* ws, int32_t* form, int32_t* lane_tasks, int32_t* edge_tasks) {
+    if (!ws) return set_error(QKD_ERR_INVALID_ARG, "null workspace");
+    if (form) *form = ws->last_cl_form;
+    if (lane_tasks) *lane_tasks = ws->last_cl_tasks;
+    if (edge_tasks) *edge_tasks = ws->last_cl_rem_tasks;
+    return QKD_OK;
+}
+
 qkd_status qkd_debug_decoder_timing(qkd_workspace* ws, int start, double* ms_total, uint64_t* launches) {
     if (!ws) return set_error(QKD_ERR_INVALID_ARG, "null workspace");
     DeviceGuard g(ws->device);
diff --git a/qkd_ldpc_amd/csrc/decode_split.hip b/qkd_ldpc_amd/csrc/decode_split.hip
--- a/qkd_ldpc_amd/csrc/decode_split.hip
+++ b/qkd_ldpc_amd/csrc/decode_split.hip
@@ -590,6 +590,125 @@
     if (bad != 0 && lane == 0) atomicOr(round_word, 2u);
 }
 
+template <int DC, bool PSI_IN>
+__device__ __forceinline__ void spec_check_phase_lanes(const uint32_t* __restrict__ clp,
+                                                       const SplitStore<double>& ms, int n_tasks, float thr_dn,
+                                                       float thr_up, uint32_t* round_word, int wave, int lane) {
+    using qkds::f2;
+    static_assert(DC % 2 == 0 && DC <= 8, "check-lane buckets: pairs of entries, degree <= 8");
+    constexpr int NW = kDecodeBlock / 64;
+    constexpr int NP = DC + 1;
+    constexpr int HP = DC / 2;
+    int t = wave;
+    if (t >= n_tasks) return;
+    struct Words {
+        uint32_t s[DC];
+        uint32_t c;
+    };
+    const uint32_t vlane = (uint32_t)lane * 4u;
+    auto load_words = [&](int tt, Words& w) {
+        const char* const base =
+            reinterpret_cast<const char*>(clp) + (size_t)__builtin_amdgcn_readfirstlane(tt * (NP * 64 * 4));
+#pragma unroll
+        for (int k = 0; k < DC; ++k) w.s[k] = *reinterpret_cast<const uint32_t*>(base + k * 256 + vlane);
+        w.c = *reinterpret_cast<const uint32_t*>(base + DC * 256 + vlane);
+    };
+    bool bad = false;
+    auto step = [&](const Words& w_t, Words& w_n) -> bool {
+        typedef __attribute__((address_space(3))) const uint32_t LdsU32;
+        SplitStore<double>::Raw x[DC];
+#pragma unroll
+        for (int k = 0; k < DC; ++k) x[k] = ms.ld_raw(w_t.s[k]);
+        const uint32_t sword = *reinterpret_cast<LdsU32*>((size_t)qkdp::chk_word_addr(w_t.c));
+        const int deg = (int)qkdp::chk_word_deg(w_t.c);
+        f2 ph[DC];
+        uint32_t negs = 0;
+#pragma unroll
+        for (int k = 0; k < DC; k += 2) {
+            const f2 b0 = qkds::unpack_iv(ms.pick(x[k])), b1 = qkds::unpack_iv(ms.pick(x[k + 1]));
+            const bool in0 = k < deg, in1 = k + 1 < deg;
+            bool n0, n1, ok0, ok1;
+            f2 r0, r1;
+            if constexpr (PSI_IN) {
+                n0 = b0.x < 0.0f;
+                n1 = b1.x < 0.0f;
+                ok0 = b0.x == b0.x;
+                ok1 = b1.x == b1.x;
+                r0 = neg_iv_if(n0, b0);
+                r1 = neg_iv_if(n1, b1);
+            } else {
+                n0 = b0.y < 0.0f;
+                n1 = b1.y < 0.0f;
+                const f2 a0 = neg_iv_if(n0, b0), a1 = neg_iv_if(n1, b1);
+                ok0 = a0.x > 1.0e-30f;
+                ok1 = a1.x > 1.0e-30f;
+                qkds::phi_bounds2(a0, a1, r0, r1);
+            }
+            bad |= (in0 && !ok0) || (in1 && !ok1);
+            negs |= (in0 && n0 ? 1u : 0u) << k;
+            negs |= (in1 && n1 ? 1u : 0u) << (k + 1);
+            ph[k] = (in0 && ok0) ? r0 : f2{0.0f, 0.0f};
+            ph[k + 1] = (in1 && ok1) ? r1 : f2{0.0f, 0.0f};
+            __builtin_amdgcn_sched_barrier(0);
+        }
+        __builtin_amdgcn_sched_barrier(0);
+        load_words(t + NW, w_n);
+        __builtin_amdgcn_sched_barrier(0);
+        const uint32_t sp = ((sword >> qkdp::chk_word_bit(w_t.c)) + (uint32_t)__popc(negs)) & 1u;
+        f2 pp[HP], oth[HP];
+#pragma unroll
+        for (int i = 0; i < HP; ++i) pp[i] = ph[2 * i] + ph[2 * i + 1];
+        {
+            f2 pre = pp[0];
+            oth[0] = f2{0.0f, 0.0f};
+#pragma unroll
+            for (int i = 1; i < HP; ++i) {
+                oth[i] = pre;
+                pre = pre + pp[i];
+            }
+            f2 suf = pp[HP - 1];
+#pragma unroll
+            for (int i = HP - 2; i >= 0; --i) {
+                oth[i] = i == 0 ? suf : oth[i] + suf;
+                suf = suf + pp[i];
+            }
+        }
+        auto ext_of = [&](int k) -> f2 {
+            const f2 sum = oth[k >> 1] + ph[k ^ 1];
+            const float mg = __builtin_fmaf(sum.y, (float)(DC + 2) * qkds::kSumRel, qkds::kRefSumAbs);
+            f2 e = sum + f2{-mg, mg};
+            e.x = e.x > 0.0f ? e.x : 0.0f;
+            bad |= k < deg && !(e.y < qkds::kPsiSumMax);
+            return e;
+        };
+#pragma unroll
+        for (int k = DC - 1; k >= 1; k -= 2) {
+            const f2 e1 = ext_of(k);
+            const f2 e0 = ext_of(k - 1);
+            f2 m0, m1;
+            qkds::phi_bounds_out2(e0, e1, m0, m1);
+            m0.x = __builtin_amdgcn_fmed3f(m0.x, 0.0f, thr_dn);
+            m0.y = __builtin_amdgcn_fmed3f(m0.y, 0.0f, thr_up);
+            m1.x = __builtin_amdgcn_fmed3f(m1.x, 0.0f, thr_dn);
+            m1.y = __builtin_amdgcn_fmed3f(m1.y, 0.0f, thr_up);
+            const uint32_t s0 = (sp ^ (negs >> (k - 1))) & 1u;
+            const uint32_t s1 = (sp ^ (negs >> k)) & 1u;
+            ms.st_w(w_t.s[k - 1], qkds::pack_iv(neg_iv_if(s0 != 0u, m0)));
+            ms.st_w(w_t.s[k], qkds::pack_iv(neg_iv_if(s1 != 0u, m1)));
+            __builtin_amdgcn_sched_barrier(0);
+        }
+        t = __builtin_amdgcn_readfirstlane(t + NW);
+        return t < n_tasks;
+    };
+    Words wa, wb;
+    load_words(t, wa);
+    for (;;) {
+        if (!step(wa, wb)) break;
+        if (!step(wb, wa)) break;
+    }
+    if (fold64(__ballot(bad)) != 0 && lane == 0) atomicOr(round_word, 2u);
+}
+
 __device__ __forceinline__ uint32_t fold_tab_pos(uint32_t p, uint32_t code) { return p * 16u + (code ^ (p & 15u)); }
 __device__ void fold_table_fill(const DeviceCode& c, const double* ctab, double log_p, double thr, double* ftab,
                                 int entries) {
@@ -844,8 +963,20 @@
 #else
 #define QKD_SPLIT_BOUNDS __launch_bounds__(kDecodeBlock)
 #endif
+typedef const __attribute__((address_space(4))) DecodeArgs KernArgs;
+__device__ __forceinline__ KernArgs* kernel_args() {
+    KernArgs* p = (KernArgs*)__builtin_amdgcn_kernarg_segment_ptr();
+    asm volatile("" : "+s"(p));
+    return p;
+}
+template <class... A>
+constexpr bool sole_decode_args(void (*)(A...)) {
+    return sizeof...(A) == 1 && (std::is_same<A, DecodeArgs>::value && ...);
+}
 template <int MODE, int RULE, int DC, bool CLAMP, int SPEC, bool LONG = false>
 __global__ QKD_SPLIT_BOUNDS void decode_split_kernel(DecodeArgs a) {
+    static_assert(sole_decode_args(&decode_split_kernel<MODE, RULE, DC, CLAMP, SPEC, LONG>),
+                  "kernel_args(): DecodeArgs must be the only kernel parameter");
     static_assert(!LONG || (MODE == kModeKeys && RULE == kRuleSp64 && SPEC == 0), "long codes: exact keys path");
     using T = typename RuleMsg<RULE>::T;
     constexpr bool MSR = RULE == kRuleMinSumSplit || RULE == kRuleMinSumSplitSc;
@@ -883,6 +1014,7 @@
         kSlotGlobalBase - L.S * (uint32_t)sizeof(T)};
     const uint2* const plan = (RULE == kRuleSp64 || MSR) ? a.plan_enc : c.plan_slot;
     const uint32_t dummy_w = encode_slot((uint32_t)c.n, L.S, (uint32_t)L.msg, (uint32_t)sizeof(T));
+    constexpr bool CLANES = SPEC == 1 && !LONG && (DC == 4 || DC == 6);
     const int tid = threadIdx.x;
     const int lane = tid & 63;
     const int wave = __builtin_amdgcn_readfirstlane(tid >> 6);
@@ -939,63 +1071,72 @@
     }
     PhaseClock pc(a.phase);
 
-    unsigned long long* const win64 = reinterpret_cast<unsigned long long*>(a.win);
-    auto window_of = [&](uint32_t fr) -> int {
-        if (!SPEC || a.spec_always || fr >= a.n_frames) return -1;
-        const uint32_t wn = fr >> a.win_shift;
-        return wn < a.win_lag ? -1 : (int)(wn - a.win_lag);
-    };
-    auto spec_policy = [&](uint32_t fr, unsigned long long v) -> uint32_t {
-        const int k = window_of(fr);
+    auto win64 = [](KernArgs* ka) { return reinterpret_cast<unsigned long long*>(ka->win); };
+    auto window_of = [&](KernArgs* ka, uint32_t fr) -> int {
+        if (!SPEC || ka->spec_always || fr >= ka->n_frames) return -1;
+        const uint32_t wn = fr >> ka->win_shift;
+        return wn < ka->win_lag ? -1 : (int)(wn - ka->win_lag);
+    };
+    auto spec_policy = [&](KernArgs* ka, uint32_t fr, unsigned long long v) -> uint32_t {
+        const int k = window_of(ka, fr);
         if (k < 0) return 1u;
-        const uint32_t W = 1u << a.win_shift;
+        const uint32_t W = 1u << ka->win_shift;
         for (uint32_t polls = 0; (uint32_t)v < W; ++polls) {
             if (polls >= (1u << 24)) return 1u;
             __builtin_amdgcn_s_sleep(2);
-            v = __hip_atomic_load(win64 + k, __ATOMIC_RELAXED, __HIP_MEMORY_SCOPE_AGENT);
+            v = __hip_atomic_load(win64(ka) + k, __ATOMIC_RELAXED, __HIP_MEMORY_SCOPE_AGENT);
         }
         return (uint32_t)(v >> 32) * 6u <= W ? 1u : 0u;
     };
-    auto window_peek = [&](uint32_t fr) -> unsigned long long {
-        const int k = window_of(fr);
-        return k < 0 ? 0ull : __hip_atomic_load(win64 + k, __ATOMIC_RELAXED, __HIP_MEMORY_SCOPE_AGENT);
-    };
-    auto claim = [&]() -> uint32_t {
-        const uint32_t k = atomicAdd(a.counter, 1u);
-        if (a.frame_list == nullptr) return k;
-        return k < *a.frame_count ? a.frame_list[k] : a.n_frames;
-    };
+    auto window_peek = [&](KernArgs* ka, uint32_t fr) -> unsigned long long {
+        const int k = window_of(ka, fr);
+        return k < 0 ? 0ull : __hip_atomic_load(win64(ka) + k, __ATOMIC_RELAXED, __HIP_MEMORY_SCOPE_AGENT);
+    };
+    auto claim = [&](KernArgs* ka) -> uint32_t {
+        const uint32_t k = atomicAdd(ka->counter, 1u);
+        if (ka->frame_list == nullptr) return k;
+        return k < *ka->frame_count ? ka->frame_list[k] : ka->n_frames;
+    };
+    KernArgs* const qa = kernel_args();
     if (tid == 0) {
-        ctl[1] = claim();
-        ctl[6] = spec_policy(ctl[1], window_peek(ctl[1]));
-    }
-    uint32_t next_f = 0;
+        ctl[1] = claim(qa);
+        ctl[6] = spec_policy(qa, ctl[1], window_peek(qa, ctl[1]));
+    }
     for (;;) {
         pc.mark(4);
-        for (int w = tid; w < m_words; w += kDecodeBlock) {
+        auto frame_tid = [&]() -> int {
+            int t0 = tid;
+            asm volatile("" : "+v"(t0));
+            return t0;
+        };
+        const int ptid = frame_tid();
+        KernArgs* const pa = kernel_args();
+        for (int w = ptid; w < m_words; w += kDecodeBlock) {
             xsyn[w] = 0;
             xunc[w] = 0;
         }
         __syncthreads();
         const uint32_t f = (uint32_t)__builtin_amdgcn_readfirstlane((int)ctl[1]);
-        if (f >= a.n_frames) break;
-        if (tid == 0) next_f = claim();
-        uint32_t frame_replays = 0;
+        if (f >= pa->n_frames) break;
+        uint32_t next_f = 0;
+        if (tid == 0) next_f = claim(pa);
+        uint32_t* const frame_replays = ctl + 9;
 
         const uint64_t* bw = reinterpret_cast<const uint64_t*>(smem + L.tval);
         if (MODE == kModeKeys) {
             uint64_t* w = reinterpret_cast<uint64_t*>(smem + L.tval);
             uint64_t* aw = reinterpret_cast<uint64_t*>(smem + L.aw);
-            const bool ka = a.key_ok != nullptr;
-            for (int q = tid; q < (int)a.words; q += kDecodeBlock) {
-                const uint64_t bv = a.bob_w[(size_t)f * a.words + q];
-                const uint64_t av = ka ? a.alice_w[(size_t)f * a.words + q] : 0ull;
+            const bool ka = pa->key_ok != nullptr;
+            const uint32_t words = pa->words;
+            for (int q = ptid; q < (int)words; q += kDecodeBlock) {
+                const uint64_t bv = pa->bob_w[(size_t)f * words + q];
+                const uint64_t av = ka ? pa->alice_w[(size_t)f * words + q] : 0ull;
                 w[q] = bv;
                 aw[q] = av;
                 if constexpr (MSC || LONG) bwl[q] = bv;
             }
-            const uint32_t* sy = a.synw + (size_t)f * 2 * m_words;
-            for (int q = tid; q < m_words; q += kDecodeBlock) {
+            const uint32_t* sy = pa->synw + (size_t)f * 2 * m_words;
+            for (int q = ptid; q < m_words; q += kDecodeBlock) {
                 tsyn[q] = sy[q];
                 qsyn[q] = sy[m_words + q];
             }
@@ -1003,9 +1144,15 @@
         }
         const bool spec0 = SPEC == 1 && ctl[6] != 0;
         uint64_t bobmask = 0;
+        unsigned long long next_win = 0;
+        if (tid == 0) {
+            ctl[8] = next_f;
+            *frame_replays = 0;
+            if (SPEC) next_win = window_peek(pa, next_f);
+        }
         auto init_slots = [&](bool as_interval) {
             int r = 0;
-            for (int i = tid; i < c.n; i += kDecodeBlock, ++r) {
+            for (int i = frame_tid(); i < c.n; i += kDecodeBlock, ++r) {
                 T l;
                 if (MODE == kModeLlr) {
                     l = (T)a.llr[(size_t)f * c.n + c.perm[i]];
@@ -1031,17 +1178,17 @@
         };
         if constexpr (kRunSyn) {
             const int zwords = (int)(n_pad >> 6);
-            for (int q = tid; q < zwords; q += kDecodeBlock)
-                zw[q] = (MODE == kModeKeys && q < (int)a.words) ? bw[q] : 0ull;
+            for (int q = ptid; q < zwords; q += kDecodeBlock)
+                zw[q] = (MODE == kModeKeys && q < (int)pa->words) ? bw[q] : 0ull;
             if (MODE == kModeKeys) {
-                for (int w = tid; w < m_words; w += kDecodeBlock)
-                    xsyn[w] = tsyn[w] ^ qsyn[w] ^ (lsign ? c.chk_odd[w] : 0u);
+                for (int w = ptid; w < m_words; w += kDecodeBlock)
+                    xsyn[w] = tsyn[w] ^ qsyn[w] ^ (lsign ? pa->code.chk_odd[w] : 0u);
             }
         }
         if (MODE == kModeLlr) {
             for (int j0 = wave * 64; j0 < c.m; j0 += kDecodeBlock) {
                 const int j = j0 + lane;
-                const int sj = j < c.m ? (a.syn[(size_t)f * c.m + j] != 0) : 0;
+                const int sj = j < c.m ? (pa->syn[(size_t)f * c.m + j] != 0) : 0;
                 const uint64_t sm = __ballot(sj);
                 if (lane == 0) {
                     tsyn[j0 >> 5] = (uint32_t)sm;
@@ -1049,15 +1196,14 @@
                 }
             }
         }
+        if (SPEC && tid == 0) *reinterpret_cast<unsigned long long*>(ctl + 10) = next_win;
         __syncthreads();
         pc.mark(0);
-        unsigned long long next_win = 0;
-        if (SPEC && tid == 0) next_win = window_peek(next_f);
 
         bool spec = spec0;
         if (SPEC == 1 && !spec && tid == 0) {
-            atomicAdd(a.replay_count, 1u);
-            frame_replays++;
+            atomicAdd(pa->replay_count, 1u);
+            ++*frame_replays;
         }
         bool done = false;
         uint32_t it = 0;
@@ -1084,11 +1230,35 @@
             uint32_t* rw = ctl + 4 + (rnd & 1u);
             if (SPEC && spec) {
                 if constexpr (SPEC) {
-                    if (!folded && fold1 && it == 1) {
+                    const bool psi_in = fold1 && it == 1;
+                    uint32_t cs = 0;
+                    if constexpr (CLANES) cs = a.cl_split;
+                    if (folded) {
+                    } else if (CLANES && (cs >> 31) != 0) {
+                        if constexpr (CLANES) {
+                            const int r_tasks = (int)((cs >> 16) & 0x7fffu);
+                            const uint2* const rplan = plan + cl_rem_offset(n_tasks);
+                            const uint32_t* const cl_words =
+                                reinterpret_cast<const uint32_t*>(plan + cl_words_offset(n_tasks, r_tasks));
+                            const int cl_tasks = (int)(cs & 0xffffu);
+                            if (psi_in) {
+                                spec_check_phase_lanes<DC, true>(cl_words, ms, cl_tasks, a.thr_dn, a.thr_up, rw, wave,
+                                                                 lane);
+                                spec_check_phase_psi<DC>(rplan, tsyn, ms, row, wtab, r_tasks, n_pad, dummy_w,
+                                                         a.thr_dn, a.thr_up, rw, wave, lane);
+                            } else {
+                                spec_check_phase_lanes<DC, false>(cl_words, ms, cl_tasks, a.thr_dn, a.thr_up, rw, wave,
+                                                                  lane);
+                                spec_check_phase_paired<DC>(rplan, tsyn, ms, row, wtab, r_tasks, n_pad, dummy_w,
+                                                            a.thr_dn, a.thr_up, rw, wave, lane);
+                            }
+                            __syncthreads();
+                        }
+                    } else if (psi_in) {
                         spec_check_phase_psi<DC>(plan, tsyn, ms, row, wtab, n_tasks, n_pad, dummy_w,
                                                  a.thr_dn, a.thr_up, rw, wave, lane);
                         __syncthreads();
-                    } else if (!folded) {
+                    } else {
                         spec_check_phase_paired<DC>(plan, tsyn, ms, row, wtab, n_tasks, n_pad, dummy_w, a.thr_dn,
                                                     a.thr_up, rw, wave, lane);
                         __syncthreads();
@@ -1282,9 +1452,9 @@
                     ms.st((uint32_t)c.n, (T)0);
                 }
                 if (tid == 0) {
-                    atomicAdd(a.replay_count, 1u);
-                    atomicAdd(a.spec_replays, 1ull);
-                    frame_replays++;
+                    atomicAdd(pa->replay_count, 1u);
+                    atomicAdd(pa->spec_replays, 1ull);
+                    ++*frame_replays;
                 }
                 continue;
             }
@@ -1307,9 +1477,9 @@
                     ms.st((uint32_t)c.n, (T)0);
                 }
                 if (tid == 0) {
-                    atomicAdd(a.replay_count, 1u);
-                    atomicAdd(a.spec_replays, 1ull);
-                    frame_replays++;
+                    atomicAdd(pa->replay_count, 1u);
+                    atomicAdd(pa->spec_replays, 1ull);
+                    ++*frame_replays;
                 }
             } else if (CKPT && !spec && it >= 2 && it + 1 < a.max_it && unsat < ck_lim) {
                 ckpt_io(true);
@@ -1319,36 +1489,39 @@
             }
         }
 
+        const int etid = frame_tid();
+        KernArgs* const ea = kernel_args();
         if (MODE == kModeKeys) {
-            if (a.key_ok) {
+            if (ea->key_ok) {
                 const uint64_t* aw = reinterpret_cast<const uint64_t*>(smem + L.aw);
                 bool mis = false;
-                if (tid < (int)a.words) {
-                    uint64_t d = zw[tid] ^ aw[tid];
-                    if ((tid + 1) * 64 > c.n) d &= (1ull << (c.n - tid * 64)) - 1ull;
+                if (etid < (int)ea->words) {
+                    uint64_t d = zw[etid] ^ aw[etid];
+                    if ((etid + 1) * 64 > c.n) d &= (1ull << (c.n - etid * 64)) - 1ull;
                     mis = d != 0;
                 }
                 if (__any(mis) && lane == 0) atomicOr(ctl + 7, 1u);
             }
-            if (a.bits_out)
-                for (int q = tid; q < (int)a.words; q += kDecodeBlock) a.zout[(size_t)f * a.words + q] = zw[q];
-        } else if (a.bits_out) {
-            for (int i = tid; i < c.n; i += kDecodeBlock)
-                a.bits_out[(size_t)f * c.n + c.perm[i]] = (uint8_t)((zw[i >> 6] >> (i & 63)) & 1u);
+            if (ea->bits_out)
+                for (int q = etid; q < (int)ea->words; q += kDecodeBlock) ea->zout[(size_t)f * ea->words + q] = zw[q];
+        } else if (ea->bits_out) {
+            for (int i = etid; i < c.n; i += kDecodeBlock)
+                ea->bits_out[(size_t)f * c.n + c.perm[i]] = (uint8_t)((zw[i >> 6] >> (i & 63)) & 1u);
         }
         if (tid == 0) {
-            a.iters[f] = done ? it + 1 : a.max_it;
-            a.sp_ok[f] = done ? 1 : 0;
-            ctl[1] = next_f;
+            ea->iters[f] = done ? it + 1 : a.max_it;
+            ea->sp_ok[f] = done ? 1 : 0;
+            const uint32_t nf = ctl[8];
+            ctl[1] = nf;
             if (SPEC) {
-                __hip_atomic_fetch_add(win64 + (f >> a.win_shift), ((unsigned long long)frame_replays << 32) | 1ull,
+                __hip_atomic_fetch_add(win64(ea) + (f >> ea->win_shift), ((unsigned long long)*frame_replays << 32) | 1ull,
                                        __ATOMIC_RELAXED, __HIP_MEMORY_SCOPE_AGENT);
-                ctl[6] = spec_policy(next_f, next_win);
+                ctl[6] = spec_policy(ea, nf, *reinterpret_cast<const unsigned long long*>(ctl + 10));
             }
         }
         __syncthreads();
-        if (MODE == kModeKeys && a.key_ok && tid == 0) {
-            a.key_ok[f] = ctl[7] ? 0 : 1;
+        if (MODE == kModeKeys && ea->key_ok && tid == 0) {
+            ea->key_ok[f] = ctl[7] ? 0 : 1;
             ctl[7] = 0;
         }
     }
diff --git a/qkd_ldpc_amd/csrc/host.cpp b/qkd_ldpc_amd/csrc/host.cpp
--- a/qkd_ldpc_amd/csrc/host.cpp
+++ b/qkd_ldpc_amd/csrc/host.cpp
@@ -33,7 +33,7 @@
     "QKD_SPEC_CAP", "QKD_SPEC_CKPT", "QKD_CKPT_UNSAT", "QKD_SPEC_POLICY", "QKD_FOLD_TABLE",
     "QKD_DECODE_KERNEL", "QKD_MINSUM_STORE", "QKD_DECODE_GRID", "QKD_SPLIT_BUDGET", "QKD_C2B_PAD",
     "QKD_ILV", "QKD_ILV_GRID", "QKD_KEYGEN", "QKD_SYN_SLICED", "QKD_SYN_BYTES", "QKD_BIT_ORDER",
-    "QKD_PHASE_TIMING"};
+    "QKD_PHASE_TIMING", "QKD_CHECK_LANES"};
 static std::mutex g_dbg_mu;
 static std::map<std::string, std::string> g_dbg;
 
@@ -420,6 +420,32 @@
         QKD_HIP(hipMalloc(&c->d_plan_slot, plan2.size() * sizeof(uint2)));
         QKD_HIP(hipMemcpy(c->d_plan_slot, plan2.data(), plan2.size() * sizeof(uint2), hipMemcpyHostToDevice));
         c->plan_slot_host = std::move(plan2);
+        c->cl_dc = 0;
+        if (c->d_bit_code && max_dc <= 6) {
+            const int dc = max_dc <= 4 ? 4 : 6;
+            std::vector<int32_t> slot_of(e);
+            for (int32_t k = 0; k < e; ++k) slot_of[k] = krow[k] * c->n_pad + inv[cidx[k]];
+            for (int form = 0; form < 2; ++form) {
+                qkdp::CheckLanePlan cl;
+                if (!qkdp::build_check_lane_plan(n, m, cptr, cidx, krow.data(), dc, kDecodeBlock / 64, form == 1, cl))
+                    return set_error(QKD_ERR_UNSUPPORTED, "check-lane plan: check degree outside [1, %d]", dc);
+                qkd_code::ClHost& h = c->cl_host[form];
+                h.cl_tasks = cl.n_tasks;
+                h.rem_tasks = cl.rem.n_tasks;
+                h.slot.resize(cl.edge.size());
+                for (size_t k = 0; k < cl.edge.size(); ++k)
+                    h.slot[k] = cl.edge[k] < 0 ? (uint32_t)n : (uint32_t)slot_of[cl.edge[k]];
+                h.chk = cl.chkw;
+                h.rem.resize(cl.rem.word.size());
+                for (size_t k = 0; k < cl.rem.word.size(); ++k) {
+                    const uint32_t b = cl.rem.word[k] & qkdp::kPlanBitMask;
+                    h.rem[k] = make_uint2((cl.rem.word[k] >> 24) * (uint32_t)c->n_pad +
+                                              (b < (uint32_t)n ? (uint32_t)inv[b] : b),
+                                          cl.rem.seg[k]);
+                }
+            }
+            c->cl_dc = dc;
+        }
     }
     const uint64_t draws = qkdr::trial_draws((uint32_t)n);
     const uint64_t per_lane = (draws + kKeygenLanes - 1) / kKeygenLanes;
diff --git a/qkd_ldpc_amd/csrc/qkd_decode.h b/qkd_ldpc_amd/csrc/qkd_decode.h
--- a/qkd_ldpc_amd/csrc/qkd_decode.h
+++ b/qkd_ldpc_amd/csrc/qkd_decode.h
@@ -67,6 +67,7 @@
     size_t totals_stride;
     uint32_t lds_budget;
     const uint2* plan_enc;
+    uint32_t cl_split;
     const uint32_t* synw;
     uint64_t* zout;
     uint32_t spec_cap;
@@ -400,6 +401,14 @@
     return (j & 31u) | (start << kSegStartShift) | (wi << kSegWiShift) | (((j >> 5) * 4u) << kSegWordShift);
 }
 
+static_assert(qkdp::kChkWordShift == kSegWordShift, "check words address syndrome words as segment words do");
+__host__ __device__ inline size_t cl_rem_offset(int n_tasks) {
+    return (size_t)(n_tasks + qkdp::kPlanPadTasks) * 64;
+}
+__host__ __device__ inline size_t cl_words_offset(int n_tasks, int rem_tasks) {
+    return cl_rem_offset(n_tasks) + (size_t)(rem_tasks + qkdp::kPlanPadTasks) * 64;
+}
+
 using DecodeFn = void (*)(DecodeArgs);
 DecodeFn pick_split_decode(int mode, int rule, bool clamp, int max_dc, int* dc);
 DecodeFn pick_split_long(bool clamp, int max_dc, int* dc);
diff --git a/qkd_ldpc_amd/csrc/qkd_internal.h b/qkd_ldpc_amd/csrc/qkd_internal.h
--- a/qkd_ldpc_amd/csrc/qkd_internal.h
+++ b/qkd_ldpc_amd/csrc/qkd_internal.h
@@ -20,6 +20,7 @@
 constexpr int kTab2MaxDv = 3;
 constexpr int kTab2MaxEntries = 2048;
 constexpr int kFoldTabMaxEntries = 1024;
+constexpr int kCheckLanesDefault = 1;
 constexpr size_t kC2bPad = 64;
 constexpr int kBitPadRounds = 4;
 __host__ __device__ inline int tab2_stride(int max_dv) { return (1 << (1 + max_dv)) * max_dv; }
@@ -90,6 +91,7 @@
     double* c2b = nullptr;
     size_t c2b_slots = 0;
     uint32_t* counter = nullptr;
+    int last_cl_form = -1, last_cl_tasks = 0, last_cl_rem_tasks = 0;
     uint64_t* alice_w = nullptr;
     uint64_t* bob_w = nullptr;
     size_t key_frames = 0;
@@ -137,6 +139,13 @@
     std::vector<uint2> plan_slot_host;
     mutable std::map<std::pair<uint32_t, uint32_t>, uint2*> d_plan_enc;
     mutable std::mutex plan_mu;
+    struct ClHost {
+        int32_t cl_tasks = 0, rem_tasks = 0;
+        std::vector<uint32_t> slot, chk;
+        std::vector<uint2> rem;
+    };
+    int32_t cl_dc = 0;
+    ClHost cl_host[2];
     int32_t n_pat = 0;
     std::vector<uint8_t> pat_deg;
     uint16_t* d_bit_pat = nullptr;
diff --git a/qkd_ldpc_amd/csrc/qkd_plan.h b/qkd_ldpc_amd/csrc/qkd_plan.h
--- a/qkd_ldpc_amd/csrc/qkd_plan.h
+++ b/qkd_ldpc_amd/csrc/qkd_plan.h
@@ -102,4 +102,74 @@
     return true;
 }
 
+constexpr uint32_t kChkDegShift = 5, kChkWordShift = 19;
+constexpr uint32_t encode_chk(uint32_t j, uint32_t deg) {
+    return (j & 31u) | (deg << kChkDegShift) | (((j >> 5) * 4u) << kChkWordShift);
 }
+constexpr uint32_t chk_word_bit(uint32_t w) { return w & 31u; }
+constexpr uint32_t chk_word_deg(uint32_t w) { return (w >> kChkDegShift) & 15u; }
+constexpr uint32_t chk_word_addr(uint32_t w) { return w >> kChkWordShift; }
+
+struct CheckLanePlan {
+    int32_t dc = 0;
+    int32_t n_tasks = 0;
+    std::vector<int32_t> edge;
+    std::vector<int32_t> chk;
+    std::vector<uint32_t> chkw;
+    std::vector<int32_t> rem_checks;
+    WavePlan rem;
+};
+
+inline bool build_check_lane_plan(int32_t n, int32_t m, const int32_t* cptr, const int32_t* cidx,
+                                  const int32_t* krow, int dc, int round_tasks, bool pure, CheckLanePlan& p) {
+    if (dc < 1 || dc > 15 || m > 65536 || round_tasks < 1) return false;
+    for (int32_t j = 0; j < m; ++j) {
+        const int32_t d = cptr[j + 1] - cptr[j];
+        if (d < 1 || d > dc) return false;
+    }
+    p.dc = dc;
+    const int32_t per_round = 64 * round_tasks;
+    const int32_t m_cl = pure ? m : (m / per_round) * per_round;
+    p.n_tasks = (m_cl + 63) / 64;
+    const size_t tasks_pad = (size_t)p.n_tasks + kPlanPadTasks;
+    p.edge.assign(tasks_pad * dc * 64, -1);
+    p.chk.assign(tasks_pad * 64, -1);
+    p.chkw.assign(tasks_pad * 64, 0u);
+    for (int32_t t = 0; t < p.n_tasks; ++t) {
+        for (int l = 0; l < 64; ++l) {
+            const int32_t j = t * 64 + l;
+            if (j >= m_cl) break;
+            p.chk[(size_t)t * 64 + l] = j;
+            const int32_t d = cptr[j + 1] - cptr[j];
+            p.chkw[(size_t)t * 64 + l] = encode_chk((uint32_t)j, (uint32_t)d);
+            for (int k = 0; k < d; ++k) p.edge[((size_t)t * dc + k) * 64 + l] = cptr[j] + k;
+        }
+    }
+    p.rem_checks.clear();
+    for (int32_t j = m_cl; j < m; ++j) p.rem_checks.push_back(j);
+    const int32_t mr = (int32_t)p.rem_checks.size();
+    std::vector<int32_t> rptr(mr + 1, 0), ridx, rrow, redge;
+    for (int32_t q = 0; q < mr; ++q) {
+        const int32_t j = p.rem_checks[q];
+        for (int32_t e = cptr[j]; e < cptr[j + 1]; ++e) {
+            ridx.push_back(cidx[e]);
+            rrow.push_back(krow[e]);
+            redge.push_back(e);
+        }
+        rptr[q + 1] = (int32_t)ridx.size();
+    }
+    p.rem = WavePlan();
+    if (!build_wave_plan(n, mr, rptr.data(), ridx.data(), rrow.data(), p.rem)) return false;
+    for (size_t s = 0; s < p.rem.chk.size(); ++s) {
+        const int32_t q = p.rem.chk[s];
+        if (q < 0) continue;
+        p.rem.chk[s] = p.rem_checks[q];
+        p.rem.seg[s] = (p.rem.seg[s] & ~kPlanChkMask) | (uint32_t)p.rem_checks[q];
+    }
+    std::vector<int32_t> soe(cptr[m], -1);
+    for (size_t r = 0; r < redge.size(); ++r) soe[redge[r]] = p.rem.slot_of_edge[r];
+    p.rem.slot_of_edge.swap(soe);
+    return true;
+}
+
+}
```

Measured after the change: 35.98 billion bit/s, median of 6. 6.1% higher.
